# LARS-research/RED-GNN

Measured on AMD Instinct MI355X. Metric: edges aggregated/sec + MRR-eval queries/sec, family KG n_layer=3 at 1/2/4/8 GPU, higher is better.
Workload: dtype f32; 1 GPU; C2 synthetic KG 10000 entities / 50 relations / 200000 triples (seed 1234), n_layer=3 hidden_dim=64 attn_dim=5, eval step = expansion + fused layers + GRU/readout + filtered ranking, 1024 queries per GPU; batch_per_gpu=1024, global_batch=1024

## Files before the change

include/redgnn.h:

```cpp
#ifndef REDGNN_H
#define REDGNN_H

#include <stddef.h>
#include <stdint.h>

#ifdef __cplusplus
extern "C" {
#endif

typedef struct rg_graph rg_graph;
typedef struct rg_frontier rg_frontier;

const char* rg_last_error(void);
int rg_version(void);
int rg_hipgraph_fill_nodes(void* hip_graph);

int rg_graph_create(int32_t n_ent, int32_t n_rel, const int32_t* triples_host, int64_t n,
                    int add_inverse, rg_graph** out);
int rg_graph_create_device(int32_t n_ent, int32_t n_rel, const int32_t* triples_dev, int64_t n,
                           int add_inverse, void* stream, rg_graph** out);
int rg_graph_export_packs(const rg_graph* g, int32_t* n_packs, int32_t* n_vrows, int32_t* ent_host, int32_t* pack_host, int32_t* rows_host,
                          int32_t* vrows_host);
int rg_tgraph_create(int32_t n_ent, int32_t n_rela_rows, int32_t n_time, const int32_t* quads_host, int64_t n,
                     rg_graph** out);
int rg_tgraph_create_excluding(int32_t n_ent, int32_t n_rela_rows, int32_t n_time, const int32_t* quads_host, int64_t n,
                               const int64_t* exclude_rows_host, int64_t n_exclude, rg_graph** out);
int rg_graph_destroy(rg_graph* g);
int64_t rg_graph_n_fact(const rg_graph* g);
int rg_graph_export(const rg_graph* g, int32_t* out_ptr_host, int32_t* out_rel_tail_host,
                    int32_t* in_ptr_host, int32_t* in_head_rel_host);
int rg_graph_export_time(const rg_graph* g, int32_t* out_time_host, int32_t* in_time_host);

size_t rg_frontier_workspace_bytes(int32_t n_ent, int32_t batch, int32_t n_levels);
int rg_frontier_create(int32_t n_ent, int32_t batch, int32_t n_levels, void* workspace_dev,
                       size_t workspace_bytes, rg_frontier** out);
int rg_frontier_destroy(rg_frontier* f);
int rg_frontier_reset(rg_frontier* f, const int32_t* q_sub_dev, void* stream);
int rg_frontier_reset_nodes(rg_frontier* f, const int32_t* nodes_dev, int64_t n, void* stream);
int rg_frontier_expand(rg_frontier* f, const rg_graph* g, int64_t* counts_host, void* stream);
int rg_frontier_expand_async(rg_frontier* f, const rg_graph* g, void* stream);
int rg_frontier_expand_nodes_async(rg_frontier* f, const rg_graph* g, int32_t* nodes_out, int32_t* prev_idx_out, void* stream);
int rg_frontier_set_edge_hint(rg_frontier* f, int64_t n_edges);
const int32_t* rg_frontier_count_ptr(const rg_frontier* f);
int rg_frontier_level_counts(const rg_frontier* f, int64_t* counts_host, void* stream);
int rg_frontier_nodes(const rg_frontier* f, int32_t* nodes_out, int32_t* prev_idx_out,
                      int32_t* old_nodes_new_idx_out, void* stream);
size_t rg_frontier_edges_scratch_bytes(int64_t n_new);
int rg_frontier_edges(const rg_frontier* f, const rg_graph* g, int32_t level,
                      const int32_t* nodes_new, int64_t n_new, int32_t* edges_out,
                      int32_t* row_ptr_out, void* scratch_dev, void* stream);

size_t rg_layer_fwd_scratch_bytes(const rg_frontier* f, const rg_graph* g, int32_t ld);
int rg_layer_fwd_plan(const rg_frontier* f, const rg_graph* g, int32_t level, int64_t n_old, int64_t n_new,
                      int64_t n_edges, int32_t ld);
int rg_layer_fwd(const rg_frontier* f, const rg_graph* g, int32_t level, int64_t n_new,
                 const float* hidden, const float* rela, int32_t d, int32_t ld,
                 const float* a_s, const float* a_r, const float* a_q, int32_t ap,
                 const float* w_alpha, const float* b_alpha, int32_t attn_dim,
                 float* agg_out, void* scratch_dev, size_t scratch_bytes, int32_t walk, void* stream);

int rg_attn_tables(int32_t n_layer, int32_t n_rela_rows, int32_t batch, int32_t d, int32_t ld, int32_t attn_dim, int32_t ap,
                   const float* const* rela, const float* const* Wr, const float* const* Wqr, const float* const* bqr,
                   const int64_t* q_rel, float* a_r_out, float* a_q_out, float* rela_pad_out, void* stream);

int rg_tlayer_fwd(const rg_frontier* f, const rg_graph* g, int32_t level, int64_t n_new, const int32_t* q_time,
                  const float* hidden_dir, const float* rela_dir, const float* time_dir, int32_t d, int32_t ld,
                  const float* a_s, const float* a_r, const float* a_q, int32_t ap,
                  const float* w_alpha, const float* b_alpha, int32_t attn_dim,
                  float* agg_out, void* scratch_dev, size_t scratch_bytes, void* stream);

int rg_frontier_set_window(rg_frontier* f, const int32_t* win_lo_dev, const int32_t* win_hi_dev, int32_t n_data);
int rg_xlayer_fwd(const rg_frontier* f, const rg_graph* g, int32_t level, int64_t n_new, const int32_t* q_time,
                  const int32_t* loop_time, const int32_t* row_time, int32_t n_data,
                  const float* hidden_p, const float* rela_p, const float* time_p, int32_t n_tab, int32_t d, int32_t ld,
                  const float* a_s, const float* a_r, const float* a_q, int32_t ap,
                  const float* w_alpha, const float* b_alpha, int32_t attn_dim,
                  float* agg_out, void* scratch_dev, size_t scratch_bytes, void* stream);

size_t rg_layer_bwd_scratch_bytes(const rg_frontier* f, const rg_graph* g, int32_t ld, int32_t ap);
int rg_layer_bwd(const rg_frontier* f, const rg_graph* g, int32_t level, int64_t n_old,
                 const float* hidden, const float* rela, int32_t d, int32_t ld,
                 const float* a_s, const float* a_r, const float* a_q, int32_t ap,
                 const float* w_alpha, const float* b_alpha, int32_t attn_dim,
                 const float* grad_agg,
                 float* grad_hidden, float* grad_rela, float* grad_a_s, float* grad_a_r, float* grad_a_q,
                 float* grad_w_alpha, float* grad_b_alpha,
                 void* scratch_dev, size_t scratch_bytes, void* stream);

size_t rg_tlayer_bwd_scratch_bytes(const rg_frontier* f, const rg_graph* g, int32_t ld, int32_t ap);
int rg_tlayer_bwd(const rg_frontier* f, const rg_graph* g, int32_t level, int64_t n_old, const int32_t* q_time,
                  const float* hidden_dir, const float* rela_dir, const float* time_dir, int32_t d, int32_t ld,
                  const float* a_s, const float* a_r, const float* a_q, int32_t ap,
                  const float* w_alpha, const float* b_alpha, int32_t attn_dim,
                  const float* grad_agg,
                  float* grad_hidden_dir, float* grad_rela_dir, float* grad_time_dir, float* grad_a_s, float* grad_a_r,
                  float* grad_a_q, float* grad_w_alpha,
                  void* scratch_dev, size_t scratch_bytes, void* stream);

int rg_xlayer_bwd(const rg_frontier* f, const rg_graph* g, int32_t level, int64_t n_old, const int32_t* q_time,
                  const int32_t* loop_time, const int32_t* row_time, int32_t n_data,
                  const float* hidden_p, const float* rela_p, const float* time_p, int32_t n_tab, int32_t d, int32_t ld,
                  const float* a_s, const float* a_r, const float* a_q, int32_t ap,
                  const float* w_alpha, const float* b_alpha, int32_t attn_dim,
                  const float* grad_agg,
                  float* grad_hidden_p, float* grad_rela_p, float* grad_time_p, float* grad_a_s, float* grad_a_r,
                  float* grad_a_q, float* grad_w_alpha,
                  void* scratch_dev, size_t scratch_bytes, void* stream);
// ... 128 lines not shown
```

red-gnn_amd/_lib.py:

```python
import ctypes as C
import os

_PKG = os.path.dirname(os.path.abspath(__file__))
LIB_PATH = os.environ.get("RG_LIB") or os.path.join(_PKG, "libredgnn.so")

SYMBOLS = [
    "rg_last_error", "rg_version", "rg_hipgraph_fill_nodes",
    "rg_graph_create", "rg_graph_create_device", "rg_graph_export_packs", "rg_tgraph_create", "rg_tgraph_create_excluding", "rg_graph_destroy", "rg_graph_n_fact", "rg_graph_export",
    "rg_frontier_workspace_bytes", "rg_frontier_create", "rg_frontier_destroy", "rg_frontier_reset",
    "rg_frontier_reset_nodes", "rg_frontier_expand", "rg_frontier_nodes", "rg_frontier_edges_scratch_bytes", "rg_frontier_edges",
    "rg_layer_fwd_scratch_bytes", "rg_layer_fwd", "rg_layer_fwd_plan", "rg_tlayer_fwd", "rg_xlayer_fwd", "rg_frontier_set_window", "rg_layer_bwd_scratch_bytes", "rg_layer_bwd", "rg_tlayer_bwd_scratch_bytes", "rg_tlayer_bwd", "rg_xlayer_bwd", "rg_dense_fwd_supported", "rg_dense_scratch_bytes", "rg_dense_fwd", "rg_dense_fwd_dev", "rg_dense_train_fwd", "rg_dense_train_fwd_as", "rg_rows_addmm", "rg_dense_train_bwd", "rg_dense_train_bwd2", "rg_split3_roundtrip", "rg_split3_product_check", "rg_gram_tn_scratch_bytes", "rg_gram_tn", "rg_rank",
    "rg_frontier_expand_async", "rg_frontier_expand_nodes_async", "rg_frontier_set_edge_hint", "rg_frontier_count_ptr", "rg_frontier_level_counts", "rg_attn_tables",
    "rg_explain_scratch_bytes", "rg_explain_seed", "rg_explain_count", "rg_explain_emit", "rg_explain_gather",
    "rg_topk",
    "rg_attn_profile",
    "rg_graph_export_time", "rg_texplain_count", "rg_texplain_emit", "rg_tattn_profile",
    "rg_segment_rank", "rg_segment_topk",
    "rg_xexplain_count", "rg_xexplain_emit",
    "rg_xattn_profile", "rg_rows_linear",
    "rg_segment_eval",
    "rg_paths_scratch_bytes", "rg_paths_topk",
]

_lib = None


class NativeError(RuntimeError):
    pass


def lib():
    global _lib
    if _lib is not None:
        return _lib
    if not os.path.exists(LIB_PATH):
        raise NativeError(
            "libredgnn.so is missing at %s: the HIP extension is not built. Run "
            "`python -c 'import __graft_entry__ as g; g.build()'` (needs hipcc). There is no CPU fallback." % LIB_PATH)
    import torch
    L = C.CDLL(LIB_PATH)
    vp, i32, i64, sz = C.c_void_p, C.c_int32, C.c_int64, C.c_size_t
    L.rg_last_error.restype = C.c_char_p
    L.rg_version.restype = C.c_int
    L.rg_hipgraph_fill_nodes.argtypes = [vp]
    L.rg_graph_create.argtypes = [i32, i32, vp, i64, C.c_int, C.POINTER(vp)]
    L.rg_graph_create_device.argtypes = [i32, i32, vp, i64, C.c_int, vp, C.POINTER(vp)]
    L.rg_graph_export_packs.argtypes = [vp, C.POINTER(i32), C.POINTER(i32), vp, vp, vp, vp]
    L.rg_tgraph_create.argtypes = [i32, i32, i32, vp, i64, C.POINTER(vp)]
    L.rg_tgraph_create_excluding.argtypes = [i32, i32, i32, vp, i64, vp, i64, C.POINTER(vp)]
    L.rg_graph_destroy.argtypes = [vp]
    L.rg_graph_n_fact.argtypes = [vp]
    L.rg_graph_n_fact.restype = i64
    L.rg_graph_export.argtypes = [vp, vp, vp, vp, vp]
    L.rg_frontier_workspace_bytes.argtypes = [i32, i32, i32]
    L.rg_frontier_workspace_bytes.restype = sz
    L.rg_frontier_create.argtypes = [i32, i32, i32, vp, sz, C.POINTER(vp)]
    L.rg_frontier_destroy.argtypes = [vp]
    L.rg_frontier_reset.argtypes = [vp, vp, vp]
    L.rg_frontier_reset_nodes.argtypes = [vp, vp, i64, vp]
    L.rg_frontier_expand.argtypes = [vp, vp, C.POINTER(i64), vp]
    L.rg_frontier_expand_async.argtypes = [vp, vp, vp]
    L.rg_frontier_expand_nodes_async.argtypes = [vp, vp, vp, vp, vp]
    L.rg_frontier_set_edge_hint.argtypes = [vp, i64]
    L.rg_attn_tables.argtypes = [i32, i32, i32, i32, i32, i32, i32, vp, vp, vp, vp, vp, vp, vp, vp, vp]
    L.rg_frontier_count_ptr.argtypes = [vp]
    L.rg_frontier_count_ptr.restype = vp
    L.rg_frontier_level_counts.argtypes = [vp, C.POINTER(i64), vp]
    L.rg_frontier_nodes.argtypes = [vp, vp, vp, vp, vp]
    L.rg_frontier_edges_scratch_bytes.argtypes = [i64]
    L.rg_frontier_edges_scratch_bytes.restype = sz
    L.rg_frontier_edges.argtypes = [vp, vp, i32, vp, i64, vp, vp, vp, vp]
    L.rg_layer_fwd_scratch_bytes.argtypes = [vp, vp, i32]
    L.rg_layer_fwd_scratch_bytes.restype = sz
    L.rg_layer_fwd.argtypes = [vp, vp, i32, i64, vp, vp, i32, i32, vp, vp, vp, i32, vp, vp, i32, vp, vp, sz, i32, vp]
    L.rg_layer_fwd_plan.argtypes = [vp, vp, i32, i64, i64, i64, i32]
    L.rg_tlayer_fwd.argtypes = [vp, vp, i32, i64, vp, vp, vp, vp, i32, i32, vp, vp, vp, i32, vp, vp, i32, vp, vp, sz, vp]
    L.rg_xlayer_fwd.argtypes = [vp, vp, i32, i64, vp, vp, vp, i32, vp, vp, vp, i32, i32, i32, vp, vp, vp, i32, vp, vp, i32, vp, vp, sz, vp]
    L.rg_frontier_set_window.argtypes = [vp, vp, vp, i32]
    L.rg_layer_bwd_scratch_bytes.argtypes = [vp, vp, i32, i32]
    L.rg_layer_bwd_scratch_bytes.restype = sz
    L.rg_layer_bwd.argtypes = [vp, vp, i32, i64, vp, vp, i32, i32, vp, vp, vp, i32, vp, vp, i32,
                               vp, vp, vp, vp, vp, vp, vp, vp, vp, sz, vp]
    L.rg_tlayer_bwd_scratch_bytes.argtypes = [vp, vp, i32, i32]
    L.rg_tlayer_bwd_scratch_bytes.restype = sz
    L.rg_tlayer_bwd.argtypes = [vp, vp, i32, i64, vp, vp, vp, vp, i32, i32, vp, vp, vp, i32, vp, vp, i32,
                                vp, vp, vp, vp, vp, vp, vp, vp, vp, sz, vp]
    L.rg_xlayer_bwd.argtypes = [vp, vp, i32, i64, vp, vp, vp, i32, vp, vp, vp, i32, i32, i32, vp, vp, vp, i32, vp, vp, i32,
                                vp, vp, vp, vp, vp, vp, vp, vp, vp, sz, vp]
    L.rg_dense_fwd_supported.argtypes = [i32, i32]
    L.rg_dense_fwd.argtypes = [i64, i32, i32, vp, vp, vp, vp, i32, vp, vp, vp, vp, vp, i32, i32, vp, vp, vp, i32, vp, vp, i32, vp, i64, vp]
    L.rg_dense_scratch_bytes.argtypes = [i32, i32]
    L.rg_dense_scratch_bytes.restype = i64
    L.rg_dense_fwd_dev.argtypes = [i64, vp, i64, i32, i32, vp, vp, vp, vp, i32, vp, vp, vp, vp, vp, i32, i32, vp, vp, vp, i32, vp, vp, i32, vp, i64, vp]
    L.rg_dense_train_fwd.argtypes = [i64, i32, vp, vp, vp, vp, i32, vp, vp, vp, vp, vp, vp, vp, vp, vp]
    L.rg_dense_train_fwd_as.argtypes = [i64, i32, vp, vp, vp, vp, i32, vp, vp, vp, vp, vp, vp, i32, i32, vp, vp, vp, vp, vp]
    L.rg_rows_addmm.argtypes = [vp, i64, vp, i64, i32, vp, i32, i64, vp, i64, vp]
    L.rg_dense_train_bwd.argtypes = [i64, i32, vp, vp, vp, vp, C.c_float, i32, vp, vp, vp, vp, vp, vp, vp, vp, vp]
    L.rg_dense_train_bwd2.argtypes = [i64, i32, vp, vp, vp, vp, C.c_float, i32, vp, vp, vp, vp, vp, vp, vp, vp, vp, vp]
    L.rg_rank.argtypes = [vp, i32, i32, vp, vp, vp, vp, vp, vp]
    L.rg_topk.argtypes = [vp, i32, i32, i32, vp, vp, vp, vp, i64, vp, vp, vp]
    L.rg_split3_roundtrip.argtypes = [vp, i64, i32, vp, vp, vp]
    L.rg_gram_tn_scratch_bytes.argtypes = [i32, i32]
    L.rg_gram_tn_scratch_bytes.restype = sz
    L.rg_gram_tn.argtypes = [vp, i64, i32, vp, i64, i32, i64, vp, vp, vp, sz, vp]
    L.rg_split3_product_check.argtypes = [i32, i64, i32, vp, vp, vp, vp, i32, vp, vp, vp, vp, vp, vp]
    L.rg_explain_scratch_bytes.argtypes = [vp]
    L.rg_explain_scratch_bytes.restype = sz
    L.rg_explain_seed.argtypes = [vp, i32, i32, i32, vp, vp, vp, vp]
    L.rg_explain_count.argtypes = [vp, vp, i32, i32, i32, vp, vp, vp, vp, i32, vp, vp, i32, C.c_float, vp, vp, vp, sz,
                                   C.POINTER(i64), vp]
    L.rg_explain_emit.argtypes = [vp, vp, i32, i32, i32, vp, vp, vp, vp, i32, vp, vp, i32, C.c_float, vp, vp, vp, vp]
    L.rg_explain_gather.argtypes = [i64, i32, i32, vp, vp, vp, vp, i64, vp, vp, vp]
    L.rg_attn_profile.argtypes = [vp, vp, i32, i32, i32, i64, vp, vp, vp, i32, vp, vp, i32, vp, vp, vp]
    L.rg_graph_export_time.argtypes = [vp, vp, vp]
    L.rg_texplain_count.argtypes = L.rg_explain_count.argtypes
    L.rg_texplain_emit.argtypes = [vp, vp, i32, i32, i32, vp, vp, vp, vp, i32, vp, vp, i32, C.c_float, vp, vp, vp, vp, vp]
    L.rg_tattn_profile.argtypes = [vp, vp, i32, i32, i32, i64, vp, vp, vp, vp, i32, vp, vp, i32, vp, vp, vp]
    L.rg_segment_rank.argtypes = [vp, vp, i64, vp, i32, vp, i32, vp, vp, vp, vp, i64, vp, vp, vp, vp, i64, vp, vp, vp, vp, vp]
    L.rg_segment_topk.argtypes = [vp, vp, i64, vp, i32, i32, i32, vp, vp, vp, vp, i64, vp, vp, vp, vp]
    L.rg_segment_eval.argtypes = [vp, vp, i64, vp, i32, vp, i32, i32, vp, vp, vp, vp, i64, vp, vp, vp, vp, i64, vp, vp, vp, vp]
    L.rg_xexplain_count.argtypes = L.rg_explain_count.argtypes
    L.rg_xexplain_emit.argtypes = L.rg_texplain_emit.argtypes
    L.rg_rows_linear.argtypes = [vp, i64, i64, i32, vp, vp, i32, vp, i64, vp]
    L.rg_xattn_profile.argtypes = [vp, vp, i32, i32, i32, i64, vp, vp, vp, vp, i32, i32, vp, vp, vp, i32, vp, vp, i32, vp, vp, vp]
    L.rg_paths_scratch_bytes.argtypes = [i64, i32]
    L.rg_paths_scratch_bytes.restype = sz
    L.rg_paths_topk.argtypes = [vp, vp, vp, i32, i32, i32, i32, vp, vp, vp, vp, vp]
    _lib = L
# ... 20 lines not shown
```

red-gnn_amd/csrc/common.h:

```cpp
#pragma once
#include <hip/hip_runtime.h>
#include <stdint.h>
#include <stdio.h>
#include <string>
#include <type_traits>

#include "redgnn.h"

namespace rg {

void set_error(const char* fmt, ...);

#define RG_CHECK(cond, ...)                 \
  do {                                      \
    if (!(cond)) {                          \
      ::rg::set_error(__VA_ARGS__);         \
      return 1;                             \
    }                                       \
  } while (0)

#define RG_HIP(expr)                                                                  \
  do {                                                                                \
    hipError_t e_ = (expr);                                                           \
    if (e_ != hipSuccess) {                                                           \
// ... 45 lines not shown
  return v + __int_as_float(t);
}

template <int G>
__device__ __forceinline__ float group_sum(float v) {
  if constexpr (G >= 16) {
    v = dpp_add<0x128>(v);
    v = dpp_add<0x124>(v);
    v = dpp_add<0x122>(v);
    v = dpp_add<0x121>(v);
    if constexpr (G >= 32) v += __shfl_xor(v, 16, 64);
    if constexpr (G >= 64) v += __shfl_xor(v, 32, 64);
  } else {
    for (int o = G / 2; o > 0; o >>= 1) v += __shfl_xor(v, o, 64);
  }
  return v;
}

}

#include <vector>
namespace rg { int place_rows_best_fit(const int4* vrows, int32_t n_vrows, std::vector<int4>* place, std::vector<int32_t>* pack_nrows); }

constexpr int RG_VROW_MAX = 128;
struct rg_vrows {
  int32_t n = 0, n_split = 0, n_slots = 0;
  int4* rows = nullptr;
  int4* split = nullptr;
};

constexpr int RG_PACK = 128;
struct rg_packs {
  int32_t n = 0;
  int2* ent = nullptr;
  int4* pack = nullptr;
  int2* rows = nullptr;
};

struct rg_graph {
  void* arena = nullptr;
  int32_t n_ent = 0, n_rel = 0;
  int32_t n_rela_rows = 0;
  int32_t n_time = 0;
  int32_t* in_time = nullptr;
  int32_t* out_time = nullptr;
  int64_t n_fact = 0;
  int32_t max_in_deg = 0, max_out_deg = 0;
  int32_t* out_ptr = nullptr;
  int2* out_rt = nullptr;
  int32_t* in_ptr = nullptr;
  int2* in_hr = nullptr;
  uint32_t* in_pk = nullptr;
  uint32_t* out_pk = nullptr;
  rg_vrows in_vr, out_vr;
  rg_packs in_pk_packs;
  int32_t* rel_ptr = nullptr;
  int2* rel_ht = nullptr;
  rg_vrows rel_vr;
  int32_t* rel_tm = nullptr;
  int32_t* time_ptr = nullptr;
  int2* time_ht = nullptr;
  int32_t* time_rel = nullptr;
  rg_vrows time_vr;
};

constexpr int RG_MAX_LEVELS = 16;
constexpr int RG_QSTRIDE = 32;
constexpr size_t RG_QUEUE_BYTES = 8 * RG_QSTRIDE * sizeof(int32_t);
struct rg_frontier {
  int32_t n_ent = 0, B = 0, BW = 0, W = 0, n_levels = 0;
  uint32_t* bitsT[2] = {nullptr, nullptr};
  int2* bm[RG_MAX_LEVELS] = {};
  uint32_t* words_tmp = nullptr;
  int32_t* prefix_tmp = nullptr;
  int32_t* scan_scratch = nullptr;
  int32_t* counters = nullptr;
  const int32_t* win_lo = nullptr;
  const int32_t* win_hi = nullptr;
  int32_t win_n_data = 0;
  mutable bool queues_clean = false;
  int32_t* queues = nullptr;
  int64_t* counts_pinned = nullptr;
  int level = -1;
  int tcur = 0;
  int64_t n_nodes[RG_MAX_LEVELS] = {};
  int64_t n_edges = 0;
  int64_t edge_hint = -1;
  const int2* bm_of(int lvl) const { return bm[lvl % n_levels]; }
};
```

red-gnn_amd/csrc/dense.hip:

```cpp
#include "dense_common.h"

using namespace rg;

namespace {

template <int DP>
__device__ __forceinline__ int sw(int row, int slot) { return row * (DP / 4) + (slot ^ (row & (DP / 4 - 1))); }


template <int NB, bool TRAIN>
__global__ __launch_bounds__(DENSE_T, 2) void dense_kernel(DenseArgs A) {
  constexpr int DP = 16 * NB;
  constexpr int S = DP / 4;
  constexpr int KS = DP / 4;
  constexpr int NW = DENSE_T / 64;
  extern __shared__ float4 lds[];
  if (A.n_dev) { A.n = *A.n_dev; A.n_tiles = (int)((A.n + 15) / 16); }
  float4* Wh_l = lds;
  float4* Wih_l = Wh_l + DP * S;
  float4* Whh_l = Wih_l + 3 * DP * S;
  float4* E_l = Whh_l + 3 * DP * S;
  float* bias_l = reinterpret_cast<float*>(E_l + 32 * S);
  float4* tiles = reinterpret_cast<float4*>(bias_l + 4 * DP);

// ... 186 lines not shown

    float hn[KS];
#pragma unroll
    for (int ob = 0; ob < NB; ++ob) {
      f32x4 ar = bias_acc(0, ob), az = bias_acc(1, ob), ai = bias_acc(2, ob), ah = bias_acc(3, ob);
      mma3(Wih_l, 0 * DP + 16 * ob, 1 * DP + 16 * ob, 2 * DP + 16 * ob, xf, ar, az, ai);
      if (any_old) mma3(Whh_l, 0 * DP + 16 * ob, 1 * DP + 16 * ob, 2 * DP + 16 * ob, hf, ar, az, ah);
      float rgv[4], zgv[4], ngv[4];
#pragma unroll
      for (int r = 0; r < 4; ++r) {
        const float rg = fast_sigmoid(ar[r]), zg = fast_sigmoid(az[r]);
        const float ng = fast_tanh(ai[r] + rg * ah[r]);
        hn[4 * ob + r] = (1.0f - zg) * ng + zg * hf[4 * ob + r];
        rgv[r] = rg; zgv[r] = zg; ngv[r] = ng;
      }
      if constexpr (TRAIN) {
        const int64_t nd = row0 + li;
        const int col = 16 * ob + 4 * hq;
        if (nd < A.n && col < d) {
          float* w = A.ws_out + nd * (5 * (int64_t)d) + col;
          *reinterpret_cast<float4*>(w) = make_float4(rgv[0], rgv[1], rgv[2], rgv[3]);
          *reinterpret_cast<float4*>(w + d) = make_float4(zgv[0], zgv[1], zgv[2], zgv[3]);
          *reinterpret_cast<float4*>(w + 2 * d) = make_float4(ngv[0], ngv[1], ngv[2], ngv[3]);
          *reinterpret_cast<float4*>(w + 3 * d) = make_float4(hf[4 * ob + 0], hf[4 * ob + 1], hf[4 * ob + 2], hf[4 * ob + 3]);
          *reinterpret_cast<float4*>(w + 4 * d) = make_float4(ah[0], ah[1], ah[2], ah[3]);
        }
      }
    }

    const int64_t node = row0 + li;
    if (A.Ws) {
      const f32x4 ae = mma(E_l, 0, hn, zero4);
      if (node < A.n && 4 * hq < A.ap)
        reinterpret_cast<float4*>(A.a_s_out + node * A.ap)[hq] = make_float4(ae[0], ae[1], ae[2], ae[3]);
    }
    if (A.W_final) {
      const f32x4 ae = mma(E_l, 16, hn, zero4);
      if (node < A.n && hq == 0) {
        const int b = A.nodes[2 * node], e = A.nodes[2 * node + 1];
        A.scores[(int64_t)b * A.n_ent + e] = ae[0];
      }
    }

    __builtin_amdgcn_fence(__ATOMIC_RELEASE, "workgroup");
    __builtin_amdgcn_wave_barrier();
#pragma unroll
    for (int ob = 0; ob < NB; ++ob)
      tile[sw<DP>(li, 4 * ob + hq)] = make_float4(hn[4 * ob + 0], hn[4 * ob + 1], hn[4 * ob + 2], hn[4 * ob + 3]);
    __builtin_amdgcn_fence(__ATOMIC_RELEASE, "workgroup");
    __builtin_amdgcn_wave_barrier();
#pragma unroll
    for (int it = 0; it < 16 * S / 64; ++it) {
      const int e = it * 64 + lane, r = e / S, sl = e - r * S;
      if (row0 + r < A.n && sl < A.ld4) A.hidden_out[(row0 + r) * A.ld4 + sl] = tile[sw<DP>(r, sl)];
    }
  }
}

template <int NB, bool TRAIN>
int launch(const DenseArgs& A, hipStream_t s) {
  constexpr int DP = 16 * NB, S = DP / 4, NW = DENSE_T / 64;
  const size_t lds = (size_t)(7 * DP * S + 32 * S) * sizeof(float4) + 4 * DP * sizeof(float) + (size_t)NW * 16 * S * sizeof(float4);
  RG_HIP(hipFuncSetAttribute((const void*)dense_kernel<NB, TRAIN>, hipFuncAttributeMaxDynamicSharedMemorySize, (int)lds));
  hipLaunchKernelGGL((dense_kernel<NB, TRAIN>), dim3(dense_grid(A, NW)), dim3(DENSE_T), lds, s, A);
  RG_LAUNCH_CHECK();
  return 0;
}

}

extern "C" int64_t rg_dense_scratch_bytes(int32_t d, int32_t precision) {
  if (d != 128) return 0;
  return precision == 1 ? rg::dense128_split_scratch_bytes() : precision == 2 ? rg::dense128_split3_scratch_bytes() : 0;
}

extern "C" int rg_dense_fwd_supported(int32_t d, int32_t attn_dim) { return ((d >= 1 && d <= 64) || d == 128) && attn_dim <= 16; }

static int dense_fwd_impl(int64_t n, const int32_t* n_dev, int64_t n_hint, int32_t d, int32_t ld, const float* agg, const float* hidden_prev,
                          const int32_t* prev_idx, const float* W_h, int32_t act, const float* w_ih, const float* w_hh,
                          const float* b_ih, const float* b_hh, const float* Ws_next, int32_t attn_dim, int32_t ap,
                          float* a_s_out, const float* W_final, const int32_t* nodes, int32_t n_ent, float* scores_all,
                          float* hidden_out, int32_t precision, void* scratch, int64_t scratch_bytes, void* stream) {
  RG_CHECK(agg && W_h && w_ih && w_hh && b_ih && b_hh && hidden_out, "rg_dense_fwd: NULL argument");
  RG_CHECK(precision >= 0 && precision <= 2, "rg_dense_fwd: precision=%d (0 = f32 MFMA, 1 = two-term f16 split, 2 = exact three-term f16 split)",
           precision);
  RG_CHECK(!prev_idx || hidden_prev, "rg_dense_fwd: prev_idx given without hidden_prev");
  RG_CHECK((d >= 1 && d <= 64) || d == 128, "rg_dense_fwd: hidden_dim %d not supported by the fused kernel (<= 64, or 128)", d);
  RG_CHECK(ld >= d && ld % 4 == 0 && ld <= 128, "rg_dense_fwd: ld=%d", ld);
  RG_CHECK(act >= 0 && act <= 2, "rg_dense_fwd: act=%d", act);
  RG_CHECK(!Ws_next || (a_s_out && attn_dim >= 1 && attn_dim <= 16 && ap >= attn_dim && ap % 4 == 0 && ap <= 16),
           "rg_dense_fwd: attn_dim=%d ap=%d not supported (<= 16)", attn_dim, ap);
  RG_CHECK(!W_final || (nodes && scores_all && n_ent > 0), "rg_dense_fwd: readout needs nodes and scores_all");
  RG_CHECK((((uintptr_t)agg | (uintptr_t)hidden_prev | (uintptr_t)hidden_out | (uintptr_t)a_s_out) & 15) == 0,
           "rg_dense_fwd: float buffers must be 16-B aligned");
  if (n == 0) return 0;
  DenseArgs A = dense_args(n, d, ld, agg, hidden_prev, prev_idx, W_h, act, w_ih, w_hh, b_ih, b_hh, hidden_out);
  A.n_dev = n_dev; A.n_hint = n_hint;
  A.Ws = Ws_next; A.attn = attn_dim; A.ap = ap; A.a_s_out = a_s_out;
  A.W_final = W_final; A.nodes = nodes; A.n_ent = n_ent; A.scores = scores_all;
  hipStream_t s = (hipStream_t)stream;
  if (d == 128)
    return precision == 1 ? rg::dense128_split_launch(A, scratch, scratch_bytes, s)
         : precision == 2 ? rg::dense128_split3_launch(A, scratch, scratch_bytes, s) : rg::dense128_launch(A, s);
  if (precision == 1) return rg::dense_split_launch(A, s);
  if (precision == 2) return rg::dense_split3_launch(A, s);
  return d <= 32 ? launch<2, false>(A, s) : launch<4, false>(A, s);
}

extern "C" int rg_dense_fwd(int64_t n, int32_t d, int32_t ld, const float* agg, const float* hidden_prev,
                            const int32_t* prev_idx, const float* W_h, int32_t act, const float* w_ih, const float* w_hh,
                            const float* b_ih, const float* b_hh, const float* Ws_next, int32_t attn_dim, int32_t ap,
                            float* a_s_out, const float* W_final, const int32_t* nodes, int32_t n_ent, float* scores_all,
                            float* hidden_out, int32_t precision, void* scratch, int64_t scratch_bytes, void* stream) {
  return dense_fwd_impl(n, nullptr, 0, d, ld, agg, hidden_prev, prev_idx, W_h, act, w_ih, w_hh, b_ih, b_hh, Ws_next, attn_dim, ap,
                        a_s_out, W_final, nodes, n_ent, scores_all, hidden_out, precision, scratch, scratch_bytes, stream);
}

extern "C" int rg_dense_fwd_dev(int64_t n_cap, const int32_t* n_dev, int64_t n_hint, int32_t d, int32_t ld, const float* agg,
                                const float* hidden_prev, const int32_t* prev_idx, const float* W_h, int32_t act,
                                const float* w_ih, const float* w_hh, const float* b_ih, const float* b_hh, const float* Ws_next,
                                int32_t attn_dim, int32_t ap, float* a_s_out, const float* W_final, const int32_t* nodes,
                                int32_t n_ent, float* scores_all, float* hidden_out, int32_t precision, void* scratch,
                                int64_t scratch_bytes, void* stream) {
  RG_CHECK(n_dev != nullptr, "rg_dense_fwd_dev: n_dev is NULL");
  return dense_fwd_impl(n_cap, n_dev, n_hint, d, ld, agg, hidden_prev, prev_idx, W_h, act, w_ih, w_hh, b_ih, b_hh, Ws_next, attn_dim, ap,
                        a_s_out, W_final, nodes, n_ent, scores_all, hidden_out, precision, scratch, scratch_bytes, stream);
}

static int dense_train_fwd_impl(const char* who, int64_t n, int32_t d, const float* agg, const float* hidden_prev, const int32_t* prev_idx,
                                const float* W_h, int32_t act, const float* w_ih, const float* w_hh, const float* b_ih,
                                const float* b_hh, const float* mask, const float* Ws_next, int32_t attn_dim, int32_t ap,
                                float* hidden_out, float* x_out, float* gates_ws_out, float* a_s_out, void* stream) {
  RG_CHECK(agg && W_h && w_ih && w_hh && b_ih && b_hh && hidden_out && x_out && gates_ws_out, "%s: NULL argument", who);
  RG_CHECK(!prev_idx || hidden_prev, "%s: prev_idx given without hidden_prev", who);
  RG_CHECK((d >= 16 && d <= 64 && d % 4 == 0) || d == 128, "%s: hidden_dim %d not supported (16..64 in steps of 4, or 128)", who, d);
  RG_CHECK(act >= 0 && act <= 2, "%s: act=%d", who, act);
// ... 30 lines not shown
```

red-gnn_amd/csrc/dense128.hip:

```cpp
#include "dense_common.h"

namespace rg {
namespace {

constexpr int DP = 128, S = 32, KS = 32, NB = 8, NW = 8, T = 512;
constexpr int BLK = 16 * S;
constexpr int CHUNK = 3 * BLK;
constexpr int NL = 16 * S / 64;

__device__ __forceinline__ int swz(int row, int slot) { return row * S + (slot ^ (row & (S - 1))); }

template <bool TRAIN>
__global__ __launch_bounds__(T, 2) void dense128_kernel(DenseArgs A) {
  extern __shared__ float4 lds[];
  if (A.n_dev) { A.n = *A.n_dev; A.n_tiles = (int)((A.n + 15) / 16); }
  float4* wbuf = lds;
  float4* E_l = wbuf + 2 * CHUNK;
  float* bias_l = reinterpret_cast<float*>(E_l + 32 * S);
  float4* tiles = reinterpret_cast<float4*>(bias_l + 4 * DP);

  for (int i = threadIdx.x; i < 32 * S; i += T) {
    const int r = i / S, sl = i - r * S;
    const float* src = r < 16 ? (A.Ws && r < A.attn ? A.Ws + (int64_t)r * DP : nullptr) : (r == 16 ? A.W_final : nullptr);
    E_l[swz(r, sl)] = src ? *reinterpret_cast<const float4*>(src + 4 * sl) : make_float4(0.f, 0.f, 0.f, 0.f);
// ... 181 lines not shown
      if (hh) issue(r_hh, 16 * ob, DP + 16 * ob, 2 * DP + 16 * ob);
      else if (!last) issue(r_ih, 16 * (ob + 1), DP + 16 * (ob + 1), 2 * DP + 16 * (ob + 1));
      mma3(xf, ar, az, ai);
      if (hh || !last) publish(); else __syncthreads();
      if (hh) {
        if (!last) issue(r_ih, 16 * (ob + 1), DP + 16 * (ob + 1), 2 * DP + 16 * (ob + 1));
        mma3(hf, ar, az, ah);
        if (!last) publish(); else __syncthreads();
      }
      __builtin_amdgcn_sched_barrier(0);
#pragma unroll
      for (int r = 0; r < 4; ++r) {
        const float rg = fast_sigmoid(ar[r]), zg = fast_sigmoid(az[r]);
        const float ng = fast_tanh(ai[r] + rg * ah[r]);
        hn[4 * ob + r] = (1.0f - zg) * ng + zg * hf[4 * ob + r];
        if constexpr (TRAIN) { ar[r] = rg; az[r] = zg; ai[r] = ng; }
      }
      if constexpr (TRAIN) {
        const int64_t nd = row0 + li;
        if (nd < A.n) {
          float* w = A.ws_out + nd * (5 * (int64_t)DP) + 16 * ob + 4 * hq;
          *reinterpret_cast<float4*>(w) = make_float4(ar[0], ar[1], ar[2], ar[3]);
          *reinterpret_cast<float4*>(w + DP) = make_float4(az[0], az[1], az[2], az[3]);
          *reinterpret_cast<float4*>(w + 2 * DP) = make_float4(ai[0], ai[1], ai[2], ai[3]);
          *reinterpret_cast<float4*>(w + 3 * DP) = make_float4(hf[4 * ob + 0], hf[4 * ob + 1], hf[4 * ob + 2], hf[4 * ob + 3]);
          *reinterpret_cast<float4*>(w + 4 * DP) = make_float4(ah[0], ah[1], ah[2], ah[3]);
        }
      }
      __builtin_amdgcn_sched_barrier(0);
    }

    const int64_t node = row0 + li;
    if (A.Ws) {
      const f32x4 ae = mma_e(0, hn);
      if (node < A.n && 4 * hq < A.ap)
        reinterpret_cast<float4*>(A.a_s_out + node * A.ap)[hq] = make_float4(ae[0], ae[1], ae[2], ae[3]);
    }
    if (A.W_final) {
      const f32x4 ae = mma_e(16, hn);
      if (node < A.n && hq == 0) {
        const int b = A.nodes[2 * node], e = A.nodes[2 * node + 1];
        A.scores[(int64_t)b * A.n_ent + e] = ae[0];
      }
    }

    wave_sync();
#pragma unroll
    for (int ob = 0; ob < NB; ++ob)
      tile[swz(li, 4 * ob + hq)] = make_float4(hn[4 * ob + 0], hn[4 * ob + 1], hn[4 * ob + 2], hn[4 * ob + 3]);
    wave_sync();
#pragma unroll
    for (int it = 0; it < NL; ++it) {
      const int e = it * 64 + lane, r = e / S, sl = e - r * S;
      if (row0 + r < A.n) A.hidden_out[(row0 + r) * S + sl] = tile[swz(r, sl)];
    }
  }
}

}

int dense128_launch(const DenseArgs& A, hipStream_t s) {
  RG_CHECK(A.d == DP && A.ld4 == S, "rg_dense_fwd: the d = 128 kernel needs ld = 128 (got d=%d ld=%d)", A.d, A.ld4 * 4);
  const size_t lds = (size_t)(2 * CHUNK + 32 * S + NW * 16 * S) * sizeof(float4) + 4 * DP * sizeof(float);
  auto kern = A.ws_out ? dense128_kernel<true> : dense128_kernel<false>;
  RG_HIP(hipFuncSetAttribute((const void*)kern, hipFuncAttributeMaxDynamicSharedMemorySize, (int)lds));
  hipLaunchKernelGGL(kern, dim3(dense_grid(A, NW)), dim3(T), lds, s, A);
  RG_LAUNCH_CHECK();
  return 0;
}

}
```

red-gnn_amd/csrc/dense128_split.hip:

```cpp
#include "split3.h"

namespace rg {
namespace {

using namespace rg::sp3;

constexpr int DP = 128, NB = 8, KST = 4, KS = 32, NW = 8, T = 512;
constexpr int S = 32;
constexpr int BLK_B = 8192;
constexpr int CHUNK_B = 3 * BLK_B;
constexpr int N_BLOCKS = 58;
constexpr int HDR_B = 256;

__global__ __launch_bounds__(T) void prepare128_kernel(const float* __restrict__ W_h, const float* __restrict__ w_ih,
                                                        const float* __restrict__ w_hh, const float* __restrict__ Ws, int attn,
                                                        const float* __restrict__ W_final, char* __restrict__ image) {
  const int r = threadIdx.x >> 5, ch = threadIdx.x & 31;
  const float4 q = prepare128_scaled_chunk<T>(W_h, w_ih, w_hh, Ws, attn, W_final, image, r, ch);
  h4 hi, lo;
  split4(q.x, q.y, q.z, q.w, hi, lo);
  const int b = blockIdx.x, kb = ch >> 2, hq = ch & 3;
  const int slot = (4 * (kb >> 1) + hq) ^ (r & 15);
  char* blk = image + HDR_B + (int64_t)b * BLK_B;
  reinterpret_cast<h4*>(blk + (r * 16 + slot) * 16)[kb & 1] = hi;
// ... 171 lines not shown

    h8 gh[KST], gl[KST];
    float sc, inv;
    if (hh) {
      float hf[KS];
#pragma unroll
      for (int ob = 0; ob < NB; ++ob) {
        my_stash[ob * 64] = vh[ob];
        hf[4 * ob] = vh[ob].x; hf[4 * ob + 1] = vh[ob].y; hf[4 * ob + 2] = vh[ob].z; hf[4 * ob + 3] = vh[ob].w;
      }
      row_scale(row_abs_max(hf, row_abs_max(xf, 0.f)), sc, inv);
      split_frag(hf, sc, gh, gl);
    } else {
      row_scale(row_abs_max(xf, 0.f), sc, inv);
    }
    split_frag(xf, sc, xh, xl);
    const float inv_s = inv * inv_w * -LOG2E, inv_t = inv * inv_w * (-2.0f * LOG2E);
    h8 nh[KST], nl[KST];
    h4 nh0, nl0;
#pragma unroll
    for (int ob = 0; ob < NB; ++ob) {
      f32x4 ar = zero4, az = zero4, ai = zero4, ag = zero4;
      const bool last = ob == NB - 1;
      if (hh) issue(32 + ob, 40 + ob, 48 + ob);
      else if (!last) issue(8 + ob + 1, 16 + ob + 1, 24 + ob + 1);
      else issue(0, 1, 2);
      mma3(xh, xl, ar, az, ai);
      if (hh || !last) publish(); else __syncthreads();
      if (hh) {
        if (!last) issue(8 + ob + 1, 16 + ob + 1, 24 + ob + 1);
        else issue(0, 1, 2);
        mma3(gh, gl, ar, az, ag);
        if (!last) publish(); else __syncthreads();
      }
      const float4 br = *reinterpret_cast<const float4*>(bias_l + 0 * DP + 16 * ob + 4 * hq);
      const float4 bz = *reinterpret_cast<const float4*>(bias_l + 1 * DP + 16 * ob + 4 * hq);
      const float4 bi = *reinterpret_cast<const float4*>(bias_l + 2 * DP + 16 * ob + 4 * hq);
      const float4 bh = *reinterpret_cast<const float4*>(bias_l + 3 * DP + 16 * ob + 4 * hq);
      float4 ho = make_float4(0.f, 0.f, 0.f, 0.f);
      if (hh) ho = my_stash[ob * 64];
      const float hov[4] = {ho.x, ho.y, ho.z, ho.w};
      const float brv[4] = {br.x, br.y, br.z, br.w}, bzv[4] = {bz.x, bz.y, bz.z, bz.w};
      const float biv[4] = {bi.x, bi.y, bi.z, bi.w}, bhv[4] = {bh.x, bh.y, bh.z, bh.w};
      float hnv[4];
#pragma unroll
      for (int r = 0; r < 4; ++r) {
        const float rg = __builtin_amdgcn_rcpf(1.0f + __builtin_amdgcn_exp2f(fmaf(ar[r], inv_s, brv[r])));
        const float zg = __builtin_amdgcn_rcpf(1.0f + __builtin_amdgcn_exp2f(fmaf(az[r], inv_s, bzv[r])));
        const float ti = fmaf(ai[r], inv_t, biv[r]);
        const float th = fmaf(ag[r], inv_t, bhv[r]);
        const float ng = fmaf(2.0f, __builtin_amdgcn_rcpf(1.0f + __builtin_amdgcn_exp2f(fmaf(rg, th, ti))), -1.0f);
        hnv[r] = fmaf(zg, hov[r] - ng, ng);
      }
      if (node_ok) (A.hidden_out + row0 * S)[lane_off + 4 * ob] = make_float4(hnv[0], hnv[1], hnv[2], hnv[3]);
      h4 ch, cl;
      split4(hnv[0], hnv[1], hnv[2], hnv[3], ch, cl);
      if (ob & 1) {
        nh[ob >> 1] = __builtin_shufflevector(nh0, ch, 0, 1, 2, 3, 4, 5, 6, 7);
        nl[ob >> 1] = __builtin_shufflevector(nl0, cl, 0, 1, 2, 3, 4, 5, 6, 7);
      } else {
        nh0 = ch; nl0 = cl;
      }
    }

    if (A.Ws) {
      const f32x4 ae = mma_e(0, nh, nl);
      if (node_ok && 4 * hq < A.ap)
        reinterpret_cast<float4*>(A.a_s_out + node * A.ap)[hq] = make_float4(ae[0] * inv_e, ae[1] * inv_e, ae[2] * inv_e, ae[3] * inv_e);
    }
    if (A.W_final) {
      const f32x4 ae = mma_e(1, nh, nl);
      if (node_ok && hq == 0) A.scores[(int64_t)qe.x * A.n_ent + qe.y] = ae[0] * inv_e;
    }
  }
}

template <int ACT>
int launch(const DenseArgs& A, const char* image, hipStream_t s) {
  const size_t lds = 2 * CHUNK_B + 2 * BLK_B + 4 * DP * sizeof(float) + (size_t)NW * NB * 64 * sizeof(float4);
  RG_HIP(hipFuncSetAttribute((const void*)dense128_split_kernel<ACT>, hipFuncAttributeMaxDynamicSharedMemorySize, (int)lds));
  hipLaunchKernelGGL((dense128_split_kernel<ACT>), dim3(dense_grid(A, NW)), dim3(T), lds, s, A, image);
  RG_LAUNCH_CHECK();
  return 0;
}

}

int64_t dense128_split_scratch_bytes() { return HDR_B + (int64_t)N_BLOCKS * BLK_B; }

int dense128_split_launch(const DenseArgs& A, void* scratch, int64_t scratch_bytes, hipStream_t s) {
  RG_CHECK(A.d == DP && A.ld4 == S, "rg_dense_fwd: the d = 128 kernel needs ld = 128 (got d=%d ld=%d)", A.d, A.ld4 * 4);
  RG_CHECK(scratch && scratch_bytes >= dense128_split_scratch_bytes() && ((uintptr_t)scratch & 255) == 0,
           "rg_dense_fwd: precision 1 at d = 128 needs a 256-B aligned scratch of rg_dense_scratch_bytes(128, 1) = %lld bytes",
           (long long)dense128_split_scratch_bytes());
  char* image = (char*)scratch;
  hipLaunchKernelGGL(prepare128_kernel, dim3(N_BLOCKS), dim3(T), 0, s, A.W_h, A.w_ih, A.w_hh, A.Ws, A.attn, A.W_final, image);
  RG_LAUNCH_CHECK();
  return with_act(A.act, [&](auto ACT) { return launch<decltype(ACT)::value>(A, image, s); });
}

}
```

red-gnn_amd/csrc/dense128_split3.hip:

```cpp
#include "split3.h"

namespace rg {
namespace {

using namespace rg::sp3;
typedef long l2v __attribute__((ext_vector_type(2)));

constexpr int DP = 128, NB = 8, KST = 4, KS = 32, NW = 4, T = 256;
constexpr int S = 32;
constexpr int F16_B = 4096;
constexpr int LO_B = 2048;
constexpr int BLK_B = 2 * F16_B + LO_B;
constexpr int CHUNK_B = 3 * BLK_B;
constexpr int N_BLOCKS = 58;
constexpr int HDR_B = 256;
constexpr int PREP_T = 512;

__device__ __forceinline__ int lo_quad(int row, int hq, int half) { return (((hq & 1) + 2 * half + 4 * (hq >> 1)) ^ (2 * ((row >> 1) & 3))); }

__global__ __launch_bounds__(PREP_T) void prepare128x3_kernel(const float* __restrict__ W_h, const float* __restrict__ w_ih,
                                                               const float* __restrict__ w_hh, const float* __restrict__ Ws, int attn,
                                                               const float* __restrict__ W_final, char* __restrict__ image) {
  const int r = threadIdx.x >> 5, ch = threadIdx.x & 31;
  const float4 q = prepare128_scaled_chunk<PREP_T>(W_h, w_ih, w_hh, Ws, attn, W_final, image, r, ch);
// ... 218 lines not shown
    drop();
    const bool hh = __syncthreads_or(has_old) != 0;
    cur ^= 1;

    float xf[KS];
    const float sc_out = inv1 * inv_w * (ACT == 2 ? -2.0f * LOG2E : 1.0f);
    auto act_store = [&](f32x4 acc, const f32x4& acc8, int ob) {
      join(acc, acc8);
#pragma unroll
      for (int r = 0; r < 4; ++r) {
        float v = acc[r] * sc_out;
        if (ACT == 1) v = fmaxf(v, 0.f);
        else if (ACT == 2) v = fmaf(2.0f, __builtin_amdgcn_rcpf(1.0f + __builtin_amdgcn_exp2f(v)), -1.0f);
        xf[4 * ob + r] = v;
      }
    };
    {
      f32x4 c[3] = {zero4, zero4, zero4}, e[3] = {zero4, zero4, zero4};
      issue(3, 4, 5);
      mma3(X, c, e);
      act_store(c[0], e[0], 0); act_store(c[1], e[1], 1); act_store(c[2], e[2], 2);
      publish();
    }
    {
      f32x4 c[3] = {zero4, zero4, zero4}, e[3] = {zero4, zero4, zero4};
      issue(6, 7, 7);
      mma3(X, c, e);
      act_store(c[0], e[0], 3); act_store(c[1], e[1], 4); act_store(c[2], e[2], 5);
      publish();
    }
    {
      f32x4 c[3] = {zero4, zero4, zero4}, e[3] = {zero4, zero4, zero4};
      issue(8, 16, 24);
      mma3(X, c, e);
      act_store(c[0], e[0], 6); act_store(c[1], e[1], 7);
      publish();
    }

    Frag4 H;
    float sc, inv;
    float hf[KS];
#pragma unroll
    for (int ob = 0; ob < NB; ++ob) { hf[4 * ob] = vh[ob].x; hf[4 * ob + 1] = vh[ob].y; hf[4 * ob + 2] = vh[ob].z; hf[4 * ob + 3] = vh[ob].w; }
    if (hh) {
      row_scale(row_abs_max(hf, row_abs_max(xf, 0.f)), sc, inv);
      split_frag(hf, sc, H);
    } else {
      row_scale(row_abs_max(xf, 0.f), sc, inv);
    }
    split_frag(xf, sc, X);
    const float inv_s = inv * inv_w * -LOG2E, inv_t = inv * inv_w * (-2.0f * LOG2E);
    float hn[KS];
    const int rows_valid = (int)(A.n - row0 < 16 ? (A.n - row0 > 0 ? A.n - row0 : 0) : 16);
    const __amdgpu_buffer_rsrc_t r_out = __builtin_amdgcn_make_buffer_rsrc(reinterpret_cast<char*>(A.hidden_out + row0 * S), 0,
                                                                            rows_valid * S * 16, 0x00020000);
    auto gate_loop = [&](auto HH_) {
      constexpr bool HH = decltype(HH_)::value;
      f32x4 P[2][4][3];
      static_for<NB + 1>([&](auto OB) {
        constexpr int ob = decltype(OB)::value, cs = ob & 1, ps = cs ^ 1, pb = ob - 1;
        constexpr int OPS_R = 25, NOPS = 4 + 4 * OPS_R + 1;
        float4 bia[4];
        float s1[4], a1[4], ar[4], az[4], ai[4], ag[4], t1[4], t2[4], e1[4], e2[4], rg[4], zg[4], ti[4], th[4], uu[4], e3[4], ng[4], hnv[4];
        auto gate_op = [&](auto K) {
          constexpr int k = decltype(K)::value;
          f32x4 (&c)[3] = P[ps][0]; f32x4 (&e)[3] = P[ps][1]; f32x4 (&cg)[3] = P[ps][2]; f32x4 (&eg)[3] = P[ps][3];
          if constexpr (k < 4) {
            bia[k] = *reinterpret_cast<const float4*>(bias_l + k * DP + 16 * pb + 4 * hq);
            RG_PIN(bia[k].x);
          } else if constexpr (k < 4 + 4 * OPS_R) {
            constexpr int j = (k - 4) / 4, r = (k - 4) % 4;
            const float bvr = r == 0 ? bia[0].x : r == 1 ? bia[0].y : r == 2 ? bia[0].z : bia[0].w;
            const float bvz = r == 0 ? bia[1].x : r == 1 ? bia[1].y : r == 2 ? bia[1].z : bia[1].w;
            const float bvi = r == 0 ? bia[2].x : r == 1 ? bia[2].y : r == 2 ? bia[2].z : bia[2].w;
            const float bvh = r == 0 ? bia[3].x : r == 1 ? bia[3].y : r == 2 ? bia[3].z : bia[3].w;
            if constexpr (j == 0) { s1[r] = HH ? e[0][r] + eg[0][r] : e[0][r]; RG_PIN(s1[r]); }
            else if constexpr (j == 1) { a1[r] = HH ? c[0][r] + cg[0][r] : c[0][r]; RG_PIN(a1[r]); }
            else if constexpr (j == 2) { ar[r] = fmaf(s1[r], LO8_INV, a1[r]); RG_PIN(ar[r]); }
            else if constexpr (j == 3) { s1[r] = HH ? e[1][r] + eg[1][r] : e[1][r]; RG_PIN(s1[r]); }
            else if constexpr (j == 4) { a1[r] = HH ? c[1][r] + cg[1][r] : c[1][r]; RG_PIN(a1[r]); }
            else if constexpr (j == 5) { az[r] = fmaf(s1[r], LO8_INV, a1[r]); RG_PIN(az[r]); }
            else if constexpr (j == 6) { ai[r] = fmaf(e[2][r], LO8_INV, c[2][r]); RG_PIN(ai[r]); }
            else if constexpr (j == 7) { ag[r] = HH ? fmaf(eg[2][r], LO8_INV, cg[2][r]) : 0.f; RG_PIN(ag[r]); }
            else if constexpr (j == 8) { t1[r] = fmaf(ar[r], inv_s, bvr); RG_PIN(t1[r]); }
            else if constexpr (j == 9) { e1[r] = __builtin_amdgcn_exp2f(t1[r]); RG_PIN(e1[r]); }
            else if constexpr (j == 10) { t2[r] = fmaf(az[r], inv_s, bvz); RG_PIN(t2[r]); }
            else if constexpr (j == 11) { e2[r] = __builtin_amdgcn_exp2f(t2[r]); RG_PIN(e2[r]); }
            else if constexpr (j == 12) { t1[r] = 1.0f + e1[r]; RG_PIN(t1[r]); }
            else if constexpr (j == 13) { t2[r] = 1.0f + e2[r]; RG_PIN(t2[r]); }
            else if constexpr (j == 14) { rg[r] = __builtin_amdgcn_rcpf(t1[r]); RG_PIN(rg[r]); }
            else if constexpr (j == 15) { zg[r] = __builtin_amdgcn_rcpf(t2[r]); RG_PIN(zg[r]); }
            else if constexpr (j == 16) { ti[r] = fmaf(ai[r], inv_t, bvi); RG_PIN(ti[r]); }
            else if constexpr (j == 17) { th[r] = fmaf(ag[r], inv_t, bvh); RG_PIN(th[r]); }
            else if constexpr (j == 18) { uu[r] = fmaf(rg[r], th[r], ti[r]); RG_PIN(uu[r]); }
            else if constexpr (j == 19) { e3[r] = __builtin_amdgcn_exp2f(uu[r]); RG_PIN(e3[r]); }
            else if constexpr (j == 20) { uu[r] = 1.0f + e3[r]; RG_PIN(uu[r]); }
            else if constexpr (j == 21) { e3[r] = __builtin_amdgcn_rcpf(uu[r]); RG_PIN(e3[r]); }
            else if constexpr (j == 22) { ng[r] = fmaf(2.0f, e3[r], -1.0f); RG_PIN(ng[r]); }
            else if constexpr (j == 23) { uu[r] = hf[4 * pb + r] - ng[r]; RG_PIN(uu[r]); }
            else { hnv[r] = fmaf(zg[r], uu[r], ng[r]); RG_PIN(hnv[r]); }
          } else {
#pragma unroll
            for (int r = 0; r < 4; ++r) hn[4 * pb + r] = hnv[r];
            const u32x4 bits = {__float_as_uint(hnv[0]), __float_as_uint(hnv[1]), __float_as_uint(hnv[2]), __float_as_uint(hnv[3])};
            __builtin_amdgcn_raw_buffer_store_b128(bits, r_out, (lane_off + 4u * pb) * 16u, 0, 0);
          }
        };
        auto no_op = [&](auto) {};
// ... 66 lines not shown
```

red-gnn_amd/csrc/dense_split.hip:

```cpp
#include <type_traits>
#include "split3.h"

using namespace rg;
using namespace rg::sp3;

namespace {

template <int NB, int ACT>
__global__ __launch_bounds__(DENSE_T, 2) void dense_split_kernel(DenseArgs A) {
  constexpr int DP = 16 * NB;
  using G = Geo<DP>;
  constexpr int SR = G::SR, KST = G::KST;
  constexpr int S = DP / 4;
  constexpr int KS = DP / 4;
  constexpr int NW = DENSE_T / 64;
  constexpr int IMG = DP * SR;
  extern __shared__ float4 lds[];
  if (A.n_dev) { A.n = *A.n_dev; A.n_tiles = (int)((A.n + 15) / 16); }
  h8* Wh_hi = reinterpret_cast<h8*>(lds);
  h8* Wh_lo = Wh_hi + IMG;
  h8* Wih_hi = Wh_lo + IMG;
  h8* Wih_lo = Wih_hi + 3 * IMG;
  h8* Whh_hi = Wih_lo + 3 * IMG;
  h8* Whh_lo = Whh_hi + 3 * IMG;
// ... 170 lines not shown
          xf[4 * ob + r] = v;
        }
      }
    }

    h8 nh[KST], nl[KST];
    auto gru = [&](auto has_old) {
      constexpr bool OLD = decltype(has_old)::value;
      h8 xh[KST], xl[KST], hh[KST], hl[KST];
      float sc, inv;
      if constexpr (OLD) {
        float hf[KS];
#pragma unroll
        for (int ob = 0; ob < NB; ++ob) {
          const float4 q = my_stash[ob * 64];
          hf[4 * ob] = q.x; hf[4 * ob + 1] = q.y; hf[4 * ob + 2] = q.z; hf[4 * ob + 3] = q.w;
        }
        row_scale(row_abs_max(hf, row_abs_max(xf, 0.f)), sc, inv);
        split_frag(hf, sc, hh, hl);
      } else {
        row_scale(row_abs_max(xf, 0.f), sc, inv);
      }
      split_frag(xf, sc, xh, xl);
      const float inv_s = inv * inv_w * -LOG2E, inv_t = inv * inv_w * (-2.0f * LOG2E);
      h4 nh0, nl0;
#pragma unroll
      for (int ob = 0; ob < NB; ++ob) {
        f32x4 ar = zero4, az = zero4, ai = zero4, ag = zero4;
        mma(O_WIH, O_WIH + P_G, 0 * DP + 16 * ob, xh, xl, ar);
        if constexpr (OLD) mma(O_WHH, O_WHH + P_G, 0 * DP + 16 * ob, hh, hl, ar);
        mma(O_WIH, O_WIH + P_G, 1 * DP + 16 * ob, xh, xl, az);
        if constexpr (OLD) mma(O_WHH, O_WHH + P_G, 1 * DP + 16 * ob, hh, hl, az);
        mma(O_WIH, O_WIH + P_G, 2 * DP + 16 * ob, xh, xl, ai);
        if constexpr (OLD) mma(O_WHH, O_WHH + P_G, 2 * DP + 16 * ob, hh, hl, ag);
        const float4 br = *reinterpret_cast<const float4*>(bias_l + 0 * DP + 16 * ob + 4 * hq);
        const float4 bz = *reinterpret_cast<const float4*>(bias_l + 1 * DP + 16 * ob + 4 * hq);
        const float4 bi = *reinterpret_cast<const float4*>(bias_l + 2 * DP + 16 * ob + 4 * hq);
        const float4 bh = *reinterpret_cast<const float4*>(bias_l + 3 * DP + 16 * ob + 4 * hq);
        float4 ho = make_float4(0.f, 0.f, 0.f, 0.f);
        if constexpr (OLD) ho = my_stash[ob * 64];
        const float hov[4] = {ho.x, ho.y, ho.z, ho.w};
        const float brv[4] = {br.x, br.y, br.z, br.w}, bzv[4] = {bz.x, bz.y, bz.z, bz.w};
        const float biv[4] = {bi.x, bi.y, bi.z, bi.w}, bhv[4] = {bh.x, bh.y, bh.z, bh.w};
        float hnv[4];
#pragma unroll
        for (int r = 0; r < 4; ++r) {
          const float rg = __builtin_amdgcn_rcpf(1.0f + __builtin_amdgcn_exp2f(fmaf(ar[r], inv_s, brv[r])));
          const float zg = __builtin_amdgcn_rcpf(1.0f + __builtin_amdgcn_exp2f(fmaf(az[r], inv_s, bzv[r])));
          const float ti = fmaf(ai[r], inv_t, biv[r]);
          const float th = OLD ? fmaf(ag[r], inv_t, bhv[r]) : bhv[r];
          const float ng = fmaf(2.0f, __builtin_amdgcn_rcpf(1.0f + __builtin_amdgcn_exp2f(fmaf(rg, th, ti))), -1.0f);
          hnv[r] = fmaf(zg, hov[r] - ng, ng);
        }
        if (node_ok && ((col_ok >> ob) & 1u))
          (A.hidden_out + row0 * A.ld4)[lane_off + 4 * ob] = make_float4(hnv[0], hnv[1], hnv[2], hnv[3]);
        h4 ch, cl;
        split4(hnv[0], hnv[1], hnv[2], hnv[3], ch, cl);
        if (ob & 1) {
          nh[ob >> 1] = __builtin_shufflevector(nh0, ch, 0, 1, 2, 3, 4, 5, 6, 7);
          nl[ob >> 1] = __builtin_shufflevector(nl0, cl, 0, 1, 2, 3, 4, 5, 6, 7);
        } else {
          nh0 = ch; nl0 = cl;
        }
      }
    };
    if (any_old) gru(std::true_type{}); else gru(std::false_type{});

    if (A.Ws) {
      f32x4 acc = zero4;
      mma(O_E, O_E + P_E, 0, nh, nl, acc);
      if (node_ok && 4 * hq < A.ap)
        reinterpret_cast<float4*>(A.a_s_out + node * A.ap)[hq] = make_float4(acc[0] * inv_w, acc[1] * inv_w, acc[2] * inv_w, acc[3] * inv_w);
    }
    if (A.W_final) {
      f32x4 acc = zero4;
      mma(O_E, O_E + P_E, 16, nh, nl, acc);
      if (node_ok && hq == 0) A.scores[(int64_t)qe.x * A.n_ent + qe.y] = acc[0] * inv_w;
    }
  }
}

template <int NB, int ACT>
int launch(const DenseArgs& A, hipStream_t s) {
  constexpr int DP = 16 * NB, SR = DP / 8, NW = DENSE_T / 64;
  const size_t lds = (size_t)(2 * 7 * DP * SR + 2 * 32 * SR) * 16 + 4 * DP * sizeof(float) + (size_t)NW * NB * 64 * sizeof(float4) + 16;
  RG_HIP(hipFuncSetAttribute((const void*)dense_split_kernel<NB, ACT>, hipFuncAttributeMaxDynamicSharedMemorySize, (int)lds));
  hipLaunchKernelGGL((dense_split_kernel<NB, ACT>), dim3(dense_grid(A, NW)), dim3(DENSE_T), lds, s, A);
  RG_LAUNCH_CHECK();
  return 0;
}

template <int NB>
int launch_act(const DenseArgs& A, hipStream_t s) {
  return with_act(A.act, [&](auto ACT) { return launch<NB, decltype(ACT)::value>(A, s); });
}

}

namespace rg {
int dense_split_launch(const DenseArgs& A, hipStream_t s) { return A.d <= 32 ? launch_act<2>(A, s) : launch_act<4>(A, s); }
}
```

red-gnn_amd/csrc/dense_split3.hip:

```cpp
#include "split3.h"

using namespace rg;
using namespace rg::sp3;

namespace {

template <int KST>
struct Frag {
  h8 h[KST], m[KST], l[KST];
  long q[KST];
};

template <int NB, int ACT, bool PROBE>
__global__ __launch_bounds__(DENSE_T, 2) void dense_split3_kernel(DenseArgs A) {
  constexpr int DP = 16 * NB;
  using G = Geo<DP>;
  constexpr int SR = G::SR, KST = G::KST;
  constexpr int S = DP / 4;
  constexpr int KS = DP / 4;
  constexpr int NW = DENSE_T / 64;
  constexpr int IMG = DP * SR;
  constexpr uint32_t O_WH = 0, O_WIH = 2 * IMG * 16, O_WHH = O_WIH + 6 * IMG * 16, O_E = O_WHH + 6 * IMG * 16;
  constexpr uint32_t P_W = IMG * 16, P_G = 3 * IMG * 16, P_E = 32 * SR * 16;
  constexpr uint32_t O_F16_END = O_E + 2 * P_E;
// ... 180 lines not shown
    asm volatile("" : "+v"(c_off));
    asm volatile("" : "+v"(lane_off));
    const bool node_ok = row0 + li < A.n;
    const bool any_old = __ballot(p_cur >= 0) != 0ull;

    float sc1, inv1;
    Frag<KST> F;
    {
      float fx[KS];
#pragma unroll
      for (int ob = 0; ob < NB; ++ob) { fx[4 * ob] = va[ob].x; fx[4 * ob + 1] = va[ob].y; fx[4 * ob + 2] = va[ob].z; fx[4 * ob + 3] = va[ob].w; }
      row_scale(row_abs_max(fx, 0.f), sc1, inv1);
      split_frag(fx, sc1, F);
    }
    load_agg(t + t_step, va);
    const int64_t node = row0 + li;
    int2 qe = make_int2(0, 0);
    if (A.W_final) qe = reinterpret_cast<const int2*>(A.nodes)[node < n_last ? node : n_last];

    float xf[KS];
    {
      const float sc_out = inv1 * inv_w * (ACT == 2 ? -2.0f * LOG2E : 1.0f);
#pragma unroll
      for (int ob = 0; ob < NB; ++ob) {
        f32x4 acc = zero4, acc8 = zero4;
        mma(O_WH, O_WH + P_W, L_WH, 16 * ob, F, acc, acc8);
        join(acc, acc8);
#pragma unroll
        for (int r = 0; r < 4; ++r) {
          float v = acc[r] * sc_out;
          if (ACT == 1) v = fmaxf(v, 0.f);
          else if (ACT == 2) v = fmaf(2.0f, __builtin_amdgcn_rcpf(1.0f + __builtin_amdgcn_exp2f(v)), -1.0f);
          xf[4 * ob + r] = v;
        }
      }
    }

    const int64_t score_at = (int64_t)qe.x * A.n_ent + qe.y;

    if (PROBE && A.probe == 1) {
#pragma unroll
      for (int ob = 0; ob < NB; ++ob)
        if (node_ok && ((col_ok >> ob) & 1u))
          (A.hidden_out + row0 * A.ld4)[lane_off + 4 * ob] = make_float4(xf[4 * ob], xf[4 * ob + 1], xf[4 * ob + 2], xf[4 * ob + 3]);
      p_cur = prev_of(t + t_step, p_next);
      load_old(t + t_step, p_cur, vh);
      p_next = load_prev(t + 2 * t_step);
      continue;
    }

    float hn[KS];
    const int rows_valid = (int)(A.n - row0 < 16 ? (A.n - row0 > 0 ? A.n - row0 : 0) : 16);
    const __amdgpu_buffer_rsrc_t r_out = __builtin_amdgcn_make_buffer_rsrc(
        reinterpret_cast<char*>(A.hidden_out + row0 * A.ld4), 0, rows_valid * A.ld4 * 16, 0x00020000);
    auto gru = [&](auto has_old) {
      constexpr bool OLD = decltype(has_old)::value;
      Frag<KST> H;
      float sc, inv;
      if constexpr (OLD) {
        float hf[KS];
#pragma unroll
        for (int ob = 0; ob < NB; ++ob) { hf[4 * ob] = vh[ob].x; hf[4 * ob + 1] = vh[ob].y; hf[4 * ob + 2] = vh[ob].z; hf[4 * ob + 3] = vh[ob].w; }
        const bool is_old = p_cur >= 0;
        row_scale(fmaxf(is_old ? row_abs_max(hf, 0.f) : 0.f, row_abs_max(xf, 0.f)), sc, inv);
        split_frag(hf, is_old ? sc : 0.f, H);
      } else {
        row_scale(row_abs_max(xf, 0.f), sc, inv);
      }
      p_cur = prev_of(t + t_step, p_next);
      load_old(t + t_step, p_cur, vh);
      p_next = load_prev(t + 2 * t_step);
      split_frag(xf, sc, F);
      const float inv_s = inv * inv_w * -LOG2E, inv_t = inv * inv_w * (-2.0f * LOG2E);
      auto products = [&](int ob, f32x4& ar, f32x4& az, f32x4& ai, f32x4& ag) {
        ar = zero4; az = zero4; ai = zero4; ag = zero4;
        {
          f32x4 r8 = zero4;
          mma(O_WIH, O_WIH + P_G, L_WIH, 0 * DP + 16 * ob, F, ar, r8);
          if constexpr (OLD) mma(O_WHH, O_WHH + P_G, L_WHH, 0 * DP + 16 * ob, H, ar, r8);
          join(ar, r8);
        }
        {
          f32x4 z8 = zero4;
          mma(O_WIH, O_WIH + P_G, L_WIH, 1 * DP + 16 * ob, F, az, z8);
          if constexpr (OLD) mma(O_WHH, O_WHH + P_G, L_WHH, 1 * DP + 16 * ob, H, az, z8);
          join(az, z8);
        }
        {
          f32x4 i8 = zero4;
          mma(O_WIH, O_WIH + P_G, L_WIH, 2 * DP + 16 * ob, F, ai, i8);
          join(ai, i8);
        }
        if constexpr (OLD) {
          f32x4 g8 = zero4;
          mma(O_WHH, O_WHH + P_G, L_WHH, 2 * DP + 16 * ob, H, ag, g8);
          join(ag, g8);
        }
      };
      auto gates = [&](int ob, const f32x4& ar, const f32x4& az, const f32x4& ai, const f32x4& ag) {
        const float4 br = *reinterpret_cast<const float4*>(bias_l + 0 * DP + 16 * ob + 4 * hq);
        const float4 bz = *reinterpret_cast<const float4*>(bias_l + 1 * DP + 16 * ob + 4 * hq);
        const float4 bi = *reinterpret_cast<const float4*>(bias_l + 2 * DP + 16 * ob + 4 * hq);
        const float4 bh = *reinterpret_cast<const float4*>(bias_l + 3 * DP + 16 * ob + 4 * hq);
        float hos[4] = {0.f, 0.f, 0.f, 0.f};
        if constexpr (OLD) {
          const int s = ob >> 1, j0 = 4 * (ob & 1);
          const h2 hh0 = {H.h[s][j0], H.h[s][j0 + 1]}, hh1 = {H.h[s][j0 + 2], H.h[s][j0 + 3]};
// ... 266 lines not shown
```

red-gnn_amd/csrc/frontier.hip:

```cpp
#include <string.h>

#include "attn.h"

namespace {

__global__ void reset_level0_kernel(const int32_t* __restrict__ q_sub, int B, int n_ent, int BW, int W, uint32_t* __restrict__ bitsT,
                                    int2* __restrict__ bm0, int32_t* __restrict__ counters) {
  const int64_t i = (int64_t)blockIdx.x * blockDim.x + threadIdx.x;
  if (i >= (int64_t)B * W) return;
  const int b = (int)(i / W), w = (int)(i - (int64_t)b * W);
  const int e = q_sub[b];
  const bool ok = e >= 0 && e < n_ent;
  const int ew = ok ? e >> 5 : W;
  bm0[i] = make_int2(w == ew ? (int)(1u << (e & 31)) : 0, b + (w > ew ? 1 : 0));
  if (w == 0) {
    if (ok) atomicOr(&bitsT[(int64_t)e * BW + (b >> 5)], 1u << (b & 31));
    else atomicOr((unsigned*)&counters[1], 1u);
    if (b == 0) { counters[0] = B; counters[4] = B; }
  }
}

__device__ __forceinline__ void end_of_hop(int32_t* __restrict__ counters, int32_t* __restrict__ queues, int slot, int t) {
  if (t < 4) {
    const int32_t v = counters[t];
    if (slot >= 0) counters[slot + t] = v;
    counters[8 + t] = v;
  }
  if (t >= 8 && t < 16) queues[(t - 8) * RG_QSTRIDE] = 0;
}
__global__ void snapshot_kernel(int32_t* __restrict__ counters, int32_t* __restrict__ queues, int slot) {
  end_of_hop(counters, queues, slot, threadIdx.x);
  __syncthreads();
  if (threadIdx.x == 0) { counters[2] = 0; counters[3] = 0; }
}

__global__ void reset_nodes_kernel(const int32_t* __restrict__ nodes, int64_t n, int B, int n_ent, int BW,
                                   uint32_t* __restrict__ bitsT, int32_t* counters) {
  const int64_t i = (int64_t)blockIdx.x * blockDim.x + threadIdx.x;
  if (i >= n) return;
  const int b = nodes[2 * i], e = nodes[2 * i + 1];
  if (e < 0 || e >= n_ent || b < 0 || b >= B) { atomicOr((unsigned*)&counters[1], 1u); return; }
  atomicOr(&bitsT[(int64_t)e * BW + (b >> 5)], 1u << (b & 31));
}

__global__ __launch_bounds__(256) void hop_or_kernel(const int4* __restrict__ vrows, int n_vrows,
                                                     const int2* __restrict__ in_hr, const uint32_t* __restrict__ oldT,
                                                     uint32_t* __restrict__ newT, int BW, int WL) {
  const int wave = (blockIdx.x * blockDim.x + threadIdx.x) >> 6;
  const int lane = threadIdx.x & 63;
  if (wave >= n_vrows) return;
  const int4 row = vrows[wave];
  const int t = row.x, beg = row.y, end = row.y + row.z;
  const int wl = lane & (WL - 1);
  const int el = lane / WL, EL = 64 / WL;
  for (int w0 = 0; w0 < BW; w0 += WL) {
    const int w = w0 + wl;
    uint32_t acc = 0;
    if (w < BW) {
      for (int j = beg + el; j < end; j += 4 * EL) {
        int hh[4];
#pragma unroll
        for (int u = 0; u < 4; ++u) hh[u] = (j + u * EL < end) ? in_hr[j + u * EL].x : -1;
#pragma unroll
        for (int u = 0; u < 4; ++u)
          if (hh[u] >= 0) acc |= oldT[(int64_t)hh[u] * BW + w];
      }
    }
    for (int o = WL; o < 64; o <<= 1) acc |= __shfl_xor(acc, o, 64);
// ... 192 lines not shown
    if (lane >= o) inc += t;
  }
  if (lane == 63) wsum[wv] = inc;
  __syncthreads();
  int32_t pre = inc - sum, total = 0;
  for (int w = 0; w < SMALL_T / 64; ++w) {
    const int32_t x = wsum[w];
    if (w < wv) pre += x;
    total += x;
  }
  for (int i = beg; i < end; ++i) {
    uint32_t w = words[i];
    bm_new[i] = make_int2((int)w, pre);
    if (nodes || prev_idx || old_new) {
      const int b = i / W, e0 = (i - b * W) * 32;
      uint32_t ow = 0; int op = 0;
      if ((prev_idx || old_new) && bm_old) { const int2 o = bm_old[i]; ow = (uint32_t)o.x; op = o.y; }
      int idx = pre;
      for (uint32_t rest = w; rest; rest &= rest - 1, ++idx) {
        const int pos = __ffs((int)rest) - 1;
        if (nodes) reinterpret_cast<int2*>(nodes)[idx] = make_int2(b, e0 + pos);
        const int prev = ((ow >> pos) & 1u) ? op + __popc(ow & ((1u << pos) - 1u)) : -1;
        if (prev_idx) prev_idx[idx] = prev;
        if (old_new && prev >= 0) old_new[prev] = idx;
      }
    }
    pre += __popc(w);
  }
  const int t = threadIdx.x;
  if (t < 4) {
    const int32_t v = t == 0 ? total : counters[t];
    if (t == 0) counters[0] = total;
    if (slot >= 0) counters[slot + t] = v;
    counters[8 + t] = v;
  }
  if (t >= 8 && t < 16) queues[(t - 8) * RG_QSTRIDE] = 0;
  __syncthreads();
  if (t == 0) { counters[2] = 0; counters[3] = 0; }
}

__global__ void set_last_kernel(int32_t* row_ptr, int64_t n, const int32_t* total) { row_ptr[n] = *total; }

size_t ws_layout(int32_t n_ent, int32_t B, int32_t n_levels, size_t* off ) {
  const size_t BW = (B + 31) / 32, W = (n_ent + 31) / 32;
  size_t o = 0;
  auto take = [&](size_t bytes) { size_t r = o; o = rg::align_up(o + bytes, 256); return r; };
  off[0] = take((size_t)n_ent * BW * 4);
  off[1] = take((size_t)n_ent * BW * 4);
  off[2] = take((size_t)B * W * 4);
  off[3] = take((size_t)B * W * 4);
  off[4] = take(rg::scan_scratch_elems((int64_t)B * W) * 4);
  off[5] = take(1024 + RG_QUEUE_BYTES);
  off[6] = take((size_t)n_levels * B * W * 8);
  return o;
}

}

extern "C" {

size_t rg_frontier_workspace_bytes(int32_t n_ent, int32_t batch, int32_t n_levels) {
  if (n_ent <= 0 || batch <= 0 || n_levels < 2 || n_levels > RG_MAX_LEVELS) return 0;
  size_t off[8];
  return ws_layout(n_ent, batch, n_levels, off);
}

int rg_frontier_create(int32_t n_ent, int32_t batch, int32_t n_levels, void* ws, size_t ws_bytes, rg_frontier** out) {
  RG_CHECK(out != nullptr, "rg_frontier_create: out is NULL");
  *out = nullptr;
  RG_CHECK(n_ent > 0 && batch > 0, "rg_frontier_create: n_ent=%d batch=%d must be positive", n_ent, batch);
  RG_CHECK(n_levels >= 2 && n_levels <= RG_MAX_LEVELS, "rg_frontier_create: n_levels=%d not in [2,%d]", n_levels, RG_MAX_LEVELS);
  RG_CHECK((int64_t)n_ent * batch < ((int64_t)1 << 31), "rg_frontier_create: batch*n_ent = %lld does not fit int32",
           (long long)n_ent * batch);
  size_t off[8];
  const size_t need = ws_layout(n_ent, batch, n_levels, off);
  RG_CHECK(ws != nullptr && ws_bytes >= need, "rg_frontier_create: workspace %zu B < required %zu B", ws_bytes, need);
  RG_CHECK(((uintptr_t)ws & 255) == 0, "rg_frontier_create: workspace must be 256-B aligned");
  rg_frontier* f = new rg_frontier();
  f->n_ent = n_ent; f->B = batch; f->BW = (batch + 31) / 32; f->W = (n_ent + 31) / 32; f->n_levels = n_levels;
  char* base = (char*)ws;
  f->bitsT[0] = (uint32_t*)(base + off[0]);
  f->bitsT[1] = (uint32_t*)(base + off[1]);
  f->words_tmp = (uint32_t*)(base + off[2]);
  f->prefix_tmp = (int32_t*)(base + off[3]);
  f->scan_scratch = (int32_t*)(base + off[4]);
  f->counters = (int32_t*)(base + off[5]);
  f->queues = f->counters + 256;
  for (int l = 0; l < n_levels; ++l) f->bm[l] = (int2*)(base + off[6] + (size_t)l * batch * f->W * 8);
  if (hipHostMalloc((void**)&f->counts_pinned, 1024, hipHostMallocDefault) != hipSuccess) {
    delete f;
    rg::set_error("rg_frontier_create: hipHostMalloc failed");
    return 1;
  }
  *out = f;
  return 0;
}

int rg_frontier_destroy(rg_frontier* f) {
  if (!f) return 0;
  if (f->counts_pinned) (void)hipHostFree(f->counts_pinned);
  delete f;
  return 0;
}

static int build_level(rg_frontier* f, hipStream_t s) {
  const int n_pairs = (f->W + 1) / 2;
  const int64_t waves = (int64_t)f->BW * n_pairs;
  hipLaunchKernelGGL(transpose_kernel, dim3(rg::ceil_div(waves, 4)), dim3(256), 0, s, f->bitsT[f->tcur], f->words_tmp,
                     f->n_ent, f->B, f->BW, f->W, n_pairs);
  RG_LAUNCH_CHECK();
  const int64_t nw = (int64_t)f->B * f->W;
  if (rg::scan_exclusive(f->words_tmp, f->prefix_tmp, nw, true, &f->counters[0], f->scan_scratch, s)) return 1;
  hipLaunchKernelGGL(pack_kernel, dim3(rg::ceil_div(nw, 256)), dim3(256), 0, s, f->words_tmp, f->prefix_tmp,
                     f->bm[f->level % f->n_levels], nw);
  RG_LAUNCH_CHECK();
  return 0;
}

int rg_frontier_reset(rg_frontier* f, const int32_t* q_sub, void* stream) {
  RG_CHECK(f && q_sub, "rg_frontier_reset: NULL argument");
  hipStream_t s = (hipStream_t)stream;
  f->level = 0; f->tcur = 0; f->n_edges = 0;
  if (rg::zero2_async(f->bitsT[0], rg::align_up((size_t)f->n_ent * f->BW * 4, 16), f->counters, 1024, s)) return 1;
  f->queues_clean = false;
  const int64_t nw = (int64_t)f->B * f->W;
  hipLaunchKernelGGL(reset_level0_kernel, dim3(rg::ceil_div(nw, 256)), dim3(256), 0, s, q_sub, f->B, f->n_ent, f->BW, f->W,
                     f->bitsT[0], f->bm[0], f->counters);
  RG_LAUNCH_CHECK();
  f->n_nodes[0] = f->B;
  return 0;
}

int rg_frontier_set_window(rg_frontier* f, const int32_t* win_lo, const int32_t* win_hi, int32_t n_data) {
  RG_CHECK(f != nullptr, "rg_frontier_set_window: frontier is NULL");
  RG_CHECK((win_lo == nullptr) == (win_hi == nullptr) && n_data >= 0, "rg_frontier_set_window: give both bounds (or neither)");
  f->win_lo = win_lo; f->win_hi = win_hi; f->win_n_data = n_data;
  return 0;
}

int rg_frontier_reset_nodes(rg_frontier* f, const int32_t* nodes, int64_t n, void* stream) {
  RG_CHECK(f && (nodes || n == 0) && n >= 0, "rg_frontier_reset_nodes: bad argument");
  hipStream_t s = (hipStream_t)stream;
  f->level = 0; f->tcur = 0; f->n_edges = 0;
  if (rg::zero2_async(f->bitsT[0], rg::align_up((size_t)f->n_ent * f->BW * 4, 16), f->counters, 1024, s)) return 1;
  f->queues_clean = false;
  if (n > 0) {
    hipLaunchKernelGGL(reset_nodes_kernel, dim3(rg::ceil_div(n, 256)), dim3(256), 0, s, nodes, n, f->B, f->n_ent, f->BW,
                       f->bitsT[0], f->counters);
    RG_LAUNCH_CHECK();
  }
  if (build_level(f, s)) return 1;
  if (rg::copy_words_async(&f->counters[4], &f->counters[0], 1, s)) return 1;
  f->n_nodes[0] = n;
  return 0;
}

static int enqueue_expand(rg_frontier* f, const rg_graph* g, hipStream_t s, int32_t* nodes = nullptr, int32_t* prev_idx = nullptr) {
  const uint32_t* oldT = f->bitsT[f->tcur];
  uint32_t* newT = f->bitsT[f->tcur ^ 1];
  int WL = 1;
  while (WL < f->BW && WL < 64) WL <<= 1;
  const bool windowed = f->win_lo != nullptr;
  RG_CHECK(!windowed || g->in_time, "rg_frontier_expand: time windows are set but the graph carries no data-row ids (rg_tgraph_create)");
  hipLaunchKernelGGL(hop_prologue_kernel, dim3(rg::ceil_div((int64_t)f->n_ent * f->BW, 256)), dim3(256), 0, s,
                     windowed ? (const int32_t*)nullptr : g->out_ptr, oldT, newT, f->n_ent, f->BW, (unsigned long long*)&f->counters[2]);
  RG_LAUNCH_CHECK();
  if (windowed)
    hipLaunchKernelGGL(hop_or_window_kernel, dim3(rg::ceil_div(g->in_vr.n, 4)), dim3(256), 0, s, g->in_vr.rows, g->in_vr.n, g->in_hr,
                       g->in_time, oldT, newT, f->BW, WL, f->B, f->win_lo, f->win_hi, f->win_n_data, (unsigned long long*)&f->counters[2]);
  else
    hipLaunchKernelGGL(hop_or_kernel, dim3(rg::ceil_div(g->in_vr.n, 4)), dim3(256), 0, s, g->in_vr.rows, g->in_vr.n, g->in_hr,
                       oldT, newT, f->BW, WL);
  RG_LAUNCH_CHECK();
  f->tcur ^= 1;
  f->level += 1;
  const int slot = f->level < RG_MAX_LEVELS ? 64 + 8 * f->level : -1;
  const int64_t nw = (int64_t)f->B * f->W;
  const int2* bm_old = f->bm_of(f->level - 1);
  if (nw <= SMALL_MAX_WORDS) {
    const bool split_emit = (nodes || prev_idx) && nw > 1024;
    hipLaunchKernelGGL(build_level_small_kernel, dim3(1), dim3(SMALL_T), (size_t)nw * 4, s, f->bitsT[f->tcur], f->n_ent, f->B, f->BW,
                       f->W, (f->W + 1) / 2, f->bm[f->level % f->n_levels], bm_old, f->counters, f->queues, slot,
                       split_emit ? (int32_t*)nullptr : nodes, split_emit ? (int32_t*)nullptr : prev_idx, (int32_t*)nullptr);
    RG_LAUNCH_CHECK();
    if (split_emit) {
      hipLaunchKernelGGL(emit_nodes_kernel, dim3(rg::ceil_div(nw * 32, 256)), dim3(256), 0, s, f->bm_of(f->level), bm_old, f->B, f->W,
                         nodes, prev_idx, (int32_t*)nullptr);
      RG_LAUNCH_CHECK();
    }
  } else {
    if (build_level(f, s)) return 1;
    hipLaunchKernelGGL(snapshot_kernel, dim3(1), dim3(64), 0, s, f->counters, f->queues, slot);
    RG_LAUNCH_CHECK();
    if (nodes || prev_idx) {
      hipLaunchKernelGGL(emit_nodes_kernel, dim3(rg::ceil_div(nw * 32, 256)), dim3(256), 0, s, f->bm_of(f->level), bm_old, f->B, f->W,
                         nodes, prev_idx, (int32_t*)nullptr);
      RG_LAUNCH_CHECK();
    }
  }
  f->queues_clean = true;
  return 0;
}

int rg_frontier_expand(rg_frontier* f, const rg_graph* g, int64_t* counts_host, void* stream) {
  RG_CHECK(f && g, "rg_frontier_expand: NULL argument");
// ... 108 lines not shown
```

red-gnn_amd/csrc/graph.hip:

```cpp
#include <stdarg.h>
#include <string.h>

#include <algorithm>
#include <vector>

#include "common.h"

namespace rg {

static thread_local std::string g_err;

void set_error(const char* fmt, ...) {
  char buf[1024];
  va_list ap;
  va_start(ap, fmt);
  vsnprintf(buf, sizeof(buf), fmt, ap);
  va_end(ap);
  g_err = buf;
}

constexpr int SCAN_T = 256;
constexpr int SCAN_ITEMS = 8;
constexpr int SCAN_TILE = SCAN_T * SCAN_ITEMS;

// ... 195 lines not shown
    if (r.z <= 0) continue;
    int32_t p;
    if (r.w >= 0) { p = (int32_t)fill.size(); fill.push_back(0); pack_nrows->push_back(0); }
    else {
      int room = r.z;
      while (room <= RG_PACK && open_by_room[room].empty()) ++room;
      if (room > RG_PACK) { p = (int32_t)fill.size(); fill.push_back(0); pack_nrows->push_back(0); room = RG_PACK; }
      else { p = open_by_room[room].back(); open_by_room[room].pop_back(); }
      if (room - r.z > 0) open_by_room[room - r.z].push_back(p);
    }
    (*place)[i] = make_int4(p, fill[p], (*pack_nrows)[p], 0);
    fill[p] += r.z;
    (*pack_nrows)[p] += 1;
  }
  return (int)fill.size();
}
}

static void host_packs(const std::vector<int4>& vrows, const std::vector<uint32_t>& in_pk, HostPacks* hp, rg_packs* out) {
  std::vector<int4> place;
  std::vector<int32_t> pack_nrows;
  const size_t n = (size_t)rg::place_rows_best_fit(vrows.data(), (int32_t)vrows.size(), &place, &pack_nrows);
  std::vector<int32_t> row0(n + 1, 0);
  for (size_t p = 0; p < n; ++p) row0[p + 1] = row0[p] + pack_nrows[p];
  hp->ent.assign(n * RG_PACK, make_int2(-1, 0));
  hp->pack.resize(n);
  hp->rows.resize(row0[n]);
  for (size_t i = 0; i < vrows.size(); ++i) {
    const int4& r = vrows[i];
    const int4& pl = place[i];
    if (pl.x < 0) continue;
    for (int32_t j = 0; j < r.z; ++j) hp->ent[(size_t)pl.x * RG_PACK + pl.y + j] = make_int2((int32_t)in_pk[r.y + j], pl.z);
    hp->rows[row0[pl.x] + pl.z] = make_int2(r.x, r.w);
    if (pl.z == 0) hp->pack[pl.x] = make_int4(row0[pl.x], pack_nrows[pl.x], r.w, r.x);
  }
  out->n = (int32_t)n;
}

struct Arena {
  struct Item { void** field; const void* src; size_t bytes, off; };
  std::vector<Item> items;
  size_t total = 0;
  template <typename P, typename V>
  void add(P** field, const V& v) {
    const size_t bytes = v.size() * sizeof(typename V::value_type);
    items.push_back({(void**)field, (const void*)v.data(), bytes, total});
    total += rg::align_up(std::max<size_t>(bytes, 16), 256);
  }
};

extern "C" {

const char* rg_last_error(void) { return rg::g_err.c_str(); }
int rg_version(void) { return 10; }

static int build_graph(int32_t n_ent, int32_t n_rel, int32_t n_rela_rows, const std::vector<int32_t>& H,
                       const std::vector<int32_t>& R, const std::vector<int32_t>& T, const std::vector<int32_t>* TIME,
                       int32_t n_time, rg_graph** out) {
  const int64_t n_fact = (int64_t)H.size();
  std::vector<int32_t> out_ptr(n_ent + 1, 0), in_ptr(n_ent + 1, 0);
  for (int64_t i = 0; i < n_fact; ++i) { out_ptr[H[i] + 1]++; in_ptr[T[i] + 1]++; }
  int32_t max_in = 0, max_out = 0;
  for (int32_t e = 0; e < n_ent; ++e) {
    max_out = out_ptr[e + 1] > max_out ? out_ptr[e + 1] : max_out;
    max_in = in_ptr[e + 1] > max_in ? in_ptr[e + 1] : max_in;
    out_ptr[e + 1] += out_ptr[e];
    in_ptr[e + 1] += in_ptr[e];
  }
  std::vector<int2> out_rt(n_fact), in_hr(n_fact);
  std::vector<int32_t> in_time(TIME ? n_fact : 0), out_time(TIME ? n_fact : 0);
  {
    std::vector<int32_t> po(out_ptr.begin(), out_ptr.end() - 1), pi(in_ptr.begin(), in_ptr.end() - 1);
    for (int64_t i = 0; i < n_fact; ++i) {
      const int32_t q = pi[T[i]]++;
      in_hr[q] = make_int2(H[i], R[i]);
      if (TIME) in_time[q] = (*TIME)[i];
    }
    std::vector<int32_t> by_rel(n_fact), out_fact(n_fact);
    {
      std::vector<int32_t> pr(n_rela_rows + 1, 0);
      for (int64_t i = 0; i < n_fact; ++i) pr[R[i] + 1]++;
      for (int32_t r = 0; r < n_rela_rows; ++r) pr[r + 1] += pr[r];
      for (int64_t i = 0; i < n_fact; ++i) by_rel[pr[R[i]]++] = (int32_t)i;
    }
    for (int64_t k = 0; k < n_fact; ++k) out_fact[po[H[by_rel[k]]]++] = by_rel[k];
    for (int64_t j = 0; j < n_fact; ++j) {
      const int32_t i = out_fact[j];
      out_rt[j] = make_int2(R[i], T[i]);
      if (TIME) out_time[j] = (*TIME)[i];
    }
  }
  rg_graph* g = new rg_graph();
  g->n_ent = n_ent; g->n_rel = n_rel; g->n_rela_rows = n_rela_rows; g->n_time = n_time;
  g->n_fact = n_fact; g->max_in_deg = max_in; g->max_out_deg = max_out;
  Arena A;
  A.add(&g->out_ptr, out_ptr); A.add(&g->in_ptr, in_ptr); A.add(&g->out_rt, out_rt); A.add(&g->in_hr, in_hr);
  if (TIME) { A.add(&g->in_time, in_time); A.add(&g->out_time, out_time); }
  std::vector<uint32_t> in_pk, out_pk;
  if (n_ent <= (1 << 20) && n_rela_rows <= (1 << 12)) {
    in_pk.resize(n_fact); out_pk.resize(n_fact);
    for (int64_t i = 0; i < n_fact; ++i) {
      in_pk[i] = ((uint32_t)in_hr[i].y << 20) | (uint32_t)in_hr[i].x;
      out_pk[i] = ((uint32_t)out_rt[i].x << 20) | (uint32_t)out_rt[i].y;
    }
    A.add(&g->in_pk, in_pk); A.add(&g->out_pk, out_pk);
  }
  std::vector<int32_t> rel_ptr(n_rela_rows + 1, 0), rel_tm(TIME ? n_fact : 0);
  std::vector<int2> rel_ht(n_fact);
  for (int64_t i = 0; i < n_fact; ++i) rel_ptr[R[i] + 1]++;
  for (int32_t r = 0; r < n_rela_rows; ++r) rel_ptr[r + 1] += rel_ptr[r];
  {
    std::vector<int32_t> pr(rel_ptr.begin(), rel_ptr.end() - 1);
    for (int64_t i = 0; i < n_fact; ++i) {
      const int32_t q = pr[R[i]]++;
      rel_ht[q] = make_int2(H[i], T[i]);
      if (TIME) rel_tm[q] = (*TIME)[i];
    }
  }
  A.add(&g->rel_ptr, rel_ptr); A.add(&g->rel_ht, rel_ht);
  std::vector<int32_t> time_ptr, time_rel;
  std::vector<int2> time_ht;
  HostVrows hv_in, hv_out, hv_rel, hv_time;
  if (TIME) {
    A.add(&g->rel_tm, rel_tm);
    time_ptr.assign(n_time + 1, 0); time_rel.resize(n_fact); time_ht.resize(n_fact);
    for (int64_t i = 0; i < n_fact; ++i) time_ptr[(*TIME)[i] + 1]++;
    for (int32_t t = 0; t < n_time; ++t) time_ptr[t + 1] += time_ptr[t];
    std::vector<int32_t> pt(time_ptr.begin(), time_ptr.end() - 1);
    for (int64_t i = 0; i < n_fact; ++i) {
      const int32_t q = pt[(*TIME)[i]]++;
      time_ht[q] = make_int2(H[i], T[i]);
      time_rel[q] = R[i];
    }
    A.add(&g->time_ptr, time_ptr); A.add(&g->time_ht, time_ht); A.add(&g->time_rel, time_rel);
    host_vrows(time_ptr, n_time, &hv_time, &g->time_vr);
    A.add(&g->time_vr.rows, hv_time.rows); A.add(&g->time_vr.split, hv_time.split);
  }
  host_vrows(in_ptr, n_ent, &hv_in, &g->in_vr);
  host_vrows(out_ptr, n_ent, &hv_out, &g->out_vr);
  host_vrows(rel_ptr, n_rela_rows, &hv_rel, &g->rel_vr);
  A.add(&g->in_vr.rows, hv_in.rows); A.add(&g->in_vr.split, hv_in.split);
  A.add(&g->out_vr.rows, hv_out.rows); A.add(&g->out_vr.split, hv_out.split);
  A.add(&g->rel_vr.rows, hv_rel.rows); A.add(&g->rel_vr.split, hv_rel.split);
  HostPacks hp;
  if (!TIME && !in_pk.empty() && n_rela_rows < (1 << 12)) {
    host_packs(hv_in.rows, in_pk, &hp, &g->in_pk_packs);
    A.add(&g->in_pk_packs.ent, hp.ent); A.add(&g->in_pk_packs.pack, hp.pack); A.add(&g->in_pk_packs.rows, hp.rows);
  }

  std::vector<char> staging(A.total);
  for (const Arena::Item& it : A.items)
    if (it.bytes) memcpy(staging.data() + it.off, it.src, it.bytes);
  hipError_t e = hipMalloc(&g->arena, A.total);
  if (e == hipSuccess) e = hipMemcpy(g->arena, staging.data(), A.total, hipMemcpyHostToDevice);
  if (e != hipSuccess) {
    rg::set_error("rg_graph_create: uploading %zu B failed: %s", A.total, hipGetErrorString(e));
    rg_graph_destroy(g);
    return 1;
// ... 26 lines not shown
}

static int tgraph_create(const char* who, int32_t n_ent, int32_t n_rela_rows, int32_t n_time, const int32_t* quads, int64_t n,
                         const int64_t* exclude, int64_t n_exclude, rg_graph** out) {
  RG_CHECK(out != nullptr, "%s: out is NULL", who);
  *out = nullptr;
  RG_CHECK(n_ent > 0 && n_rela_rows > 0 && n_time > 0, "%s: n_ent=%d n_rela_rows=%d n_time=%d must be positive", who, n_ent, n_rela_rows, n_time);
  RG_CHECK(n >= 0 && n < ((int64_t)1 << 31) && (n == 0 || quads != nullptr), "%s: bad quadruples (n=%lld)", who, (long long)n);
  RG_CHECK(n_exclude >= 0 && (n_exclude == 0 || exclude != nullptr), "%s: bad exclusion list", who);
  std::vector<char> drop(n_exclude ? n : 0, 0);
  for (int64_t k = 0; k < n_exclude; ++k) {
    RG_CHECK(exclude[k] >= 0 && exclude[k] < n, "%s: excluded row %lld out of range (n=%lld)", who, (long long)exclude[k], (long long)n);
    drop[exclude[k]] = 1;
  }
  std::vector<int32_t> H, R, T, TM;
  H.reserve(n); R.reserve(n); T.reserve(n); TM.reserve(n);
  for (int64_t i = 0; i < n; ++i) {
    if (n_exclude && drop[i]) continue;
    const int32_t h = quads[4 * i], r = quads[4 * i + 1], t = quads[4 * i + 2], tm = quads[4 * i + 3];
    RG_CHECK(h >= 0 && h < n_ent && t >= 0 && t < n_ent && r >= 0 && r < n_rela_rows && tm >= 0 && tm < n_time,
             "%s: quadruple %lld = (%d,%d,%d,%d) out of range", who, (long long)i, h, r, t, tm);
    H.push_back(h); R.push_back(r); T.push_back(t); TM.push_back(tm);
  }
  return build_graph(n_ent, 0, n_rela_rows, H, R, T, &TM, n_time, out);
}

int rg_tgraph_create(int32_t n_ent, int32_t n_rela_rows, int32_t n_time, const int32_t* quads, int64_t n, rg_graph** out) {
  return tgraph_create("rg_tgraph_create", n_ent, n_rela_rows, n_time, quads, n, nullptr, 0, out);
}

int rg_tgraph_create_excluding(int32_t n_ent, int32_t n_rela_rows, int32_t n_time, const int32_t* quads, int64_t n,
                               const int64_t* exclude_rows, int64_t n_exclude, rg_graph** out) {
  return tgraph_create("rg_tgraph_create_excluding", n_ent, n_rela_rows, n_time, quads, n, exclude_rows, n_exclude, out);
}

int rg_graph_destroy(rg_graph* g) {
  if (!g) return 0;
  if (g->arena) (void)hipFree(g->arena);
  delete g;
  return 0;
}

int64_t rg_graph_n_fact(const rg_graph* g) { return g ? g->n_fact : -1; }

int rg_graph_export(const rg_graph* g, int32_t* out_ptr, int32_t* out_rt, int32_t* in_ptr, int32_t* in_hr) {
  RG_CHECK(g != nullptr, "rg_graph_export: graph is NULL");
  if (out_ptr) RG_HIP(hipMemcpy(out_ptr, g->out_ptr, (g->n_ent + 1) * sizeof(int32_t), hipMemcpyDeviceToHost));
  if (in_ptr) RG_HIP(hipMemcpy(in_ptr, g->in_ptr, (g->n_ent + 1) * sizeof(int32_t), hipMemcpyDeviceToHost));
  if (out_rt) RG_HIP(hipMemcpy(out_rt, g->out_rt, g->n_fact * sizeof(int2), hipMemcpyDeviceToHost));
  if (in_hr) RG_HIP(hipMemcpy(in_hr, g->in_hr, g->n_fact * sizeof(int2), hipMemcpyDeviceToHost));
  return 0;
}

int rg_graph_export_time(const rg_graph* g, int32_t* out_time, int32_t* in_time) {
  RG_CHECK(g != nullptr, "rg_graph_export_time: graph is NULL");
  RG_CHECK(g->n_time > 0 && g->in_time && g->out_time, "rg_graph_export_time: the graph has no timestamps (build it with rg_tgraph_create)");
  if (out_time) RG_HIP(hipMemcpy(out_time, g->out_time, g->n_fact * sizeof(int32_t), hipMemcpyDeviceToHost));
  if (in_time) RG_HIP(hipMemcpy(in_time, g->in_time, g->n_fact * sizeof(int32_t), hipMemcpyDeviceToHost));
  return 0;
}

int rg_hipgraph_fill_nodes(void* graph) {
  size_t n = 0;
  if (hipGraphGetNodes((hipGraph_t)graph, nullptr, &n) != hipSuccess) { rg::set_error("rg_hipgraph_fill_nodes: hipGraphGetNodes failed"); return -1; }
  std::vector<hipGraphNode_t> nodes(n);
  if (n && hipGraphGetNodes((hipGraph_t)graph, nodes.data(), &n) != hipSuccess) { rg::set_error("rg_hipgraph_fill_nodes: hipGraphGetNodes failed"); return -1; }
  int count = 0;
  for (size_t i = 0; i < n; ++i) {
    hipGraphNodeType t;
    if (hipGraphNodeGetType(nodes[i], &t) != hipSuccess) { rg::set_error("rg_hipgraph_fill_nodes: hipGraphNodeGetType failed"); return -1; }
    if (t == hipGraphNodeTypeMemset) ++count;
  }
  return count;
}

int rg_graph_export_packs(const rg_graph* g, int32_t* n_packs, int32_t* n_vrows, int32_t* ent, int32_t* pack, int32_t* rows, int32_t* vrows) {
  RG_CHECK(g != nullptr, "rg_graph_export_packs: graph is NULL");
  if (n_packs) *n_packs = g->in_pk_packs.n;
  if (n_vrows) *n_vrows = g->in_vr.n;
  if (ent && g->in_pk_packs.n) RG_HIP(hipMemcpy(ent, g->in_pk_packs.ent, (size_t)g->in_pk_packs.n * RG_PACK * sizeof(int2), hipMemcpyDeviceToHost));
  if (pack && g->in_pk_packs.n) RG_HIP(hipMemcpy(pack, g->in_pk_packs.pack, (size_t)g->in_pk_packs.n * sizeof(int4), hipMemcpyDeviceToHost));
  if (rows && g->in_pk_packs.n) RG_HIP(hipMemcpy(rows, g->in_pk_packs.rows, (size_t)g->in_vr.n * sizeof(int2), hipMemcpyDeviceToHost));
  if (vrows) RG_HIP(hipMemcpy(vrows, g->in_vr.rows, (size_t)g->in_vr.n * sizeof(int4), hipMemcpyDeviceToHost));
  return 0;
}

}
```

red-gnn_amd/csrc/graph_device.hip:

```cpp
#include <hipcub/hipcub.hpp>

#include <algorithm>
#include <vector>

#include "common.h"

namespace {

struct Tmp {
  std::vector<void*> ptrs;
  char* block = nullptr;
  size_t block_bytes = 0, used = 0;
  explicit Tmp(size_t bytes) {
    if (hipMalloc((void**)&block, bytes) == hipSuccess) block_bytes = bytes; else block = nullptr;
  }
  template <typename T>
  T* get(size_t n) {
    const size_t bytes = rg::align_up(std::max<size_t>(n, 1) * sizeof(T), 256);
    if (used + bytes <= block_bytes) { T* p = (T*)(block + used); used += bytes; return p; }
    void* p = nullptr;
    if (hipMalloc(&p, bytes) != hipSuccess) return nullptr;
    ptrs.push_back(p);
    return (T*)p;
  }
  ~Tmp() {
    for (void* p : ptrs) (void)hipFree(p);
    if (block) (void)hipFree(block);
  }
};

__global__ void rows_kernel(const int32_t* __restrict__ trip, int64_t n, int add_inverse, int n_ent, int n_rel, int max_rel,
                            int32_t* __restrict__ H, int32_t* __restrict__ R, int32_t* __restrict__ T, int64_t n_fact, int32_t* __restrict__ err) {
  const int64_t i = (int64_t)blockIdx.x * blockDim.x + threadIdx.x;
  if (i >= n_fact) return;
  const int64_t n_dir = add_inverse ? 2 * n : n;
  if (i < n_dir) {
    const int64_t j = i < n ? i : i - n;
    const int32_t h = trip[3 * j], r = trip[3 * j + 1], t = trip[3 * j + 2];
    if (h < 0 || h >= n_ent || t < 0 || t >= n_ent || r < 0 || r >= max_rel) { atomicMax(err, 1 + (int32_t)std::min<int64_t>(j, 0x7ffffffe)); H[i] = R[i] = T[i] = 0; return; }
    if (i < n) { H[i] = h; R[i] = r; T[i] = t; }
    else { H[i] = t; R[i] = r + n_rel; T[i] = h; }
  } else {
    const int32_t e = (int32_t)(i - n_dir);
    H[i] = e; R[i] = 2 * n_rel; T[i] = e;
  }
}

__global__ void iota_kernel(uint32_t* __restrict__ v, int64_t n) {
  const int64_t i = (int64_t)blockIdx.x * blockDim.x + threadIdx.x;
  if (i < n) v[i] = (uint32_t)i;
}

template <int MODE>
__global__ void keys_kernel(const int32_t* __restrict__ H, const int32_t* __restrict__ R, const int32_t* __restrict__ T, int rel_bits,
                            uint64_t* __restrict__ keys, int64_t n) {
  const int64_t i = (int64_t)blockIdx.x * blockDim.x + threadIdx.x;
  if (i >= n) return;
  keys[i] = MODE == 0 ? (uint64_t)T[i] : (MODE == 1 ? (((uint64_t)H[i] << rel_bits) | (uint64_t)R[i]) : (uint64_t)R[i]);
}

__global__ void hist_kernel(const int32_t* __restrict__ key, int64_t n, uint32_t* __restrict__ cnt) {
  const int64_t i = (int64_t)blockIdx.x * blockDim.x + threadIdx.x;
  if (i < n) atomicAdd(&cnt[key[i]], 1u);
}

__global__ void gather_pairs_kernel(const uint32_t* __restrict__ perm, const int32_t* __restrict__ A, const int32_t* __restrict__ B,
                                    int2* __restrict__ out, uint32_t* __restrict__ pk, int pk_mode, int64_t n) {
  const int64_t q = (int64_t)blockIdx.x * blockDim.x + threadIdx.x;
  if (q >= n) return;
  const uint32_t i = perm[q];
  const int2 v = make_int2(A[i], B[i]);
  out[q] = v;
  if (pk) pk[q] = pk_mode == 0 ? (((uint32_t)v.y << 20) | (uint32_t)v.x)
                               : (((uint32_t)v.x << 20) | (uint32_t)v.y);
}

__global__ void vrow_count_kernel(const int32_t* __restrict__ ptr, int n_rows, uint32_t* __restrict__ n_seg, uint32_t* __restrict__ is_split,
                                  uint32_t* __restrict__ split_seg) {
  const int e = blockIdx.x * blockDim.x + threadIdx.x;
  if (e >= n_rows) return;
  const int len = ptr[e + 1] - ptr[e];
  const int cut = len > RG_VROW_MAX;
  const int k = cut ? (len + RG_VROW_MAX - 1) / RG_VROW_MAX : 1;
  n_seg[e] = k; is_split[e] = cut; split_seg[e] = cut ? k : 0;
}

__global__ void vrow_emit_kernel(const int32_t* __restrict__ ptr, int n_rows, const int32_t* __restrict__ row_off, const int32_t* __restrict__ split_off,
                                 const int32_t* __restrict__ slot_off, int4* __restrict__ rows, uint32_t* __restrict__ keys, int4* __restrict__ split) {
  const int e = blockIdx.x * blockDim.x + threadIdx.x;
  if (e >= n_rows) return;
  const int beg = ptr[e], len = ptr[e + 1] - ptr[e];
  if (len <= RG_VROW_MAX) {
    rows[row_off[e]] = make_int4(e, beg, len, -1);
    keys[row_off[e]] = (uint32_t)(RG_VROW_MAX - len);
  } else {
    const int k = (len + RG_VROW_MAX - 1) / RG_VROW_MAX;
    split[split_off[e]] = make_int4(e, slot_off[e], k, 0);
    for (int j = 0; j < k; ++j) {
      const int b = beg + j * RG_VROW_MAX, l = min(RG_VROW_MAX, beg + len - b);
      rows[row_off[e] + j] = make_int4(e, b, l, slot_off[e] + j);
      keys[row_off[e] + j] = (uint32_t)(RG_VROW_MAX - l);
    }
  }
}

__global__ void gather_rows_kernel(const uint32_t* __restrict__ perm, const int4* __restrict__ in, int4* __restrict__ out, int n) {
  const int i = blockIdx.x * blockDim.x + threadIdx.x;
  if (i < n) out[i] = in[perm[i]];
}

__global__ void pack_emit_kernel(const int4* __restrict__ vrows, const int4* __restrict__ place, int n_vrows, const int32_t* __restrict__ pack_row0,
// ... 65 lines not shown
  uint32_t* is_split = tmp.get<uint32_t>(n_rows + 1);
  uint32_t* split_seg = tmp.get<uint32_t>(n_rows + 1);
  int32_t* row_off = tmp.get<int32_t>(n_rows + 1);
  int32_t* split_off = tmp.get<int32_t>(n_rows + 1);
  int32_t* slot_off = tmp.get<int32_t>(n_rows + 1);
  int32_t* scr = tmp.get<int32_t>(rg::scan_scratch_elems(n_rows + 1));
  out->cap_rows = (int)(n_rows + n_fact / RG_VROW_MAX + 2);
  out->cap_split = (int)(n_fact / (RG_VROW_MAX + 1) + 2);
  int4* rows_u = tmp.get<int4>(out->cap_rows);
  uint32_t* keys = tmp.get<uint32_t>(out->cap_rows);
  uint32_t* keys_o = tmp.get<uint32_t>(out->cap_rows);
  uint32_t* iota = tmp.get<uint32_t>(out->cap_rows);
  uint32_t* perm = tmp.get<uint32_t>(out->cap_rows);
  out->rows = tmp.get<int4>(out->cap_rows);
  out->split = tmp.get<int4>(out->cap_split);
  out->counts = tmp.get<int32_t>(4);
  if (!n_seg || !is_split || !split_seg || !row_off || !split_off || !slot_off || !scr || !rows_u || !keys || !keys_o || !iota || !perm ||
      !out->rows || !out->split || !out->counts) { rg::set_error("rg_graph_create_device: out of device memory"); return 1; }
  hipLaunchKernelGGL(vrow_count_kernel, dim3(blocks(n_rows)), dim3(256), 0, s, ptr, n_rows, n_seg, is_split, split_seg);
  if (rg::scan_exclusive(n_seg, row_off, n_rows, false, &out->counts[0], scr, s)) return 1;
  if (rg::scan_exclusive(is_split, split_off, n_rows, false, &out->counts[1], scr, s)) return 1;
  if (rg::scan_exclusive(split_seg, slot_off, n_rows, false, &out->counts[2], scr, s)) return 1;
  hipLaunchKernelGGL(vrow_emit_kernel, dim3(blocks(n_rows)), dim3(256), 0, s, ptr, n_rows, row_off, split_off, slot_off, rows_u, keys, out->split);
  int32_t n_v = 0;
  DEV_HIP(hipMemcpyAsync(&n_v, &out->counts[0], 4, hipMemcpyDeviceToHost, s));
  DEV_HIP(hipStreamSynchronize(s));
  hipLaunchKernelGGL(iota_kernel, dim3(blocks(n_v)), dim3(256), 0, s, iota, (int64_t)n_v);
  size_t bytes = 0;
  DEV_HIP(hipcub::DeviceRadixSort::SortPairs(nullptr, bytes, keys, keys_o, iota, perm, n_v, 0, 8, s));
  char* scratch = tmp.get<char>(bytes);
  if (!scratch) { rg::set_error("rg_graph_create_device: out of device memory"); return 1; }
  DEV_HIP(hipcub::DeviceRadixSort::SortPairs(scratch, bytes, keys, keys_o, iota, perm, n_v, 0, 8, s));
  hipLaunchKernelGGL(gather_rows_kernel, dim3(blocks(n_v)), dim3(256), 0, s, perm, rows_u, out->rows, n_v);
  RG_LAUNCH_CHECK();
  return 0;
}

}

extern "C" int rg_graph_create_device(int32_t n_ent, int32_t n_rel, const int32_t* triples_dev, int64_t n, int add_inverse, void* stream,
                                      rg_graph** out) {
  RG_CHECK(out != nullptr, "rg_graph_create_device: out is NULL");
  *out = nullptr;
  RG_CHECK(n_ent > 0 && n_rel > 0, "rg_graph_create_device: n_ent=%d n_rel=%d must be positive", n_ent, n_rel);
  RG_CHECK(n >= 0 && (n == 0 || triples_dev != nullptr), "rg_graph_create_device: bad triples (n=%lld)", (long long)n);
  const int64_t n_fact = (add_inverse ? 2 * n : n) + n_ent;
  RG_CHECK(n_fact < (int64_t)1 << 31, "rg_graph_create_device: %lld fact rows do not fit int32", (long long)n_fact);
  hipStream_t s = (hipStream_t)stream;
  const int n_rela_rows = 2 * n_rel + 1;
  const int max_rel = add_inverse ? n_rel : 2 * n_rel;
  int rel_bits = 1, ent_bits = 1;
  while ((1 << rel_bits) < n_rela_rows) ++rel_bits;
  while (((int64_t)1 << ent_bits) < n_ent) ++ent_bits;
  Tmp tmp((size_t)n_fact * 160 + (size_t)n_ent * 96 + ((size_t)8 << 20));
  int32_t* H = tmp.get<int32_t>(n_fact); int32_t* R = tmp.get<int32_t>(n_fact); int32_t* T = tmp.get<int32_t>(n_fact);
  uint64_t* keys = tmp.get<uint64_t>(n_fact);
  uint32_t* perm_in = tmp.get<uint32_t>(n_fact); uint32_t* perm_out = tmp.get<uint32_t>(n_fact); uint32_t* perm_rel = tmp.get<uint32_t>(n_fact);
  int32_t* flags = tmp.get<int32_t>(16);
  int32_t* out_ptr = tmp.get<int32_t>(n_ent + 2); int32_t* in_ptr = tmp.get<int32_t>(n_ent + 2); int32_t* rel_ptr = tmp.get<int32_t>(n_rela_rows + 2);
  int2* out_rt = tmp.get<int2>(n_fact); int2* in_hr = tmp.get<int2>(n_fact); int2* rel_ht = tmp.get<int2>(n_fact);
  const bool packed = n_ent <= (1 << 20) && n_rela_rows <= (1 << 12);
  uint32_t* in_pk = packed ? tmp.get<uint32_t>(n_fact) : nullptr; uint32_t* out_pk = packed ? tmp.get<uint32_t>(n_fact) : nullptr;
  RG_CHECK(H && R && T && keys && perm_in && perm_out && perm_rel && flags && out_ptr && in_ptr && rel_ptr && out_rt && in_hr && rel_ht &&
           (!packed || (in_pk && out_pk)), "rg_graph_create_device: out of device memory");
  DEV_HIP(hipMemsetAsync(flags, 0, 64, s));
  hipLaunchKernelGGL(rows_kernel, dim3(blocks(n_fact)), dim3(256), 0, s, triples_dev, n, add_inverse, n_ent, n_rel, max_rel, H, R, T, n_fact, flags);
  hipLaunchKernelGGL(keys_kernel<0>, dim3(blocks(n_fact)), dim3(256), 0, s, H, R, T, rel_bits, keys, n_fact);
  if (sort_perm(tmp, keys, ent_bits, n_fact, perm_in, s)) return 1;
  hipLaunchKernelGGL(keys_kernel<1>, dim3(blocks(n_fact)), dim3(256), 0, s, H, R, T, rel_bits, keys, n_fact);
  if (sort_perm(tmp, keys, ent_bits + rel_bits, n_fact, perm_out, s)) return 1;
  hipLaunchKernelGGL(keys_kernel<2>, dim3(blocks(n_fact)), dim3(256), 0, s, H, R, T, rel_bits, keys, n_fact);
  if (sort_perm(tmp, keys, rel_bits, n_fact, perm_rel, s)) return 1;
  hipLaunchKernelGGL(gather_pairs_kernel, dim3(blocks(n_fact)), dim3(256), 0, s, perm_in, H, R, in_hr, in_pk, 0, n_fact);
  hipLaunchKernelGGL(gather_pairs_kernel, dim3(blocks(n_fact)), dim3(256), 0, s, perm_out, R, T, out_rt, out_pk, 1, n_fact);
  hipLaunchKernelGGL(gather_pairs_kernel, dim3(blocks(n_fact)), dim3(256), 0, s, perm_rel, H, T, rel_ht, (uint32_t*)nullptr, 0, n_fact);
  if (build_ptr(tmp, T, n_fact, n_ent, in_ptr, s) || build_ptr(tmp, H, n_fact, n_ent, out_ptr, s) || build_ptr(tmp, R, n_fact, n_rela_rows, rel_ptr, s)) return 1;
  hipLaunchKernelGGL(max_kernel, dim3(blocks(n_ent)), dim3(256), 0, s, in_ptr, n_ent, &flags[1]);
  hipLaunchKernelGGL(max_kernel, dim3(blocks(n_ent)), dim3(256), 0, s, out_ptr, n_ent, &flags[2]);
  VrowsDev vin, vout, vrel;
  if (build_vrows(tmp, in_ptr, n_ent, n_fact, &vin, s) || build_vrows(tmp, out_ptr, n_ent, n_fact, &vout, s) ||
      build_vrows(tmp, rel_ptr, n_rela_rows, n_fact, &vrel, s)) return 1;
  int32_t host[16];
  DEV_HIP(hipMemcpyAsync(host, vin.counts, 12, hipMemcpyDeviceToHost, s));
  DEV_HIP(hipMemcpyAsync(host + 4, vout.counts, 12, hipMemcpyDeviceToHost, s));
  DEV_HIP(hipMemcpyAsync(host + 8, vrel.counts, 12, hipMemcpyDeviceToHost, s));
  DEV_HIP(hipMemcpyAsync(host + 12, flags, 16, hipMemcpyDeviceToHost, s));
  DEV_HIP(hipStreamSynchronize(s));
  RG_CHECK(host[12] == 0, "rg_graph_create_device: triple %d out of range", host[12] - 1);
  const bool want_packs = packed && n_rela_rows < (1 << 12);
  int4* place = nullptr; int32_t* pack_nrows = nullptr; int32_t* pack_row0 = nullptr;
  int n_packs = 0;
  if (want_packs) {
    const int nv = host[0];
    place = tmp.get<int4>(nv);
    pack_nrows = tmp.get<int32_t>(nv + 1);
    pack_row0 = tmp.get<int32_t>(nv + 1);
    int32_t* scr = tmp.get<int32_t>(rg::scan_scratch_elems(nv + 1));
    RG_CHECK(place && pack_nrows && pack_row0 && scr, "rg_graph_create_device: out of device memory");
    std::vector<int4> vrows_h(nv), place_h;
    std::vector<int32_t> nrows_h;
    DEV_HIP(hipMemcpyAsync(vrows_h.data(), vin.rows, (size_t)nv * sizeof(int4), hipMemcpyDeviceToHost, s));
    DEV_HIP(hipStreamSynchronize(s));
    n_packs = rg::place_rows_best_fit(vrows_h.data(), nv, &place_h, &nrows_h);
    DEV_HIP(hipMemcpyAsync(place, place_h.data(), (size_t)nv * sizeof(int4), hipMemcpyHostToDevice, s));
    if (n_packs) DEV_HIP(hipMemcpyAsync(pack_nrows, nrows_h.data(), (size_t)n_packs * sizeof(int32_t), hipMemcpyHostToDevice, s));
    DEV_HIP(hipStreamSynchronize(s));
    if (rg::scan_exclusive((const uint32_t*)pack_nrows, pack_row0, n_packs, false, nullptr, scr, s)) return 1;
  }
  rg_graph* g = new rg_graph();
  g->n_ent = n_ent; g->n_rel = n_rel; g->n_rela_rows = n_rela_rows; g->n_time = 0; g->n_fact = n_fact;
  g->max_in_deg = host[13]; g->max_out_deg = host[14];
  g->in_vr.n = host[0]; g->in_vr.n_split = host[1]; g->in_vr.n_slots = host[2];
  g->out_vr.n = host[4]; g->out_vr.n_split = host[5]; g->out_vr.n_slots = host[6];
  g->rel_vr.n = host[8]; g->rel_vr.n_split = host[9]; g->rel_vr.n_slots = host[10];
  g->in_pk_packs.n = n_packs;
  struct Item { void** field; const void* src; size_t bytes, off; };
  std::vector<Item> items;
  size_t total = 0;
  auto add = [&](void** field, const void* src, size_t bytes) {
    items.push_back({field, src, bytes, total});
    total += rg::align_up(std::max<size_t>(bytes, 16), 256);
  };
  add((void**)&g->out_ptr, out_ptr, (size_t)(n_ent + 1) * 4); add((void**)&g->in_ptr, in_ptr, (size_t)(n_ent + 1) * 4);
  add((void**)&g->out_rt, out_rt, (size_t)n_fact * 8); add((void**)&g->in_hr, in_hr, (size_t)n_fact * 8);
  if (packed) { add((void**)&g->in_pk, in_pk, (size_t)n_fact * 4); add((void**)&g->out_pk, out_pk, (size_t)n_fact * 4); }
  add((void**)&g->rel_ptr, rel_ptr, (size_t)(n_rela_rows + 1) * 4); add((void**)&g->rel_ht, rel_ht, (size_t)n_fact * 8);
  add((void**)&g->in_vr.rows, vin.rows, (size_t)g->in_vr.n * 16); add((void**)&g->in_vr.split, vin.split, (size_t)g->in_vr.n_split * 16);
  add((void**)&g->out_vr.rows, vout.rows, (size_t)g->out_vr.n * 16); add((void**)&g->out_vr.split, vout.split, (size_t)g->out_vr.n_split * 16);
  add((void**)&g->rel_vr.rows, vrel.rows, (size_t)g->rel_vr.n * 16); add((void**)&g->rel_vr.split, vrel.split, (size_t)g->rel_vr.n_split * 16);
  const size_t ent_off = total;
  if (n_packs > 0) {
    add((void**)&g->in_pk_packs.ent, nullptr, (size_t)n_packs * RG_PACK * 8);
    add((void**)&g->in_pk_packs.pack, nullptr, (size_t)n_packs * 16);
    add((void**)&g->in_pk_packs.rows, nullptr, (size_t)g->in_vr.n * 8);
  }
  hipError_t e = hipMalloc(&g->arena, total);
  if (e != hipSuccess) {
    rg::set_error("rg_graph_create_device: allocating %zu B failed: %s", total, hipGetErrorString(e));
    delete g;
    return 1;
  }
  for (const Item& it : items) {
    *it.field = (char*)g->arena + it.off;
    if (it.src && it.bytes) (void)hipMemcpyAsync(*it.field, it.src, it.bytes, hipMemcpyDeviceToDevice, s);
  }
  (void)ent_off;
  if (n_packs > 0) {
    hipLaunchKernelGGL(fill_int2_kernel, dim3(blocks((int64_t)n_packs * RG_PACK)), dim3(256), 0, s, g->in_pk_packs.ent, (int64_t)n_packs * RG_PACK,
                       make_int2(-1, 0));
    hipLaunchKernelGGL(pack_emit_kernel, dim3(g->in_vr.n), dim3(64), 0, s, g->in_vr.rows, place, g->in_vr.n, pack_row0, g->in_pk, g->in_pk_packs.ent,
                       g->in_pk_packs.pack, g->in_pk_packs.rows);
    hipLaunchKernelGGL(pack_count_kernel, dim3(blocks(n_packs)), dim3(256), 0, s, pack_nrows, g->in_pk_packs.pack, n_packs);
  }
  e = hipStreamSynchronize(s);
  if (e == hipSuccess) e = hipGetLastError();
  if (e != hipSuccess) {
    rg::set_error("rg_graph_create_device: build failed: %s", hipGetErrorString(e));
    rg_graph_destroy(g);
    return 1;
  }
  *out = g;
  return 0;
}
```

red-gnn_amd/csrc/layer_fwd.hip:

```cpp
#include "layer_fwd_kernel.h"
#include "layer_fwd_wp.h"

extern "C" size_t rg_layer_fwd_scratch_bytes(const rg_frontier* f, const rg_graph* g, int32_t ld) {
  if (!f || !g) return 0;
  return rg::align_up((size_t)f->B * g->in_vr.n_slots * ld * sizeof(float), 256) + rg::align_up((size_t)f->B * g->in_vr.n_slots, 256) + 256;
}

static int plan_walk(const rg_frontier* f, const rg_graph* g, int32_t level, int64_t n_old, int64_t n_new, int64_t n_edges, int32_t ld) {
  if (g->in_pk_packs.n == 0 || level != f->level || n_old < 0 || n_new <= 0 || n_edges < 0 || !rgwp::offsets_fit(n_old, ld)) return 1;
  const double candidates = (double)n_new * (double)g->n_fact / (double)g->n_ent;
  const bool tiny = n_new * 16 < (int64_t)f->B * f->n_ent;
  const bool short_rows = (double)g->n_fact < 12.0 * (double)g->n_ent;
  if (!tiny && !short_rows && (double)n_edges >= 0.4 * candidates) return 1;
  const double group_bytes = (double)n_old * ld * sizeof(float) / f->BW;
  int code = group_bytes <= 3.0 * (1 << 20) ? 2 : (group_bytes <= 6.0 * (1 << 20) ? 3 : 4);
  auto items = [&](int c) { return (int64_t)f->BW * (1 << (c - 2)) * g->in_pk_packs.n; };
  while (code < 5 && items(code) < 16384 && n_edges > 256 * items(code)) ++code;
  return code;
}

extern "C" int rg_layer_fwd_plan(const rg_frontier* f, const rg_graph* g, int32_t level, int64_t n_old, int64_t n_new,
                                 int64_t n_edges, int32_t ld) {
  if (!f || !g) return 1;
  return plan_walk(f, g, level, n_old, n_new, n_edges, ld);
}

extern "C" int rg_layer_fwd(const rg_frontier* f, const rg_graph* g, int32_t level, int64_t n_new, const float* hidden,
                            const float* rela, int32_t d, int32_t ld, const float* a_s, const float* a_r,
                            const float* a_q, int32_t ap, const float* w_alpha, const float* b_alpha, int32_t attn_dim,
                            float* agg_out, void* scratch, size_t scratch_bytes, int32_t walk, void* stream) {
  RG_CHECK(f && g && hidden && rela && a_s && a_r && a_q && w_alpha && b_alpha && agg_out, "rg_layer_fwd: NULL argument");
  RG_CHECK((((uintptr_t)hidden | (uintptr_t)rela | (uintptr_t)a_s | (uintptr_t)a_r | (uintptr_t)a_q | (uintptr_t)agg_out |
             (uintptr_t)scratch) & 15) == 0, "rg_layer_fwd: float buffers must be 16-B aligned");
  RG_CHECK(walk >= 0 && walk <= 7, "rg_layer_fwd: walk=%d not in 0..7", walk);
  rgfwd::FwdArgs A;
  if (rgfwd::fill_common("rg_layer_fwd", f, g, level, n_new, d, ld, ap, attn_dim, scratch, scratch_bytes,
                         rg_layer_fwd_scratch_bytes(f, g, ld), &A)) return 1;
  if (n_new == 0) return 0;
  A.hidden = (const float4*)hidden; A.rela = (const float4*)rela;
  A.a_s = (const float4*)a_s; A.a_r = (const float4*)a_r; A.a_q = (const float4*)a_q;
  A.w_alpha = w_alpha; A.b_alpha = b_alpha;
  A.agg = (float4*)agg_out; A.partial = (float4*)scratch;
  hipStream_t s = (hipStream_t)stream;
  if (walk == 0)
    walk = plan_walk(f, g, level, f->n_nodes[(level - 1) % f->n_levels], f->n_nodes[level % f->n_levels],
                     level == f->level ? f->n_edges : -1, ld);
  if (walk >= 2 && f->n_nodes[(level - 1) % f->n_levels] < 0 && !rgwp::offsets_fit((int64_t)f->B * f->n_ent, ld))
    walk = 1;
  if (walk >= 2) {
    RG_CHECK(g->in_pk_packs.n > 0, "rg_layer_fwd: the word-parallel walk needs a static graph with packed entries");
    RG_CHECK(level == f->level, "rg_layer_fwd: the word-parallel walk reads the entity-major bitmaps of the newest hop only "
             "(level %d, newest %d)", level, f->level);
    const int64_t n_old = f->n_nodes[(level - 1) % f->n_levels] >= 0 ? f->n_nodes[(level - 1) % f->n_levels] : (int64_t)f->B * f->n_ent;
    RG_CHECK(rgwp::offsets_fit(n_old, ld), "rg_layer_fwd: the word-parallel walk addresses the previous level by 32-bit byte offsets "
             "(%lld rows x %d floats is 4 GiB or more)", (long long)n_old, ld);
    rgwp::WpArgs W;
    W.n_sub = 1 << (walk - 2);
    W.n_packs = g->in_pk_packs.n; W.BW = f->BW; W.W = f->W; W.n_slots = g->in_vr.n_slots;
    W.n_items = (int64_t)f->BW * W.n_sub * W.n_packs;
    W.ent = g->in_pk_packs.ent; W.pack = g->in_pk_packs.pack; W.rows = g->in_pk_packs.rows;
    W.bits_old = f->bitsT[f->tcur ^ 1]; W.bits_new = f->bitsT[f->tcur];
    W.bm_old = A.bm_old; W.bm_new = A.bm_new;
    W.hidden = A.hidden; W.rela = A.rela; W.ld4 = A.ld4; W.a_s = A.a_s; W.a_r = A.a_r; W.a_q = A.a_q;
    W.w_alpha = w_alpha; W.b_alpha = b_alpha; W.attn_dim = attn_dim; W.n_rela_rows = g->n_rela_rows;
    W.agg = A.agg; W.partial = A.partial; W.queues = f->queues; W.queues_clean = A.walk.queues_clean;
    const int64_t n_e = level == f->level ? (f->n_edges >= 0 ? f->n_edges : f->edge_hint) : -1;
    const int64_t by_work = n_e < 0 ? 2 : 200 * W.n_items / std::max<int64_t>(n_e, 1);
    W.ipt = (int32_t)std::max<int64_t>(std::min<int64_t>(std::min<int64_t>(by_work, W.n_items / 8192), 32), 1);
    const size_t n_part = (size_t)f->B * g->in_vr.n_slots;
    W.written = n_part ? (uint8_t*)scratch + rg::align_up(n_part * ld * sizeof(float), 256) : nullptr;
    if (n_part && rg::zero_async(W.written, rg::align_up(n_part, 256), s)) return 1;
    if (rgwp::launch(W, ap / 4, s)) return 1;
    return rgfwd::launch_combine(A, f->B, g->in_vr, s, W.written);
  }
  const bool dense = n_new * 4 >= (int64_t)f->B * f->n_ent;
  return rgfwd::dispatch<false>(A, ld / 4, ap / 4, f->B, g->in_vr, dense, rg::walk_kpg(g->n_fact, g->in_vr.n), s);
}
```

red-gnn_amd/engine.py:

```python
import ctypes as C

import numpy as np
import torch

from . import _lib


FORCE_WALK = 0

KERNEL_EVENTS = None
DENSE_EVENTS = None
BWD_EVENTS = None
EXPLAIN_EVENTS = None
PROFILE_EVENTS = None


def _require_gpu(device):
    device = torch.device(device)
    if device.type != "cuda":
        raise _lib.NativeError("red_gnn_amd runs on an MI355X (device 'cuda'); got device %r. "
                               "There is no CPU path in the product — the CPU restatement lives in oracle/ for tests only."
                               % (device,))
    if not torch.cuda.is_available():
        raise _lib.NativeError("red_gnn_amd needs an MI355X: no ROCm device is visible to this process. The HIP path has "
# ... 7 lines not shown
def _next_serial():
    _GRAPH_SERIAL[0] += 1
    return _GRAPH_SERIAL[0]


class Graph:

    def __init__(self, n_ent, n_rel, triples, add_inverse=True, device="cuda"):
        self.serial = _next_serial()
        self.device = _require_gpu(device)
        trip = np.ascontiguousarray(np.asarray(triples, dtype=np.int32).reshape(-1, 3))
        self.n_ent, self.n_rel = int(n_ent), int(n_rel)
        h = C.c_void_p()
        with torch.cuda.device(self.device):
            _lib.check(_lib.lib().rg_graph_create(self.n_ent, self.n_rel, _lib.ptr(trip), len(trip),
                                                  1 if add_inverse else 0, C.byref(h)))
        self.handle = h
        self.n_fact = int(_lib.lib().rg_graph_n_fact(h))

    @classmethod
    def from_device(cls, n_ent, n_rel, triples_dev, add_inverse=True):
        self = cls.__new__(cls)
        self.serial = _next_serial()
        self.device = _require_gpu(triples_dev.device)
        assert triples_dev.dtype == torch.int32 and triples_dev.dim() == 2 and triples_dev.shape[1] == 3
        trip = triples_dev.contiguous()
        self.n_ent, self.n_rel = int(n_ent), int(n_rel)
        h = C.c_void_p()
        with torch.cuda.device(self.device):
            _lib.check(_lib.lib().rg_graph_create_device(self.n_ent, self.n_rel, _lib.ptr(trip), trip.shape[0], 1 if add_inverse else 0,
                                                         _lib.stream_ptr(), C.byref(h)))
        self.handle = h
        self.n_fact = int(_lib.lib().rg_graph_n_fact(h))
        return self

    def export_packs(self):
        L = _lib.lib()
        n_packs, n_vrows = C.c_int32(), C.c_int32()
        _lib.check(L.rg_graph_export_packs(self.handle, C.byref(n_packs), C.byref(n_vrows), None, None, None, None))
        vr = np.empty((n_vrows.value, 4), np.int32)
        ent = np.empty((n_packs.value * 128, 2), np.int32)
        pack = np.empty((n_packs.value, 4), np.int32)
        rows = np.empty((n_vrows.value if n_packs.value else 0, 2), np.int32)
        _lib.check(L.rg_graph_export_packs(self.handle, None, None, _lib.ptr(ent), _lib.ptr(pack), _lib.ptr(rows), _lib.ptr(vr)))
        return vr, ent, pack, rows

    def export(self):
        op = np.empty(self.n_ent + 1, np.int32)
        ip = np.empty(self.n_ent + 1, np.int32)
        ort = np.empty((self.n_fact, 2), np.int32)
        ihr = np.empty((self.n_fact, 2), np.int32)
        _lib.check(_lib.lib().rg_graph_export(self.handle, _lib.ptr(op), _lib.ptr(ort), _lib.ptr(ip), _lib.ptr(ihr)))
        return op, ort, ip, ihr

    def close(self):
        if getattr(self, "handle", None) is not None and _lib._lib is not None:
            _lib.lib().rg_graph_destroy(self.handle)
        self.handle = None

    def __del__(self):
        try:
            self.close()
        except Exception:
            pass


class TemporalGraph(Graph):

    def __init__(self, n_ent, n_rela_rows, n_time, quads, device="cuda", exclude=None):
        self.serial = _next_serial()
        self.device = _require_gpu(device)
        q = quads if (isinstance(quads, np.ndarray) and quads.dtype == np.int32 and quads.flags.c_contiguous and quads.ndim == 2) \
            else np.ascontiguousarray(np.asarray(quads, dtype=np.int32).reshape(-1, 4))
        self.n_ent, self.n_rel, self.n_rela_rows, self.n_time = int(n_ent), 0, int(n_rela_rows), int(n_time)
        h = C.c_void_p()
        with torch.cuda.device(self.device):
            if exclude is None:
                _lib.check(_lib.lib().rg_tgraph_create(self.n_ent, self.n_rela_rows, self.n_time, _lib.ptr(q), len(q), C.byref(h)))
            else:
                ex = np.ascontiguousarray(np.asarray(exclude, dtype=np.int64).reshape(-1))
                _lib.check(_lib.lib().rg_tgraph_create_excluding(self.n_ent, self.n_rela_rows, self.n_time, _lib.ptr(q), len(q),
                                                                 _lib.ptr(ex), len(ex), C.byref(h)))
        self.handle = h
        self.n_fact = int(_lib.lib().rg_graph_n_fact(h))


    def export_time(self):
        ot = np.empty(self.n_fact, np.int32)
        it = np.empty(self.n_fact, np.int32)
        _lib.check(_lib.lib().rg_graph_export_time(self.handle, _lib.ptr(ot), _lib.ptr(it)))
        return ot, it


class Frontier:

    def __init__(self, n_ent, batch, n_levels=2, device="cuda"):
        self.device = _require_gpu(device)
        L = _lib.lib()
        self.n_ent, self.batch, self.n_levels = int(n_ent), int(batch), int(n_levels)
        nbytes = L.rg_frontier_workspace_bytes(self.n_ent, self.batch, self.n_levels)
        if nbytes == 0:
            raise _lib.NativeError("bad frontier shape n_ent=%d batch=%d n_levels=%d" % (n_ent, batch, n_levels))
        self.workspace = torch.empty(nbytes + 256, dtype=torch.uint8, device=self.device)
        base = self.workspace.data_ptr()
        aligned = (base + 255) // 256 * 256
        h = C.c_void_p()
# ... 266 lines not shown
        ev[1].record()
        PROFILE_EVENTS.append((ev[0], ev[1], level))


def tattn_profile(frontier, graph, level, q_time, a_s, a_r, a_q, w_alpha, b_alpha, attn_dim, sum_out, count_out):
    for t in (a_s, a_r, a_q, w_alpha, b_alpha):
        assert t.is_cuda and t.dtype == torch.float32 and t.is_contiguous()
    ap = a_s.shape[1]
    assert a_r.shape == (graph.n_rela_rows, ap) and a_q.shape == (frontier.batch, ap)
    assert q_time.is_cuda and q_time.dtype == torch.int32 and q_time.is_contiguous() and q_time.numel() == frontier.batch
    for t in (sum_out, count_out):
        assert t.is_cuda and t.dtype == torch.int64 and t.is_contiguous() and t.shape == (frontier.batch, 3, a_r.shape[0])
    ev = None
    if PROFILE_EVENTS is not None:
        ev = (torch.cuda.Event(enable_timing=True), torch.cuda.Event(enable_timing=True))
        ev[0].record()
    _lib.check(_lib.lib().rg_tattn_profile(frontier.handle, graph.handle, frontier.batch, frontier.n_ent, level, a_s.shape[0],
                                           _lib.ptr(q_time), _lib.ptr(a_s), _lib.ptr(a_r), _lib.ptr(a_q), ap, _lib.ptr(w_alpha),
                                           _lib.ptr(b_alpha), attn_dim, _lib.ptr(sum_out), _lib.ptr(count_out), _lib.stream_ptr()))
    if ev is not None:
        ev[1].record()
        PROFILE_EVENTS.append((ev[0], ev[1], level))


def xattn_profile(frontier, graph, level, q_time, loop_time, row_time, lag_bin, n_bins, a_s, a_r, a_q, w_alpha, b_alpha, attn_dim, sum_out,
                  count_out):
    for t in (a_s, a_r, a_q, w_alpha, b_alpha):
        assert t.is_cuda and t.dtype == torch.float32 and t.is_contiguous()
    ap = a_s.shape[1]
    assert a_r.shape == (graph.n_rela_rows, ap) and a_q.shape == (frontier.batch, ap)
    for t in (q_time, loop_time, row_time):
        assert t.is_cuda and t.dtype == torch.int32 and t.is_contiguous()
    assert q_time.numel() == frontier.batch and loop_time.numel() == frontier.batch
    assert lag_bin.is_cuda and lag_bin.dtype == torch.uint8 and lag_bin.is_contiguous() and lag_bin.dim() == 1 and lag_bin.numel() >= 1
    for t in (sum_out, count_out):
        assert t.is_cuda and t.dtype == torch.int64 and t.is_contiguous() and t.shape == (frontier.batch, n_bins, a_r.shape[0])
    ev = None
    if PROFILE_EVENTS is not None:
        ev = (torch.cuda.Event(enable_timing=True), torch.cuda.Event(enable_timing=True))
        ev[0].record()
    _lib.check(_lib.lib().rg_xattn_profile(frontier.handle, graph.handle, frontier.batch, frontier.n_ent, level, a_s.shape[0],
                                           _lib.ptr(q_time), _lib.ptr(loop_time), _lib.ptr(row_time), _lib.ptr(lag_bin), lag_bin.numel(),
                                           int(n_bins), _lib.ptr(a_s), _lib.ptr(a_r), _lib.ptr(a_q), ap, _lib.ptr(w_alpha),
                                           _lib.ptr(b_alpha), attn_dim, _lib.ptr(sum_out), _lib.ptr(count_out), _lib.stream_ptr()))
    if ev is not None:
        ev[1].record()
        PROFILE_EVENTS.append((ev[0], ev[1], level))


def layer_fwd_plan(frontier, graph, level, n_old, n_new, n_edges, ld):
    return int(_lib.lib().rg_layer_fwd_plan(frontier.handle, graph.handle, level, n_old, n_new, n_edges, ld))


def layer_fwd_scratch_bytes(frontier, graph, ld):
    return _lib.lib().rg_layer_fwd_scratch_bytes(frontier.handle, graph.handle, ld)


def layer_fwd_into(frontier, graph, level, n_hint, hidden, rela, d, a_s, a_r, a_q, w_alpha, b_alpha, attn_dim, agg, scratch, walk=1):
    ld, ap = hidden.shape[1], a_s.shape[1]
    _lib.check(_lib.lib().rg_layer_fwd(frontier.handle, graph.handle, level, max(int(n_hint), 1),
                                       _lib.ptr(hidden), _lib.ptr(rela), d, ld, _lib.ptr(a_s), _lib.ptr(a_r),
                                       _lib.ptr(a_q), ap, _lib.ptr(w_alpha), _lib.ptr(b_alpha), attn_dim,
                                       _lib.ptr(agg), _lib.ptr(scratch), scratch.numel(), FORCE_WALK or max(int(walk), 1), _lib.stream_ptr()))


def tlayer_fwd(frontier, graph, level, n_new, q_time, hidden_dir, rela_dir, time_dir, d, a_s, a_r, a_q, w_alpha, b_alpha, attn_dim):
    ld, ap = hidden_dir.shape[1], a_s.shape[1]
    for t in (hidden_dir, rela_dir, time_dir, a_s, a_r, a_q, w_alpha, b_alpha):
        assert t.is_cuda and t.dtype == torch.float32 and t.is_contiguous()
    assert q_time.dtype == torch.int32 and q_time.is_cuda
    agg = torch.empty((n_new, ld), dtype=torch.float32, device=hidden_dir.device)
    nbytes = _lib.lib().rg_layer_fwd_scratch_bytes(frontier.handle, graph.handle, ld)
    scratch = frontier.scratch(nbytes)
    ev = None
    if KERNEL_EVENTS is not None:
        ev = (torch.cuda.Event(enable_timing=True), torch.cuda.Event(enable_timing=True))
        ev[0].record()
    _lib.check(_lib.lib().rg_tlayer_fwd(frontier.handle, graph.handle, level, n_new, _lib.ptr(q_time), _lib.ptr(hidden_dir),
                                        _lib.ptr(rela_dir), _lib.ptr(time_dir), d, ld, _lib.ptr(a_s), _lib.ptr(a_r), _lib.ptr(a_q),
                                        ap, _lib.ptr(w_alpha), _lib.ptr(b_alpha), attn_dim, _lib.ptr(agg), _lib.ptr(scratch),
                                        nbytes, _lib.stream_ptr()))
    if ev is not None:
        ev[1].record()
        KERNEL_EVENTS.append((ev[0], ev[1], frontier.n_edges, n_new))
    return agg


def xlayer_fwd(frontier, graph, level, n_new, q_time, loop_time, row_time, n_data, hidden_p, rela_p, time_p, d, a_s, a_r, a_q, w_alpha, b_alpha, attn_dim):
    ld, ap = hidden_p.shape[1], a_s.shape[1]
    for t in (hidden_p, rela_p, time_p, a_s, a_r, a_q, w_alpha, b_alpha):
        assert t.is_cuda and t.dtype == torch.float32 and t.is_contiguous()
    for t in (q_time, loop_time, row_time):
        assert t.dtype == torch.int32 and t.is_cuda and t.is_contiguous()
    agg = torch.empty((n_new, ld), dtype=torch.float32, device=hidden_p.device)
    nbytes = _lib.lib().rg_layer_fwd_scratch_bytes(frontier.handle, graph.handle, ld)
    scratch = frontier.scratch(nbytes)
    ev = None
    if KERNEL_EVENTS is not None:
        ev = (torch.cuda.Event(enable_timing=True), torch.cuda.Event(enable_timing=True))
        ev[0].record()
    _lib.check(_lib.lib().rg_xlayer_fwd(frontier.handle, graph.handle, level, n_new, _lib.ptr(q_time), _lib.ptr(loop_time), _lib.ptr(row_time),
                                        int(n_data), _lib.ptr(hidden_p), _lib.ptr(rela_p), _lib.ptr(time_p), time_p.shape[0], d, ld,
                                        _lib.ptr(a_s), _lib.ptr(a_r), _lib.ptr(a_q), ap, _lib.ptr(w_alpha), _lib.ptr(b_alpha), attn_dim,
                                        _lib.ptr(agg), _lib.ptr(scratch), nbytes, _lib.stream_ptr()))
    if ev is not None:
        ev[1].record()
# ... 84 lines not shown
    n_rows, m, n = g.shape[0], g.shape[1], x.shape[1]
    L = _lib.lib()
    out = torch.empty((m, n), dtype=torch.float32, device=g.device)
    cs = torch.empty(m, dtype=torch.float32, device=g.device) if colsum else None
    for m0 in range(0, m, 192):
        mc = min(192, m - m0)
        for n0 in range(0, n, 64):
            nc = min(64, n - n0)
            nbytes = L.rg_gram_tn_scratch_bytes(mc, nc)
            key = (str(g.device), torch.cuda.current_stream(g.device).cuda_stream)
            scratch = _GRAM_SCRATCH.get(key)
            if scratch is None or scratch.numel() < nbytes:
                scratch = _GRAM_SCRATCH[key] = torch.empty(nbytes, dtype=torch.uint8, device=g.device)
            tile = out if (mc == m and nc == n) else torch.empty((mc, nc), dtype=torch.float32, device=g.device)
            cs_t = None
            if colsum and n0 == 0:
                cs_t = cs if mc == m else torch.empty(mc, dtype=torch.float32, device=g.device)
            gv, xv = g[:, m0:m0 + mc], x[:, n0:n0 + nc]
            _lib.check(L.rg_gram_tn(C.c_void_p(gv.data_ptr()), g.stride(0), mc, C.c_void_p(xv.data_ptr()), x.stride(0), nc, n_rows,
                                    _lib.ptr(tile), _lib.ptr(cs_t), _lib.ptr(scratch), scratch.numel(), _lib.stream_ptr()))
            if tile is not out:
                out[m0:m0 + mc, n0:n0 + nc] = tile
            if cs_t is not None and cs_t is not cs:
                cs[m0:m0 + mc] = cs_t
    return (out, cs) if colsum else out


_BLAS_CHOICE = [None]


def prefer_blas(n_rows):
    choice = "cublas" if n_rows < (1 << 17) else "cublaslt"
    if _BLAS_CHOICE[0] != choice:
        import warnings
        with warnings.catch_warnings():
            warnings.simplefilter("ignore")
            torch.backends.cuda.preferred_blas_library(choice)
        _BLAS_CHOICE[0] = choice


def dense_supported(d, attn_dim):
    return bool(_lib.lib().rg_dense_fwd_supported(d, attn_dim))


DENSE_PRECISIONS = {"f32": 0, "f16x2": 1, "f16x3": 2}


def dense_scratch(d, precision, device):
    nbytes = int(_lib.lib().rg_dense_scratch_bytes(d, DENSE_PRECISIONS[precision]))
    return torch.empty(nbytes, dtype=torch.uint8, device=device) if nbytes else None


def dense_fwd(agg, hidden_prev, prev_idx, d, W_h, act, gate, Ws_next=None, attn_dim=0, ap=0, W_final=None, nodes=None,
              n_ent=0, scores_all=None, precision="f32"):
    n, ld = agg.shape
    hidden = torch.empty_like(agg)
    a_s = torch.empty((n, ap), dtype=torch.float32, device=agg.device) if Ws_next is not None else None
    c = lambda t: None if t is None else t.detach().contiguous()
    W_h, w_ih, w_hh, b_ih, b_hh = c(W_h), c(gate.weight_ih_l0), c(gate.weight_hh_l0), c(gate.bias_ih_l0), c(gate.bias_hh_l0)
    Ws_next, W_final = c(Ws_next), c(W_final)
    scratch = dense_scratch(d, precision, agg.device)
    ev = None
    if DENSE_EVENTS is not None:
        ev = (torch.cuda.Event(enable_timing=True), torch.cuda.Event(enable_timing=True))
        ev[0].record()
    _lib.check(_lib.lib().rg_dense_fwd(n, d, ld, _lib.ptr(agg), _lib.ptr(hidden_prev), _lib.ptr(prev_idx), _lib.ptr(W_h),
                                       {"idd": 0, "relu": 1, "tanh": 2}[act], _lib.ptr(w_ih), _lib.ptr(w_hh), _lib.ptr(b_ih),
                                       _lib.ptr(b_hh), _lib.ptr(Ws_next), attn_dim, ap, _lib.ptr(a_s), _lib.ptr(W_final),
                                       _lib.ptr(nodes), n_ent, _lib.ptr(scores_all), _lib.ptr(hidden), DENSE_PRECISIONS[precision],
                                       _lib.ptr(scratch), 0 if scratch is None else scratch.numel(), _lib.stream_ptr()))
    if ev is not None:
        ev[1].record()
        DENSE_EVENTS.append((ev[0], ev[1], n))
    return hidden, a_s


def dense_fwd_dev(n_cap, count_ptr, agg, hidden_prev, prev_idx, d, W_h, act, gate, hidden_out, Ws_next=None, attn_dim=0, ap=0,
                  a_s_out=None, W_final=None, nodes=None, n_ent=0, scores_all=None, n_hint=0, precision="f32", scratch=None):
    ld = agg.shape[1]
    c = lambda t: None if t is None else t.detach().contiguous()
    W_h, w_ih, w_hh, b_ih, b_hh = c(W_h), c(gate.weight_ih_l0), c(gate.weight_hh_l0), c(gate.bias_ih_l0), c(gate.bias_hh_l0)
    Ws_next, W_final = c(Ws_next), c(W_final)
    if scratch is None:
        scratch = dense_scratch(d, precision, agg.device)
    _lib.check(_lib.lib().rg_dense_fwd_dev(n_cap, count_ptr, int(n_hint), d, ld, _lib.ptr(agg), _lib.ptr(hidden_prev), _lib.ptr(prev_idx),
                                           _lib.ptr(W_h), {"idd": 0, "relu": 1, "tanh": 2}[act], _lib.ptr(w_ih), _lib.ptr(w_hh),
                                           _lib.ptr(b_ih), _lib.ptr(b_hh), _lib.ptr(Ws_next), attn_dim, ap, _lib.ptr(a_s_out),
                                           _lib.ptr(W_final), _lib.ptr(nodes), n_ent, _lib.ptr(scores_all), _lib.ptr(hidden_out),
                                           DENSE_PRECISIONS[precision], _lib.ptr(scratch), 0 if scratch is None else scratch.numel(),
                                           _lib.stream_ptr()))


def dense_train_supported(d, act):
    return ((16 <= d <= 64 and d % 4 == 0) or d == 128) and act in ("idd", "relu", "tanh")


def dense_train_fwd(agg, hidden_prev, prev_idx, W_h, act, gate, mask=None, Ws_next=None):
    n, d = agg.shape
    dev = agg.device
    hidden = torch.empty((n, d), dtype=torch.float32, device=dev)
    x = torch.empty((n, d), dtype=torch.float32, device=dev)
    ws = torch.empty((n, 5 * d), dtype=torch.float32, device=dev)
    c = lambda t: None if t is None else t.detach().contiguous()
    common = (n, d, _lib.ptr(c(agg)), _lib.ptr(c(hidden_prev)), _lib.ptr(prev_idx), _lib.ptr(c(W_h)),
              {"idd": 0, "relu": 1, "tanh": 2}[act], _lib.ptr(c(gate.weight_ih_l0)), _lib.ptr(c(gate.weight_hh_l0)),
              _lib.ptr(c(gate.bias_ih_l0)), _lib.ptr(c(gate.bias_hh_l0)), _lib.ptr(c(mask)))
    if Ws_next is None:
        _lib.check(_lib.lib().rg_dense_train_fwd(*common, _lib.ptr(hidden), _lib.ptr(x), _lib.ptr(ws), _lib.stream_ptr()))
        return hidden, x, ws, None
# ... 212 lines not shown
```

red-gnn_amd/models.py:

```python
import os

import numpy as np
import torch
import torch.nn as nn
import torch.nn.functional as F

import ctypes

from . import _lib as _lib_mod
from . import engine


def _pad4(n):
    return (n + 3) // 4 * 4


def pad_attn(a):
    if a > 32:
        raise ValueError("attn_dim=%d: the HIP layer kernels cover attention widths up to 32" % a)
    return _pad4(a) if a <= 16 else 32


_FUSED_BWD_ROWS = 1 << 13
_TALL_ROWS = 1 << 15
# ... 189 lines not shown
        self.model, self.graph, self.n, self.hints = model, graph, n, hints
        d, a = model.hidden_dim, model.attn_dim
        self.ld, self.ap = max(16, _pad4(d)), pad_attn(a)
        n_ent = graph.n_ent
        cap = self.cap = n * n_ent
        f32 = dict(dtype=torch.float32, device=device)
        self.q_sub = torch.zeros(n, dtype=torch.int32, device=device)
        self.q_rel = torch.zeros(n, dtype=torch.int64, device=device)
        self.fr = engine.Frontier(n_ent, n, 2, device)
        self.nodes = torch.empty((cap, 2), dtype=torch.int32, device=device)
        self.prev = torch.empty(cap, dtype=torch.int32, device=device)
        self.agg = torch.empty((cap, self.ld), **f32)
        self.hid = [torch.empty((cap, self.ld), **f32) for _ in range(2)]
        self.a_s = [torch.empty((cap, self.ap), **f32) for _ in range(2)]
        self.scores = torch.empty(cap, **f32)
        nbytes = engine.layer_fwd_scratch_bytes(self.fr, graph, self.ld)
        self.scratch = torch.empty(max(nbytes, 256), dtype=torch.uint8, device=device)
        self.dense_scratch = engine.dense_scratch(d, model.dense_precision, device)
        self.key_ptr = model.W_final.weight.data_ptr()
        side = torch.cuda.Stream(device=device)
        side.wait_stream(torch.cuda.current_stream(device))
        with torch.cuda.stream(side), torch.no_grad():
            self._enqueue()
        torch.cuda.current_stream(device).wait_stream(side)
        self.cuda_graph = None
        if os.environ.get("RG_NO_CAPTURE") != "1":
            self.cuda_graph = torch.cuda.CUDAGraph(keep_graph=True)
            with torch.cuda.graph(self.cuda_graph), torch.no_grad():
                self._enqueue()
            n_fill = _lib_mod.lib().rg_hipgraph_fill_nodes(ctypes.c_void_p(self.cuda_graph.raw_cuda_graph()))
            if n_fill != 0:
                raise RuntimeError("captured forward holds %d memset nodes (expected none)" % n_fill)
            self.cuda_graph.instantiate()

    @staticmethod
    def bytes_needed(n, n_ent, ld, ap):
        return n * n_ent * (4 * (3 * ld + 2 * ap + 1) + 12)

    def _enqueue(self):
        m, fr, graph, n = self.model, self.fr, self.graph, self.n
        d, a, ld, ap = m.hidden_dim, m.attn_dim, self.ld, self.ap
        fr.reset(self.q_sub)
        hidden, a_s = self.hid[1], self.a_s[1]
        torch._foreach_zero_([hidden[:n], a_s[:n], self.scores])
        tables = m.inference_tables(self.q_rel, ld, ap)
        for i in range(m.n_layer):
            layer = m.gnn_layers[i]
            n_hint, walk, e_hint = (tuple(self.hints[i]) + (None,))[:3]
            fr.expand_nodes_async(graph, self.nodes, self.prev, edge_hint=e_hint)
            a_r, a_q, rela_p = tables[i]
            engine.layer_fwd_into(fr, graph, fr.level, n_hint, hidden, rela_p, d, a_s, a_r, a_q,
                                  layer.w_alpha.weight.reshape(-1).contiguous(), layer.w_alpha.bias, a, self.agg, self.scratch, walk=walk)
            last = i + 1 == m.n_layer
            out_h, out_a = self.hid[i % 2], self.a_s[i % 2]
            engine.dense_fwd_dev(self.cap, fr.count_ptr(), self.agg, hidden, self.prev, d, layer.W_h.weight, m.act_name, m.gate, out_h,
                                 Ws_next=None if last else m.gnn_layers[i + 1].Ws_attn.weight, attn_dim=a, ap=ap,
                                 a_s_out=None if last else out_a, W_final=m.W_final.weight if last else None,
                                 nodes=self.nodes, n_ent=graph.n_ent, scores_all=self.scores, n_hint=n_hint, precision=m.dense_precision,
                                 scratch=self.dense_scratch)
            hidden, a_s = out_h, out_a

    def run(self, q_sub, q_rel):
        self.q_sub.copy_(q_sub, non_blocking=True)
        self.q_rel.copy_(q_rel, non_blocking=True)
        if self.cuda_graph is not None:
            self.cuda_graph.replay()
        else:
            self._enqueue()
        return self.scores.view(self.n, self.graph.n_ent).clone()

    def stats(self):
        counts = self.fr.level_counts()
        return dict(n_edges=[e for (_, e) in counts[1:]], n_nodes=counts[-1][0])


class RED_GNN_trans(nn.Module):
    def __init__(self, params, loader):
        super().__init__()
        self.n_layer, self.hidden_dim, self.attn_dim, self.n_rel = params.n_layer, params.hidden_dim, params.attn_dim, params.n_rel
        self.loader = loader
        acts = {"relu": nn.ReLU(), "tanh": torch.tanh, "idd": lambda x: x}
        act = acts[params.act]
        self.act_name = params.act
        self.gnn_layers = nn.ModuleList(
            [GNNLayer(self.hidden_dim, self.hidden_dim, self.attn_dim, self.n_rel, act=act) for _ in range(self.n_layer)])
        self.dropout = nn.Dropout(params.dropout)
        self.W_final = nn.Linear(self.hidden_dim, 1, bias=False)
        self.gate = nn.GRU(self.hidden_dim, self.hidden_dim)
        self._frontiers = engine.FrontierPool()
        self._last_stats = None
        self.fused_dense = True
        self.dense_precision = "f16x3"
        self.use_graphs = True
        self._graphed, self._seen, self._hints, self._pending_key, self._graph_failed = {}, {}, {}, None, set()

    @property
    def last_stats(self):
        if callable(self._last_stats):
            self._last_stats = self._last_stats()
        return self._last_stats

    @last_stats.setter
    def last_stats(self, value):
        self._last_stats = value

    def _frontier(self, n_ent, batch, n_levels, device):
        return self._frontiers.get(n_ent, batch, n_levels, device)
# ... 119 lines not shown
            ld, ap = max(16, _pad4(self.hidden_dim)), pad_attn(self.attn_dim)
            seen = self._seen.get(key, 0)
            self._seen[key] = seen + 1
            budget = _GraphedInference.budget(device)
            if seen < 2 or _GraphedInference.bytes_needed(n, graph.n_ent, ld, ap) > budget:
                self._pending_key = key
                return None
            hints = self._hints.get(key) or [(n * graph.n_ent, 1, None)] * self.n_layer
            if key in self._graph_failed:
                return None
            need = _GraphedInference.bytes_needed(n, graph.n_ent, ld, ap)
            held = sum(_GraphedInference.bytes_needed(v.n, v.graph.n_ent, v.ld, v.ap) for v in self._graphed.values())
            if len(self._graphed) >= 80 or held + need > 2 * budget:
                self.release_replay_buffers()
            try:
                g = self._graphed[key] = _GraphedInference(self, graph, n, device, hints)
            except Exception as exc:
                import warnings
                warnings.warn("RED_GNN_trans: HIP graph capture failed for batch size %d (%s: %s); this shape stays on the eager "
                              "path" % (n, type(exc).__name__, exc))
                self._graph_failed.add(key)
                torch.cuda.synchronize(device)
                return None
        scores = g.run(q_sub, q_rel)
        self._last_stats = g.stats
        return scores

    def replay_bytes_held(self):
        return sum(_GraphedInference.bytes_needed(v.n, v.graph.n_ent, v.ld, v.ap) for v in self._graphed.values())

    def release_replay_buffers(self):
        if self._graphed:
            torch.cuda.synchronize()
        self._graphed.clear()
        self._seen.clear()
        self._hints.clear()
        self._graph_failed.clear()
        self._pending_key = None

    def _forward_inference(self, fr, graph, q_sub, q_rel, n, device, trace, kept=None):
        d, a = self.hidden_dim, self.attn_dim
        ld, ap = max(16, _pad4(d)), pad_attn(a)
        n_ent = graph.n_ent
        hidden = torch.zeros((n, ld), device=device)
        a_s = torch.zeros((n, ap), device=device)
        scores_all = torch.zeros(n * n_ent, device=device)
        n_edges, sizes = [], []
        nodes = None
        tables = self.inference_tables(q_rel, ld, ap)
        for i in range(self.n_layer):
            n_new, n_e, n_old = fr.expand(graph)
            nodes, prev_idx, old_new = fr.nodes(want_prev=True, want_old_new=trace is not None)
            n_edges.append(n_e)
            sizes.append((n_new, engine.layer_fwd_plan(fr, graph, fr.level, n_old, n_new, n_e, ld), n_e))
            layer = self.gnn_layers[i]
            if kept is not None:
                kept.append(dict(a_s=a_s, tables=tables[i]))
            agg = layer.aggregate_nograd(tables[i], hidden, a_s, fr, graph, fr.level, nodes)
            last = i + 1 == self.n_layer
            hidden, a_s = engine.dense_fwd(
                agg, hidden, prev_idx, d, layer.W_h.weight, self.act_name, self.gate,
                Ws_next=None if last else self.gnn_layers[i + 1].Ws_attn.weight, attn_dim=a, ap=ap,
                W_final=self.W_final.weight if last else None, nodes=nodes, n_ent=n_ent, scores_all=scores_all,
                precision=self.dense_precision)
            if trace is not None:
                trace.append(dict(nodes=nodes, old_nodes_new_idx=old_new, n_edges=n_e, hidden=hidden[:, :d]))
        self.last_stats = dict(n_edges=n_edges, n_nodes=int(nodes.shape[0]))
        if getattr(self, "_pending_key", None) is not None:
            if len(self._hints) > 16:
                self._hints.clear()
            self._hints[self._pending_key] = sizes
            self._pending_key = None
        return scores_all.view(n, n_ent)


class RED_GNN_induc(RED_GNN_trans):

    def forward(self, subs, rels, mode="transductive", trace=None):
        return super().forward(subs, rels, mode=mode, trace=trace)

    def explain(self, subs, rels, objs=None, mode="transductive", min_alpha=0.0):
        return super().explain(subs, rels, objs=objs, mode=mode, min_alpha=min_alpha)

    def rules(self, subs, rels, objs=None, k=1, mode="transductive", min_alpha=0.0):
        return super().rules(subs, rels, objs=objs, k=k, mode=mode, min_alpha=min_alpha)

    def predict(self, subs, rels, k=10, exclude_known=True, mode="transductive"):
        return super().predict(subs, rels, k=k, exclude_known=exclude_known, mode=mode)

    def attention_profile(self, subs, rels, mode="transductive", group="relation"):
        return super().attention_profile(subs, rels, mode=mode, group=group)
```

Baseline: 30.37 billion edges/s.

## Add single-source first-layer kernel using tail-sorted out-lists and skip final hidden write

Adds a tail-ordered out-edge list per head to the graph, records each query's source entity in the frontier, and adds a specialized layer-forward kernel (walk mode 8) for the first layer. There every edge starts from the single query source, so it walks that source's out-list grouped by tail and aggregates messages directly without gathering the frontier edge list. The final layer's dense/GRU step also skips writing the hidden output when only scores are needed. The cost is extra graph memory, a larger build, and a new kernel path with chunk-boundary segment handling.

```diff
diff --git a/include/redgnn.h b/include/redgnn.h
--- a/include/redgnn.h
+++ b/include/redgnn.h
@@ -29,6 +29,7 @@
 int64_t rg_graph_n_fact(const rg_graph* g);
 int rg_graph_export(const rg_graph* g, int32_t* out_ptr_host, int32_t* out_rel_tail_host,
                     int32_t* in_ptr_host, int32_t* in_head_rel_host);
+int rg_graph_export_out_by_tail(const rg_graph* g, int32_t* rel_tail_host, int32_t* pos_host, uint32_t* packed_host);
 int rg_graph_export_time(const rg_graph* g, int32_t* out_time_host, int32_t* in_time_host);
 
 size_t rg_frontier_workspace_bytes(int32_t n_ent, int32_t batch, int32_t n_levels);
@@ -53,6 +54,7 @@
 size_t rg_layer_fwd_scratch_bytes(const rg_frontier* f, const rg_graph* g, int32_t ld);
 int rg_layer_fwd_plan(const rg_frontier* f, const rg_graph* g, int32_t level, int64_t n_old, int64_t n_new,
                       int64_t n_edges, int32_t ld);
+int rg_layer_fwd_single_source(const rg_frontier* f, const rg_graph* g, int32_t level);
 int rg_layer_fwd(const rg_frontier* f, const rg_graph* g, int32_t level, int64_t n_new,
                  const float* hidden, const float* rela, int32_t d, int32_t ld,
                  const float* a_s, const float* a_r, const float* a_q, int32_t ap,
diff --git a/red-gnn_amd/_lib.py b/red-gnn_amd/_lib.py
--- a/red-gnn_amd/_lib.py
+++ b/red-gnn_amd/_lib.py
@@ -6,10 +6,10 @@
 
 SYMBOLS = [
     "rg_last_error", "rg_version", "rg_hipgraph_fill_nodes",
-    "rg_graph_create", "rg_graph_create_device", "rg_graph_export_packs", "rg_tgraph_create", "rg_tgraph_create_excluding", "rg_graph_destroy", "rg_graph_n_fact", "rg_graph_export",
+    "rg_graph_create", "rg_graph_create_device", "rg_graph_export_packs", "rg_tgraph_create", "rg_tgraph_create_excluding", "rg_graph_destroy", "rg_graph_n_fact", "rg_graph_export", "rg_graph_export_out_by_tail",
     "rg_frontier_workspace_bytes", "rg_frontier_create", "rg_frontier_destroy", "rg_frontier_reset",
     "rg_frontier_reset_nodes", "rg_frontier_expand", "rg_frontier_nodes", "rg_frontier_edges_scratch_bytes", "rg_frontier_edges",
-    "rg_layer_fwd_scratch_bytes", "rg_layer_fwd", "rg_layer_fwd_plan", "rg_tlayer_fwd", "rg_xlayer_fwd", "rg_frontier_set_window", "rg_layer_bwd_scratch_bytes", "rg_layer_bwd", "rg_tlayer_bwd_scratch_bytes", "rg_tlayer_bwd", "rg_xlayer_bwd", "rg_dense_fwd_supported", "rg_dense_scratch_bytes", "rg_dense_fwd", "rg_dense_fwd_dev", "rg_dense_train_fwd", "rg_dense_train_fwd_as", "rg_rows_addmm", "rg_dense_train_bwd", "rg_dense_train_bwd2", "rg_split3_roundtrip", "rg_split3_product_check", "rg_gram_tn_scratch_bytes", "rg_gram_tn", "rg_rank",
+    "rg_layer_fwd_scratch_bytes", "rg_layer_fwd", "rg_layer_fwd_plan", "rg_layer_fwd_single_source", "rg_tlayer_fwd", "rg_xlayer_fwd", "rg_frontier_set_window", "rg_layer_bwd_scratch_bytes", "rg_layer_bwd", "rg_tlayer_bwd_scratch_bytes", "rg_tlayer_bwd", "rg_xlayer_bwd", "rg_dense_fwd_supported", "rg_dense_scratch_bytes", "rg_dense_fwd", "rg_dense_fwd_dev", "rg_dense_train_fwd", "rg_dense_train_fwd_as", "rg_rows_addmm", "rg_dense_train_bwd", "rg_dense_train_bwd2", "rg_split3_roundtrip", "rg_split3_product_check", "rg_gram_tn_scratch_bytes", "rg_gram_tn", "rg_rank",
     "rg_frontier_expand_async", "rg_frontier_expand_nodes_async", "rg_frontier_set_edge_hint", "rg_frontier_count_ptr", "rg_frontier_level_counts", "rg_attn_tables",
     "rg_explain_scratch_bytes", "rg_explain_seed", "rg_explain_count", "rg_explain_emit", "rg_explain_gather",
     "rg_topk",
@@ -52,6 +52,7 @@
     L.rg_graph_n_fact.argtypes = [vp]
     L.rg_graph_n_fact.restype = i64
     L.rg_graph_export.argtypes = [vp, vp, vp, vp, vp]
+    L.rg_graph_export_out_by_tail.argtypes = [vp, vp, vp, vp]
     L.rg_frontier_workspace_bytes.argtypes = [i32, i32, i32]
     L.rg_frontier_workspace_bytes.restype = sz
     L.rg_frontier_create.argtypes = [i32, i32, i32, vp, sz, C.POINTER(vp)]
@@ -74,6 +75,7 @@
     L.rg_layer_fwd_scratch_bytes.restype = sz
     L.rg_layer_fwd.argtypes = [vp, vp, i32, i64, vp, vp, i32, i32, vp, vp, vp, i32, vp, vp, i32, vp, vp, sz, i32, vp]
     L.rg_layer_fwd_plan.argtypes = [vp, vp, i32, i64, i64, i64, i32]
+    L.rg_layer_fwd_single_source.argtypes = [vp, vp, i32]
     L.rg_tlayer_fwd.argtypes = [vp, vp, i32, i64, vp, vp, vp, vp, i32, i32, vp, vp, vp, i32, vp, vp, i32, vp, vp, sz, vp]
     L.rg_xlayer_fwd.argtypes = [vp, vp, i32, i64, vp, vp, vp, i32, vp, vp, vp, i32, i32, i32, vp, vp, vp, i32, vp, vp, i32, vp, vp, sz, vp]
     L.rg_frontier_set_window.argtypes = [vp, vp, vp, i32]
diff --git a/red-gnn_amd/csrc/common.h b/red-gnn_amd/csrc/common.h
--- a/red-gnn_amd/csrc/common.h
+++ b/red-gnn_amd/csrc/common.h
@@ -121,6 +121,9 @@
   int2* in_hr = nullptr;
   uint32_t* in_pk = nullptr;
   uint32_t* out_pk = nullptr;
+  int2* out_bt_rt = nullptr;
+  uint32_t* out_bt_pk = nullptr;
+  int32_t* out_bt_pos = nullptr;
   rg_vrows in_vr, out_vr;
   rg_packs in_pk_packs;
   int32_t* rel_ptr = nullptr;
@@ -154,6 +157,8 @@
   int tcur = 0;
   int64_t n_nodes[RG_MAX_LEVELS] = {};
   int64_t n_edges = 0;
+  bool single_source = false;
+  int32_t* sub = nullptr;
   int64_t edge_hint = -1;
   const int2* bm_of(int lvl) const { return bm[lvl % n_levels]; }
 };
diff --git a/red-gnn_amd/csrc/dense.hip b/red-gnn_amd/csrc/dense.hip
--- a/red-gnn_amd/csrc/dense.hip
+++ b/red-gnn_amd/csrc/dense.hip
@@ -262,7 +262,7 @@
 #pragma unroll
     for (int it = 0; it < 16 * S / 64; ++it) {
       const int e = it * 64 + lane, r = e / S, sl = e - r * S;
-      if (row0 + r < A.n && sl < A.ld4) A.hidden_out[(row0 + r) * A.ld4 + sl] = tile[sw<DP>(r, sl)];
+      if (A.hidden_out && row0 + r < A.n && sl < A.ld4) A.hidden_out[(row0 + r) * A.ld4 + sl] = tile[sw<DP>(r, sl)];
     }
   }
 }
@@ -291,7 +291,8 @@
                           const float* b_ih, const float* b_hh, const float* Ws_next, int32_t attn_dim, int32_t ap,
                           float* a_s_out, const float* W_final, const int32_t* nodes, int32_t n_ent, float* scores_all,
                           float* hidden_out, int32_t precision, void* scratch, int64_t scratch_bytes, void* stream) {
-  RG_CHECK(agg && W_h && w_ih && w_hh && b_ih && b_hh && hidden_out, "rg_dense_fwd: NULL argument");
+  RG_CHECK(agg && W_h && w_ih && w_hh && b_ih && b_hh, "rg_dense_fwd: NULL argument");
+  RG_CHECK(hidden_out || (W_final && !Ws_next), "rg_dense_fwd: hidden_out is NULL (allowed only with W_final and without Ws_next)");
   RG_CHECK(precision >= 0 && precision <= 2, "rg_dense_fwd: precision=%d (0 = f32 MFMA, 1 = two-term f16 split, 2 = exact three-term f16 split)",
            precision);
   RG_CHECK(!prev_idx || hidden_prev, "rg_dense_fwd: prev_idx given without hidden_prev");
diff --git a/red-gnn_amd/csrc/dense128.hip b/red-gnn_amd/csrc/dense128.hip
--- a/red-gnn_amd/csrc/dense128.hip
+++ b/red-gnn_amd/csrc/dense128.hip
@@ -257,7 +257,7 @@
 #pragma unroll
     for (int it = 0; it < NL; ++it) {
       const int e = it * 64 + lane, r = e / S, sl = e - r * S;
-      if (row0 + r < A.n) A.hidden_out[(row0 + r) * S + sl] = tile[swz(r, sl)];
+      if (A.hidden_out && row0 + r < A.n) A.hidden_out[(row0 + r) * S + sl] = tile[swz(r, sl)];
     }
   }
 }
diff --git a/red-gnn_amd/csrc/dense128_split.hip b/red-gnn_amd/csrc/dense128_split.hip
--- a/red-gnn_amd/csrc/dense128_split.hip
+++ b/red-gnn_amd/csrc/dense128_split.hip
@@ -247,7 +247,7 @@
         const float ng = fmaf(2.0f, __builtin_amdgcn_rcpf(1.0f + __builtin_amdgcn_exp2f(fmaf(rg, th, ti))), -1.0f);
         hnv[r] = fmaf(zg, hov[r] - ng, ng);
       }
-      if (node_ok) (A.hidden_out + row0 * S)[lane_off + 4 * ob] = make_float4(hnv[0], hnv[1], hnv[2], hnv[3]);
+      if (A.hidden_out && node_ok) (A.hidden_out + row0 * S)[lane_off + 4 * ob] = make_float4(hnv[0], hnv[1], hnv[2], hnv[3]);
       h4 ch, cl;
       split4(hnv[0], hnv[1], hnv[2], hnv[3], ch, cl);
       if (ob & 1) {
diff --git a/red-gnn_amd/csrc/dense128_split3.hip b/red-gnn_amd/csrc/dense128_split3.hip
--- a/red-gnn_amd/csrc/dense128_split3.hip
+++ b/red-gnn_amd/csrc/dense128_split3.hip
@@ -294,8 +294,9 @@
     const float inv_s = inv * inv_w * -LOG2E, inv_t = inv * inv_w * (-2.0f * LOG2E);
     float hn[KS];
     const int rows_valid = (int)(A.n - row0 < 16 ? (A.n - row0 > 0 ? A.n - row0 : 0) : 16);
-    const __amdgpu_buffer_rsrc_t r_out = __builtin_amdgcn_make_buffer_rsrc(reinterpret_cast<char*>(A.hidden_out + row0 * S), 0,
-                                                                            rows_valid * S * 16, 0x00020000);
+    const __amdgpu_buffer_rsrc_t r_out = __builtin_amdgcn_make_buffer_rsrc(
+        A.hidden_out ? reinterpret_cast<char*>(A.hidden_out + row0 * S) : reinterpret_cast<char*>(const_cast<float4*>(A.agg)), 0,
+        A.hidden_out ? rows_valid * S * 16 : 0, 0x00020000);
     auto gate_loop = [&](auto HH_) {
       constexpr bool HH = decltype(HH_)::value;
       f32x4 P[2][4][3];
diff --git a/red-gnn_amd/csrc/dense_split.hip b/red-gnn_amd/csrc/dense_split.hip
--- a/red-gnn_amd/csrc/dense_split.hip
+++ b/red-gnn_amd/csrc/dense_split.hip
@@ -246,7 +246,7 @@
           const float ng = fmaf(2.0f, __builtin_amdgcn_rcpf(1.0f + __builtin_amdgcn_exp2f(fmaf(rg, th, ti))), -1.0f);
           hnv[r] = fmaf(zg, hov[r] - ng, ng);
         }
-        if (node_ok && ((col_ok >> ob) & 1u))
+        if (A.hidden_out && node_ok && ((col_ok >> ob) & 1u))
           (A.hidden_out + row0 * A.ld4)[lane_off + 4 * ob] = make_float4(hnv[0], hnv[1], hnv[2], hnv[3]);
         h4 ch, cl;
         split4(hnv[0], hnv[1], hnv[2], hnv[3], ch, cl);
diff --git a/red-gnn_amd/csrc/dense_split3.hip b/red-gnn_amd/csrc/dense_split3.hip
--- a/red-gnn_amd/csrc/dense_split3.hip
+++ b/red-gnn_amd/csrc/dense_split3.hip
@@ -256,7 +256,8 @@
     float hn[KS];
     const int rows_valid = (int)(A.n - row0 < 16 ? (A.n - row0 > 0 ? A.n - row0 : 0) : 16);
     const __amdgpu_buffer_rsrc_t r_out = __builtin_amdgcn_make_buffer_rsrc(
-        reinterpret_cast<char*>(A.hidden_out + row0 * A.ld4), 0, rows_valid * A.ld4 * 16, 0x00020000);
+        A.hidden_out ? reinterpret_cast<char*>(A.hidden_out + row0 * A.ld4) : reinterpret_cast<char*>(const_cast<float4*>(A.agg)), 0,
+        A.hidden_out ? rows_valid * A.ld4 * 16 : 0, 0x00020000);
     auto gru = [&](auto has_old) {
       constexpr bool OLD = decltype(has_old)::value;
       Frag<KST> H;
diff --git a/red-gnn_amd/csrc/frontier.hip b/red-gnn_amd/csrc/frontier.hip
--- a/red-gnn_amd/csrc/frontier.hip
+++ b/red-gnn_amd/csrc/frontier.hip
@@ -5,7 +5,7 @@
 namespace {
 
 __global__ void reset_level0_kernel(const int32_t* __restrict__ q_sub, int B, int n_ent, int BW, int W, uint32_t* __restrict__ bitsT,
-                                    int2* __restrict__ bm0, int32_t* __restrict__ counters) {
+                                    int2* __restrict__ bm0, int32_t* __restrict__ counters, int32_t* __restrict__ sub) {
   const int64_t i = (int64_t)blockIdx.x * blockDim.x + threadIdx.x;
   if (i >= (int64_t)B * W) return;
   const int b = (int)(i / W), w = (int)(i - (int64_t)b * W);
@@ -14,6 +14,7 @@
   const int ew = ok ? e >> 5 : W;
   bm0[i] = make_int2(w == ew ? (int)(1u << (e & 31)) : 0, b + (w > ew ? 1 : 0));
   if (w == 0) {
+    sub[b] = ok ? e : -1;
     if (ok) atomicOr(&bitsT[(int64_t)e * BW + (b >> 5)], 1u << (b & 31));
     else atomicOr((unsigned*)&counters[1], 1u);
     if (b == 0) { counters[0] = B; counters[4] = B; }
@@ -312,6 +313,7 @@
   off[4] = take(rg::scan_scratch_elems((int64_t)B * W) * 4);
   off[5] = take(1024 + RG_QUEUE_BYTES);
   off[6] = take((size_t)n_levels * B * W * 8);
+  off[7] = take((size_t)B * 4);
   return o;
 }
 
@@ -347,6 +349,7 @@
   f->counters = (int32_t*)(base + off[5]);
   f->queues = f->counters + 256;
   for (int l = 0; l < n_levels; ++l) f->bm[l] = (int2*)(base + off[6] + (size_t)l * batch * f->W * 8);
+  f->sub = (int32_t*)(base + off[7]);
   if (hipHostMalloc((void**)&f->counts_pinned, 1024, hipHostMallocDefault) != hipSuccess) {
     delete f;
     rg::set_error("rg_frontier_create: hipHostMalloc failed");
@@ -385,8 +388,9 @@
   f->queues_clean = false;
   const int64_t nw = (int64_t)f->B * f->W;
   hipLaunchKernelGGL(reset_level0_kernel, dim3(rg::ceil_div(nw, 256)), dim3(256), 0, s, q_sub, f->B, f->n_ent, f->BW, f->W,
-                     f->bitsT[0], f->bm[0], f->counters);
-  RG_LAUNCH_CHECK();
+                     f->bitsT[0], f->bm[0], f->counters, f->sub);
+  RG_LAUNCH_CHECK();
+  f->single_source = true;
   f->n_nodes[0] = f->B;
   return 0;
 }
@@ -411,6 +415,7 @@
   }
   if (build_level(f, s)) return 1;
   if (rg::copy_words_async(&f->counters[4], &f->counters[0], 1, s)) return 1;
+  f->single_source = false;
   f->n_nodes[0] = n;
   return 0;
 }
diff --git a/red-gnn_amd/csrc/graph.hip b/red-gnn_amd/csrc/graph.hip
--- a/red-gnn_amd/csrc/graph.hip
+++ b/red-gnn_amd/csrc/graph.hip
@@ -271,7 +271,7 @@
 extern "C" {
 
 const char* rg_last_error(void) { return rg::g_err.c_str(); }
-int rg_version(void) { return 10; }
+int rg_version(void) { return 11; }
 
 static int build_graph(int32_t n_ent, int32_t n_rel, int32_t n_rela_rows, const std::vector<int32_t>& H,
                        const std::vector<int32_t>& R, const std::vector<int32_t>& T, const std::vector<int32_t>* TIME,
@@ -323,6 +323,25 @@
       out_pk[i] = ((uint32_t)out_rt[i].x << 20) | (uint32_t)out_rt[i].y;
     }
     A.add(&g->in_pk, in_pk); A.add(&g->out_pk, out_pk);
+  }
+  std::vector<int2> out_bt_rt;
+  std::vector<uint32_t> out_bt_pk;
+  std::vector<int32_t> out_bt_pos;
+  if (!TIME) {
+    out_bt_rt.resize(n_fact); out_bt_pos.resize(n_fact);
+    std::vector<int32_t> po(out_ptr.begin(), out_ptr.end() - 1);
+    for (int32_t t = 0; t < n_ent; ++t)
+      for (int32_t q = in_ptr[t]; q < in_ptr[t + 1]; ++q) {
+        const int32_t j = po[in_hr[q].x]++;
+        out_bt_rt[j] = make_int2(in_hr[q].y, t);
+        out_bt_pos[j] = q;
+      }
+    A.add(&g->out_bt_rt, out_bt_rt); A.add(&g->out_bt_pos, out_bt_pos);
+    if (!in_pk.empty()) {
+      out_bt_pk.resize(n_fact);
+      for (int64_t j = 0; j < n_fact; ++j) out_bt_pk[j] = ((uint32_t)out_bt_rt[j].x << 20) | (uint32_t)out_bt_rt[j].y;
+      A.add(&g->out_bt_pk, out_bt_pk);
+    }
   }
   std::vector<int32_t> rel_ptr(n_rela_rows + 1, 0), rel_tm(TIME ? n_fact : 0);
   std::vector<int2> rel_ht(n_fact);
@@ -455,6 +474,16 @@
   return 0;
 }
 
+int rg_graph_export_out_by_tail(const rg_graph* g, int32_t* rel_tail, int32_t* pos, uint32_t* packed) {
+  RG_CHECK(g != nullptr, "rg_graph_export_out_by_tail: graph is NULL");
+  RG_CHECK(g->out_bt_rt && g->out_bt_pos, "rg_graph_export_out_by_tail: the graph has no out-list by tail (static graphs only)");
+  RG_CHECK(!packed || g->out_bt_pk, "rg_graph_export_out_by_tail: the graph's entries are not packed");
+  if (rel_tail) RG_HIP(hipMemcpy(rel_tail, g->out_bt_rt, g->n_fact * sizeof(int2), hipMemcpyDeviceToHost));
+  if (pos) RG_HIP(hipMemcpy(pos, g->out_bt_pos, g->n_fact * sizeof(int32_t), hipMemcpyDeviceToHost));
+  if (packed) RG_HIP(hipMemcpy(packed, g->out_bt_pk, g->n_fact * sizeof(uint32_t), hipMemcpyDeviceToHost));
+  return 0;
+}
+
 int rg_graph_export_time(const rg_graph* g, int32_t* out_time, int32_t* in_time) {
   RG_CHECK(g != nullptr, "rg_graph_export_time: graph is NULL");
   RG_CHECK(g->n_time > 0 && g->in_time && g->out_time, "rg_graph_export_time: the graph has no timestamps (build it with rg_tgraph_create)");
diff --git a/red-gnn_amd/csrc/graph_device.hip b/red-gnn_amd/csrc/graph_device.hip
--- a/red-gnn_amd/csrc/graph_device.hip
+++ b/red-gnn_amd/csrc/graph_device.hip
@@ -56,7 +56,17 @@
                             uint64_t* __restrict__ keys, int64_t n) {
   const int64_t i = (int64_t)blockIdx.x * blockDim.x + threadIdx.x;
   if (i >= n) return;
-  keys[i] = MODE == 0 ? (uint64_t)T[i] : (MODE == 1 ? (((uint64_t)H[i] << rel_bits) | (uint64_t)R[i]) : (uint64_t)R[i]);
+  keys[i] = MODE == 0 ? (uint64_t)T[i] : (MODE == 1 ? (((uint64_t)H[i] << rel_bits) | (uint64_t)R[i])
+                                       : (MODE == 2 ? (uint64_t)R[i] : (((uint64_t)H[i] << rel_bits) | (uint64_t)T[i])));
+}
+
+__global__ void invert_perm_kernel(const uint32_t* __restrict__ perm, int32_t* __restrict__ inv, int64_t n) {
+  const int64_t q = (int64_t)blockIdx.x * blockDim.x + threadIdx.x;
+  if (q < n) inv[perm[q]] = (int32_t)q;
+}
+__global__ void gather_words_kernel(const uint32_t* __restrict__ perm, const int32_t* __restrict__ in, int32_t* __restrict__ out, int64_t n) {
+  const int64_t j = (int64_t)blockIdx.x * blockDim.x + threadIdx.x;
+  if (j < n) out[j] = in[perm[j]];
 }
 
 __global__ void hist_kernel(const int32_t* __restrict__ key, int64_t n, uint32_t* __restrict__ cnt) {
@@ -228,7 +238,7 @@
   int rel_bits = 1, ent_bits = 1;
   while ((1 << rel_bits) < n_rela_rows) ++rel_bits;
   while (((int64_t)1 << ent_bits) < n_ent) ++ent_bits;
-  Tmp tmp((size_t)n_fact * 160 + (size_t)n_ent * 96 + ((size_t)8 << 20));
+  Tmp tmp((size_t)n_fact * 208 + (size_t)n_ent * 96 + ((size_t)8 << 20));
   int32_t* H = tmp.get<int32_t>(n_fact); int32_t* R = tmp.get<int32_t>(n_fact); int32_t* T = tmp.get<int32_t>(n_fact);
   uint64_t* keys = tmp.get<uint64_t>(n_fact);
   uint32_t* perm_in = tmp.get<uint32_t>(n_fact); uint32_t* perm_out = tmp.get<uint32_t>(n_fact); uint32_t* perm_rel = tmp.get<uint32_t>(n_fact);
@@ -250,6 +260,15 @@
   hipLaunchKernelGGL(gather_pairs_kernel, dim3(blocks(n_fact)), dim3(256), 0, s, perm_in, H, R, in_hr, in_pk, 0, n_fact);
   hipLaunchKernelGGL(gather_pairs_kernel, dim3(blocks(n_fact)), dim3(256), 0, s, perm_out, R, T, out_rt, out_pk, 1, n_fact);
   hipLaunchKernelGGL(gather_pairs_kernel, dim3(blocks(n_fact)), dim3(256), 0, s, perm_rel, H, T, rel_ht, (uint32_t*)nullptr, 0, n_fact);
+  uint32_t* perm_bt = tmp.get<uint32_t>(n_fact); int32_t* inv_in = tmp.get<int32_t>(n_fact);
+  int2* out_bt_rt = tmp.get<int2>(n_fact); int32_t* out_bt_pos = tmp.get<int32_t>(n_fact);
+  uint32_t* out_bt_pk = packed ? tmp.get<uint32_t>(n_fact) : nullptr;
+  RG_CHECK(perm_bt && inv_in && out_bt_rt && out_bt_pos && (!packed || out_bt_pk), "rg_graph_create_device: out of device memory");
+  hipLaunchKernelGGL(keys_kernel<3>, dim3(blocks(n_fact)), dim3(256), 0, s, H, R, T, ent_bits, keys, n_fact);
+  if (sort_perm(tmp, keys, 2 * ent_bits, n_fact, perm_bt, s)) return 1;
+  hipLaunchKernelGGL(invert_perm_kernel, dim3(blocks(n_fact)), dim3(256), 0, s, perm_in, inv_in, n_fact);
+  hipLaunchKernelGGL(gather_pairs_kernel, dim3(blocks(n_fact)), dim3(256), 0, s, perm_bt, R, T, out_bt_rt, out_bt_pk, 1, n_fact);
+  hipLaunchKernelGGL(gather_words_kernel, dim3(blocks(n_fact)), dim3(256), 0, s, perm_bt, inv_in, out_bt_pos, n_fact);
   if (build_ptr(tmp, T, n_fact, n_ent, in_ptr, s) || build_ptr(tmp, H, n_fact, n_ent, out_ptr, s) || build_ptr(tmp, R, n_fact, n_rela_rows, rel_ptr, s)) return 1;
   hipLaunchKernelGGL(max_kernel, dim3(blocks(n_ent)), dim3(256), 0, s, in_ptr, n_ent, &flags[1]);
   hipLaunchKernelGGL(max_kernel, dim3(blocks(n_ent)), dim3(256), 0, s, out_ptr, n_ent, &flags[2]);
@@ -300,6 +319,8 @@
   add((void**)&g->out_ptr, out_ptr, (size_t)(n_ent + 1) * 4); add((void**)&g->in_ptr, in_ptr, (size_t)(n_ent + 1) * 4);
   add((void**)&g->out_rt, out_rt, (size_t)n_fact * 8); add((void**)&g->in_hr, in_hr, (size_t)n_fact * 8);
   if (packed) { add((void**)&g->in_pk, in_pk, (size_t)n_fact * 4); add((void**)&g->out_pk, out_pk, (size_t)n_fact * 4); }
+  add((void**)&g->out_bt_rt, out_bt_rt, (size_t)n_fact * 8); add((void**)&g->out_bt_pos, out_bt_pos, (size_t)n_fact * 4);
+  if (packed) add((void**)&g->out_bt_pk, out_bt_pk, (size_t)n_fact * 4);
   add((void**)&g->rel_ptr, rel_ptr, (size_t)(n_rela_rows + 1) * 4); add((void**)&g->rel_ht, rel_ht, (size_t)n_fact * 8);
   add((void**)&g->in_vr.rows, vin.rows, (size_t)g->in_vr.n * 16); add((void**)&g->in_vr.split, vin.split, (size_t)g->in_vr.n_split * 16);
   add((void**)&g->out_vr.rows, vout.rows, (size_t)g->out_vr.n * 16); add((void**)&g->out_vr.split, vout.split, (size_t)g->out_vr.n_split * 16);
diff --git a/red-gnn_amd/csrc/layer_fwd.hip b/red-gnn_amd/csrc/layer_fwd.hip
--- a/red-gnn_amd/csrc/layer_fwd.hip
+++ b/red-gnn_amd/csrc/layer_fwd.hip
@@ -1,4 +1,5 @@
 #include "layer_fwd_kernel.h"
+#include "layer_fwd_src1.h"
 #include "layer_fwd_wp.h"
 
 extern "C" size_t rg_layer_fwd_scratch_bytes(const rg_frontier* f, const rg_graph* g, int32_t ld) {
@@ -6,7 +7,11 @@
   return rg::align_up((size_t)f->B * g->in_vr.n_slots * ld * sizeof(float), 256) + rg::align_up((size_t)f->B * g->in_vr.n_slots, 256) + 256;
 }
 
-static int plan_walk(const rg_frontier* f, const rg_graph* g, int32_t level, int64_t n_old, int64_t n_new, int64_t n_edges, int32_t ld) {
+static bool src1_applies(const rg_frontier* f, const rg_graph* g, int32_t level) {
+  return level == 1 && f->level >= 1 && f->single_source && f->sub && !f->win_lo && g->n_time == 0 && g->out_bt_pos && g->out_bt_rt;
+}
+
+static int plan_general(const rg_frontier* f, const rg_graph* g, int32_t level, int64_t n_old, int64_t n_new, int64_t n_edges, int32_t ld) {
   if (g->in_pk_packs.n == 0 || level != f->level || n_old < 0 || n_new <= 0 || n_edges < 0 || !rgwp::offsets_fit(n_old, ld)) return 1;
   const double candidates = (double)n_new * (double)g->n_fact / (double)g->n_ent;
   const bool tiny = n_new * 16 < (int64_t)f->B * f->n_ent;
@@ -19,10 +24,18 @@
   return code;
 }
 
+static int plan_walk(const rg_frontier* f, const rg_graph* g, int32_t level, int64_t n_old, int64_t n_new, int64_t n_edges, int32_t ld) {
+  return src1_applies(f, g, level) ? 8 : plan_general(f, g, level, n_old, n_new, n_edges, ld);
+}
+
+extern "C" int rg_layer_fwd_single_source(const rg_frontier* f, const rg_graph* g, int32_t level) {
+  return f && g && src1_applies(f, g, level) ? 1 : 0;
+}
+
 extern "C" int rg_layer_fwd_plan(const rg_frontier* f, const rg_graph* g, int32_t level, int64_t n_old, int64_t n_new,
                                  int64_t n_edges, int32_t ld) {
   if (!f || !g) return 1;
-  return plan_walk(f, g, level, n_old, n_new, n_edges, ld);
+  return plan_general(f, g, level, n_old, n_new, n_edges, ld);
 }
 
 extern "C" int rg_layer_fwd(const rg_frontier* f, const rg_graph* g, int32_t level, int64_t n_new, const float* hidden,
@@ -32,7 +45,9 @@
   RG_CHECK(f && g && hidden && rela && a_s && a_r && a_q && w_alpha && b_alpha && agg_out, "rg_layer_fwd: NULL argument");
   RG_CHECK((((uintptr_t)hidden | (uintptr_t)rela | (uintptr_t)a_s | (uintptr_t)a_r | (uintptr_t)a_q | (uintptr_t)agg_out |
              (uintptr_t)scratch) & 15) == 0, "rg_layer_fwd: float buffers must be 16-B aligned");
-  RG_CHECK(walk >= 0 && walk <= 7, "rg_layer_fwd: walk=%d not in 0..7", walk);
+  RG_CHECK(walk >= 0 && walk <= 8, "rg_layer_fwd: walk=%d not in 0..8", walk);
+  RG_CHECK(walk != 8 || src1_applies(f, g, level), "rg_layer_fwd: the single-source walk (8) needs level 1 of a frontier started by "
+           "rg_frontier_reset, on a static graph (level %d, newest %d)", level, f->level);
   rgfwd::FwdArgs A;
   if (rgfwd::fill_common("rg_layer_fwd", f, g, level, n_new, d, ld, ap, attn_dim, scratch, scratch_bytes,
                          rg_layer_fwd_scratch_bytes(f, g, ld), &A)) return 1;
@@ -45,6 +60,15 @@
   if (walk == 0)
     walk = plan_walk(f, g, level, f->n_nodes[(level - 1) % f->n_levels], f->n_nodes[level % f->n_levels],
                      level == f->level ? f->n_edges : -1, ld);
+  if (walk == 8) {
+    rgsrc1::Src1Args S;
+    S.B = f->B; S.W = f->W; S.sub = f->sub; S.out_ptr = g->out_ptr; S.in_ptr = g->in_ptr;
+    S.list_pk = g->out_bt_pk; S.list_rt = g->out_bt_rt; S.list_pos = g->out_bt_pos; S.bm_new = A.bm_new;
+    S.hidden = A.hidden; S.rela = A.rela; S.ld4 = A.ld4; S.a_s = A.a_s; S.a_r = A.a_r; S.a_q = A.a_q;
+    S.w_alpha = w_alpha; S.b_alpha = b_alpha; S.attn_dim = attn_dim; S.agg = A.agg;
+    f->queues_clean = A.walk.queues_clean;
+    return rgsrc1::launch(S, ld / 4, ap / 4, g->max_out_deg, s);
+  }
   if (walk >= 2 && f->n_nodes[(level - 1) % f->n_levels] < 0 && !rgwp::offsets_fit((int64_t)f->B * f->n_ent, ld))
     walk = 1;
   if (walk >= 2) {
diff --git a/red-gnn_amd/csrc/layer_fwd_src1.h b/red-gnn_amd/csrc/layer_fwd_src1.h
--- /dev/null
+++ b/red-gnn_amd/csrc/layer_fwd_src1.h
@@ -0,0 +1,29 @@
+#pragma once
+#include "common.h"
+
+namespace rgsrc1 {
+
+struct Src1Args {
+  int B, W;
+  const int32_t* sub;
+  const int32_t* out_ptr;
+  const int32_t* in_ptr;
+  const uint32_t* list_pk;
+  const int2* list_rt;
+  const int32_t* list_pos;
+  const int2* bm_new;
+  const float4* hidden;
+  const float4* rela;
+  int ld4;
+  const float4* a_s;
+  const float4* a_r;
+  const float4* a_q;
+  const float* w_alpha;
+  const float* b_alpha;
+  int attn_dim;
+  float4* agg;
+};
+
+int launch(const Src1Args& A, int ld4, int ap4, int max_out_deg, hipStream_t s);
+
+}
diff --git a/red-gnn_amd/csrc/layer_fwd_src1.hip b/red-gnn_amd/csrc/layer_fwd_src1.hip
--- /dev/null
+++ b/red-gnn_amd/csrc/layer_fwd_src1.hip
@@ -0,0 +1,143 @@
+#include "attn.h"
+#include "layer_fwd_src1.h"
+
+namespace rgsrc1 {
+namespace {
+
+constexpr int SRC1_BLOCK = 256;
+constexpr int SRC1_CHUNK = 32;
+constexpr int SRC1_MAX_Y = 8;
+
+template <int G, int AP4, bool PACKED>
+__global__ __launch_bounds__(SRC1_BLOCK) void layer_fwd_src1_kernel(Src1Args A) {
+  __shared__ float4 stage[SRC1_BLOCK];
+  constexpr int NG = SRC1_BLOCK / G;
+  const int b = blockIdx.x;
+  const int s = A.sub[b];
+  if (s < 0) return;
+  const int beg = A.out_ptr[s], end = A.out_ptr[s + 1];
+  const int n_chunks = (end - beg + SRC1_CHUNK - 1) / SRC1_CHUNK;
+  if ((int)blockIdx.y * NG >= n_chunks) return;
+
+  const int lane = threadIdx.x & 63;
+  const int lane_g = lane & (G - 1), grp = threadIdx.x / G;
+  float4* my_stage = stage + grp * G;
+  const bool row_lane = lane_g < A.ld4;
+  const int lane_c = row_lane ? lane_g : A.ld4 - 1;
+  const float4 hv = A.hidden[(int64_t)b * A.ld4 + lane_c];
+  const float b_alpha = A.b_alpha[0];
+  const int2* bm_row = A.bm_new + (int64_t)b * A.W;
+  const float4* as_p = A.a_s + (int64_t)b * AP4;
+  const float4* aq_p = A.a_q + (int64_t)b * AP4;
+
+  auto tail_of = [&](int i) -> int {
+    if constexpr (PACKED) return (int)(A.list_pk[i] & 0xFFFFF);
+    else return A.list_rt[i].y;
+  };
+
+  for (int c = (int)blockIdx.y * NG + grp; c < n_chunks; c += (int)gridDim.y * NG) {
+    const int lo = beg + c * SRC1_CHUNK, hi = min(lo + SRC1_CHUNK, end);
+    int skip_o = -1;
+    if (c > 0) {
+      const int tp = tail_of(lo - 1);
+      const int2 wp = bm_row[tp >> 5];
+      if (rg::bm_has(wp, tp)) skip_o = rg::bm_rank(wp, tp);
+    }
+    int cur_o = -2, cur_seg = 0;
+    bool started = false, done = false;
+    float4 acc = rg::f4zero(), total = rg::f4zero();
+    auto close_segment = [&]() {
+      if (!started) { total = acc; started = true; }
+      else { total.x += acc.x; total.y += acc.y; total.z += acc.z; total.w += acc.w; }
+    };
+    auto close_row = [&]() {
+      if (cur_o < 0) return;
+      close_segment();
+      if (row_lane) A.agg[(int64_t)cur_o * A.ld4 + lane_g] = total;
+    };
+
+    for (int i0 = lo; i0 < end && !done; i0 += G) {
+      const int i = i0 + lane_g;
+      int o = -1, r = 0, seg = 0;
+      float alpha = 0.f;
+      if (i < end) {
+        int t;
+        if constexpr (PACKED) { const uint32_t pk = A.list_pk[i]; t = pk & 0xFFFFF; r = pk >> 20; }
+        else { const int2 rt = A.list_rt[i]; r = rt.x; t = rt.y; }
+        const int pos = A.list_pos[i];
+        const int2 wp = bm_row[t >> 5];
+        const int ip0 = A.in_ptr[t], ip1 = A.in_ptr[t + 1];
+        if (rg::bm_has(wp, t)) {
+          o = rg::bm_rank(wp, t);
+          seg = ip1 - ip0 > RG_VROW_MAX ? (pos - ip0) / RG_VROW_MAX : 0;
+          float z = b_alpha;
+#pragma clang loop unroll_count(AP4 >= 8 ? 2 : AP4)
+          for (int k = 0; k < AP4; ++k) {
+            const float4 as = as_p[k];
+            const float4 ar = A.a_r[(int64_t)r * AP4 + k];
+            const float4 w = rg::attn_w4(A.w_alpha, A.attn_dim, k);
+            const float4 q = aq_p[k];
+            rg::attn_acc_fwd(z, w, as, ar, q);
+          }
+          alpha = rg::attn_alpha(z);
+        }
+      }
+      rg::strip_fence<false>();
+      my_stage[lane_g] = make_float4(__int_as_float(o), __int_as_float(r), alpha, __int_as_float(seg));
+      rg::strip_fence<false>();
+
+      const int n = min(G, end - i0);
+      for (int k0 = 0; k0 < n && !done; k0 += 4) {
+        float4 tp[4], rv[4];
+#pragma unroll
+        for (int u = 0; u < 4; ++u) tp[u] = my_stage[min(k0 + u, G - 1)];
+#pragma unroll
+        for (int u = 0; u < 4; ++u) rv[u] = A.rela[(int64_t)__float_as_int(tp[u].y) * A.ld4 + lane_c];
+#pragma unroll
+        for (int u = 0; u < 4; ++u) {
+          if (k0 + u >= n || done) continue;
+          const int ou = __float_as_int(tp[u].x), su = __float_as_int(tp[u].w);
+          if (i0 + k0 + u >= hi && ou != cur_o) { done = true; continue; }
+          if (ou < 0) continue;
+          if (skip_o >= 0) {
+            if (ou == skip_o) continue;
+            skip_o = -1;
+          }
+          if (ou != cur_o) {
+            close_row();
+            cur_o = ou; cur_seg = su; started = false; acc = rg::f4zero();
+          } else if (su != cur_seg) {
+            close_segment();
+            cur_seg = su; acc = rg::f4zero();
+          }
+          const float al = tp[u].z;
+          acc.x = fmaf(al, hv.x + rv[u].x, acc.x);
+          acc.y = fmaf(al, hv.y + rv[u].y, acc.y);
+          acc.z = fmaf(al, hv.z + rv[u].z, acc.z);
+          acc.w = fmaf(al, hv.w + rv[u].w, acc.w);
+        }
+      }
+    }
+    close_row();
+  }
+}
+
+template <int G, int AP4>
+int launch2(const Src1Args& A, int max_out_deg, hipStream_t s) {
+  constexpr int NG = SRC1_BLOCK / G;
+  const int y = (int)std::min<int64_t>(std::max<int64_t>(rg::ceil_div(rg::ceil_div(max_out_deg, SRC1_CHUNK), NG), 1), SRC1_MAX_Y);
+  if (A.list_pk) hipLaunchKernelGGL((layer_fwd_src1_kernel<G, AP4, true>), dim3(A.B, y), dim3(SRC1_BLOCK), 0, s, A);
+  else hipLaunchKernelGGL((layer_fwd_src1_kernel<G, AP4, false>), dim3(A.B, y), dim3(SRC1_BLOCK), 0, s, A);
+  RG_LAUNCH_CHECK();
+  return 0;
+}
+
+}
+
+int launch(const Src1Args& A, int ld4, int ap4, int max_out_deg, hipStream_t s) {
+  return rg::with_g(ld4, [&](auto g) {
+    return rg::with_ap4(ap4, "rg_layer_fwd", [&](auto ap) { return launch2<decltype(g)::value, decltype(ap)::value>(A, max_out_deg, s); });
+  });
+}
+
+}
diff --git a/red-gnn_amd/engine.py b/red-gnn_amd/engine.py
--- a/red-gnn_amd/engine.py
+++ b/red-gnn_amd/engine.py
@@ -83,6 +83,12 @@
         ihr = np.empty((self.n_fact, 2), np.int32)
         _lib.check(_lib.lib().rg_graph_export(self.handle, _lib.ptr(op), _lib.ptr(ort), _lib.ptr(ip), _lib.ptr(ihr)))
         return op, ort, ip, ihr
+
+    def export_out_by_tail(self):
+        rt = np.empty((self.n_fact, 2), np.int32)
+        pos = np.empty(self.n_fact, np.int32)
+        _lib.check(_lib.lib().rg_graph_export_out_by_tail(self.handle, _lib.ptr(rt), _lib.ptr(pos), None))
+        return rt, pos
 
     def close(self):
         if getattr(self, "handle", None) is not None and _lib._lib is not None:
@@ -455,6 +461,12 @@
     return int(_lib.lib().rg_layer_fwd_plan(frontier.handle, graph.handle, level, n_old, n_new, n_edges, ld))
 
 
+def layer_fwd_walk(frontier, graph, level, n_old, n_new, n_edges, ld):
+    if _lib.lib().rg_layer_fwd_single_source(frontier.handle, graph.handle, level):
+        return 8
+    return layer_fwd_plan(frontier, graph, level, n_old, n_new, n_edges, ld)
+
+
 def layer_fwd_scratch_bytes(frontier, graph, ld):
     return _lib.lib().rg_layer_fwd_scratch_bytes(frontier.handle, graph.handle, ld)
 
@@ -645,9 +657,9 @@
 
 
 def dense_fwd(agg, hidden_prev, prev_idx, d, W_h, act, gate, Ws_next=None, attn_dim=0, ap=0, W_final=None, nodes=None,
-              n_ent=0, scores_all=None, precision="f32"):
+              n_ent=0, scores_all=None, precision="f32", want_hidden=True):
     n, ld = agg.shape
-    hidden = torch.empty_like(agg)
+    hidden = torch.empty_like(agg) if want_hidden else None
     a_s = torch.empty((n, ap), dtype=torch.float32, device=agg.device) if Ws_next is not None else None
     c = lambda t: None if t is None else t.detach().contiguous()
     W_h, w_ih, w_hh, b_ih, b_hh = c(W_h), c(gate.weight_ih_l0), c(gate.weight_hh_l0), c(gate.bias_ih_l0), c(gate.bias_hh_l0)
diff --git a/red-gnn_amd/models.py b/red-gnn_amd/models.py
--- a/red-gnn_amd/models.py
+++ b/red-gnn_amd/models.py
@@ -265,7 +265,7 @@
             engine.layer_fwd_into(fr, graph, fr.level, n_hint, hidden, rela_p, d, a_s, a_r, a_q,
                                   layer.w_alpha.weight.reshape(-1).contiguous(), layer.w_alpha.bias, a, self.agg, self.scratch, walk=walk)
             last = i + 1 == m.n_layer
-            out_h, out_a = self.hid[i % 2], self.a_s[i % 2]
+            out_h, out_a = None if last else self.hid[i % 2], self.a_s[i % 2]
             engine.dense_fwd_dev(self.cap, fr.count_ptr(), self.agg, hidden, self.prev, d, layer.W_h.weight, m.act_name, m.gate, out_h,
                                  Ws_next=None if last else m.gnn_layers[i + 1].Ws_attn.weight, attn_dim=a, ap=ap,
                                  a_s_out=None if last else out_a, W_final=m.W_final.weight if last else None,
@@ -491,7 +491,7 @@
             n_new, n_e, n_old = fr.expand(graph)
             nodes, prev_idx, old_new = fr.nodes(want_prev=True, want_old_new=trace is not None)
             n_edges.append(n_e)
-            sizes.append((n_new, engine.layer_fwd_plan(fr, graph, fr.level, n_old, n_new, n_e, ld), n_e))
+            sizes.append((n_new, engine.layer_fwd_walk(fr, graph, fr.level, n_old, n_new, n_e, ld), n_e))
             layer = self.gnn_layers[i]
             if kept is not None:
                 kept.append(dict(a_s=a_s, tables=tables[i]))
@@ -501,7 +501,7 @@
                 agg, hidden, prev_idx, d, layer.W_h.weight, self.act_name, self.gate,
                 Ws_next=None if last else self.gnn_layers[i + 1].Ws_attn.weight, attn_dim=a, ap=ap,
                 W_final=self.W_final.weight if last else None, nodes=nodes, n_ent=n_ent, scores_all=scores_all,
-                precision=self.dense_precision)
+                precision=self.dense_precision, want_hidden=not last or trace is not None or kept is not None)
             if trace is not None:
                 trace.append(dict(nodes=nodes, old_nodes_new_idx=old_new, n_edges=n_e, hidden=hidden[:, :d]))
         self.last_stats = dict(n_edges=n_edges, n_nodes=int(nodes.shape[0]))
```

After: 31.29 billion edges/s (median of 6 runs). 1.03x the previous value.
